# defineZYP/ADT

Hardware: AMD Instinct MI355X
Metric: train sequences/sec, SASRec-ADT ml-1m (seq_len=200, d=64, 2 blocks) (higher is better)
Workload: dtype bf16; 1 GPU; SASRec-ADT ml-1m shape, 2 blocks d=64 H=2 seq_len=200, global batch 256 (256 sequences on this GPU), dropout 0.5, full train step (fwd+loss+bwd+clip+Adam), ids resident in HBM; global_batch=256, seq_len=200, parallelism=dp1, hip_graph=True, table_gradients=sorted segmented sums, bit-reproducible (ADT_ITEM_SORT=1), world_size=1

## Files before the change

### adt_amd/csrc/adt_attn_args.h

```cpp
#pragma once
#include "adt_common.cuh"

namespace adt {

struct AttnArgs {
  const float* Q; int ldq;
  const float* K; int ldk;
  const float* V; int ldv;
  float* O; int ldo;
  float* LSE;
  int B, H, L;
  int causal;
  float scale;
  DropCfg drop;
  uint32_t bh_offset;
  const float* dO; int lddo;
  float* dQ; int lddq;
  float* dK; int lddk;
  float* dV; int lddv;
  uint32_t* mask;
  unsigned long long* stamps;
  int in_bf16;
  int out_bf16;
  const void* do_bf16; const float* do_delta;
};

}
```

### adt_amd/csrc/adt_bwdchain_args.h

```cpp
#pragma once
#include "adt_common.cuh"

namespace adt {

struct BwdChainArgs {
  int T, L, B;
  const int* ids;
  DropCfg drop; uint32_t site1, site2; uint32_t row_offset;
  float ln_eps;
  const float* gy;
  const float* u;
  const float* xin;
  const float* o;
  const float* dqkv; int lddqkv;
  const float* dkv2;
  int grad_bf16;
  const float* dh;
  const float* f;
  const float* W0; const float* W1; const float* W2; const float* W3;
  const float* gamma; const float* beta;
  float* out0; int acc0;
  float* out1; int acc1;
  float* dW0; float* dW1; float* dW2; float* dW3;
  float* db0; float* db1; float* db2; float* db3;
  float* dgamma; float* dbeta;
  const float* rec; const float* drec; const float* Ws; float* dWs; float* dbs; int H;
  int ablate;
  int nrep; size_t rep_stride;
  float gy_scale;
  float* part[4]; size_t part_stride;
  int saved_bf16;
  unsigned long long* stamps;
  const float* wp_base; const void* wp_img;
  float* vpart;
  const float* lnl_x; const float* lnl_gamma; float lnl_eps; float* vpart2; float* lnl_dgamma; float* lnl_dbeta;
  void* do_bf16; float* do_delta; float do_scale; int do_hd;
  int nsplit;
};

}
```

### adt_amd/csrc/adt_sasrec.hip

```cpp
#include "adt_host.h"
#include <string.h>
#include <mutex>
#include "adt_bwdchain_args.h"
#include "adt_fwdchain_args.h"
#include "adt_seq_args.h"
#include "adt_seqbwd_args.h"

namespace {

constexpr float LN_EPS = 1e-8f;
constexpr int NREPP = 16;
constexpr int LN_PART_BLOCKS = 1024;
constexpr int NREP = 16;

struct Layout {
  int64_t off[4 + 30 * 16];
  int64_t total;
  int nl;
  int64_t item() const { return off[0]; }
  int64_t posw() const { return off[1]; }
  int64_t lnl_w() const { return off[2]; }
  int64_t lnl_b() const { return off[3]; }
  int64_t enc(int i, int k) const { return off[4 + 14 * i + k]; }
  int64_t dec(int i, int k) const { return off[4 + 14 * nl + 16 * i + k]; }
};
enum { E_LN1W, E_LN1B, E_INW, E_INB, E_OW, E_OB, E_LN2W, E_LN2B, E_C1W, E_C1B, E_C2W, E_C2B, E_SW, E_SB };
enum { D_LNW, D_LNB, D_SINW, D_SINB, D_SOW, D_SOB, D_EINW, D_EINB, D_EOW, D_EOB, D_C1W, D_C1B, D_C2W, D_C2B, D_UW, D_UB };

int64_t up64(int64_t x) { return (x + 63) / 64 * 64; }

StepPlan step_plan(const adt_sasrec_cfg* c, int B) {
  const StepFacts f{c->prec, c->maxlen, c->hidden, c->num_heads, c->num_layers, B, c->item_num + 1, adt_item_sort_supported(c->item_num + 1) != 0,
                    c->num_heads > 0 ? adt_seq_attn_bwd_lds(c->maxlen, c->num_heads) : 0};
  return adt_step_plan(f, adt_seq_switches());
}

bool make_layout(const adt_sasrec_cfg* c, Layout* lo) {
  if (c->num_layers < 1 || c->num_layers > 16) return false;
  const int64_t d = c->hidden, H = c->num_heads, hd = d / H, L = c->maxlen, V = c->item_num;
  lo->nl = c->num_layers;
  int64_t o = 0;
  int n = 0;
  auto put = [&](int64_t sz) { lo->off[n++] = o; o += up64(sz); };
  put((V + 1) * d); put(L * d); put(d); put(d);
  for (int i = 0; i < c->num_layers; ++i) {
    put(d); put(d); put(3 * d * d); put(3 * d); put(d * d); put(d); put(d); put(d);
    put(d * d); put(d); put(d * d); put(d); put(H * hd); put(H);
  }
  for (int i = 0; i < c->num_layers; ++i) {
    put(d); put(d);
    put(3 * d * d); put(3 * d); put(d * d); put(d);
    put(3 * d * d); put(3 * d); put(d * d); put(d);
    put(d * d); put(d); put(d * d); put(d); put(d); put(d);
  }
  lo->total = o;
  return true;
}

struct WS {
  int64_t T, d, H, L, nl, B;
  int64_t enc_x, dec_x, f, posl, negl;
  int64_t e_qn, e_qkv, e_o, e_lse, e_h, e_h2, e_u, e_rec, e_mask, e_stride;
  int64_t d_dn, d_qkv, d_o1, d_lse1, d_a1, d_q2, d_kv2, d_o2, d_lse2, d_a2, d_u, d_mask1, d_mask2, d_stride;
  int64_t g_enc_x, g_dec_x, g_f, g_pos, g_neg, g_rec;
  int64_t s1, s2, s3, s4, s5;
  int64_t loss, norms, scal;
  int64_t rep, rep_stride;
  int64_t prep, prep_stride;
  int64_t wpack;
  int64_t part, part_stride;
  int64_t isort, isort_n;
  int64_t dodelta;
  int64_t vpart, vcall, lnpart, gnpart;
  int64_t total;
};

void make_ws(const adt_sasrec_cfg* c, int B, const StepPlan& pl, WS* w) {
  w->B = B; w->d = c->hidden; w->H = c->num_heads; w->L = c->maxlen; w->nl = c->num_layers;
  w->T = (int64_t)B * w->L;
  const int64_t Td = up64(w->T * w->d), T1 = up64(w->T), lse = up64((int64_t)B * w->H * w->L);
  const int64_t rec = up64(w->T * w->H * w->H);
  int64_t o = 0;
  auto take = [&](int64_t n) { int64_t r = o; o += n; return r; };
  w->enc_x = take((w->nl + 1) * Td); w->dec_x = take((w->nl + 1) * Td); w->f = take(Td);
  w->posl = take(T1); w->negl = take(T1);
  {
    const int64_t s = o;
    w->e_qn = take(Td); w->e_qkv = take(3 * Td); w->e_o = take(Td); w->e_lse = take(lse); w->e_h = take(Td);
    w->e_h2 = take(Td); w->e_u = take(Td); w->e_rec = take(rec); w->e_mask = take(8 * lse);
    w->e_stride = o - s;
    o = s + w->e_stride * w->nl;
  }
  {
    const int64_t s = o;
    w->d_dn = take(Td); w->d_qkv = take(3 * Td); w->d_o1 = take(Td); w->d_lse1 = take(lse); w->d_a1 = take(Td);
    w->d_q2 = take(Td); w->d_kv2 = take(2 * Td); w->d_o2 = take(Td); w->d_lse2 = take(lse); w->d_a2 = take(Td);
    w->d_u = take(Td); w->d_mask1 = take(8 * lse); w->d_mask2 = take(8 * lse);
    w->d_stride = o - s;
    o = s + w->d_stride * w->nl;
  }
  w->g_enc_x = take((w->nl + 1) * Td); w->g_dec_x = take((w->nl + 1) * Td); w->g_f = take(Td);
  w->g_pos = take(T1); w->g_neg = take(T1); w->g_rec = take(rec * w->nl);
  w->s1 = take(Td); w->s2 = take(Td); w->s3 = take(3 * Td); w->s4 = take(2 * Td); w->s5 = take(Td);
  w->loss = take(64 * (2 + 2 * 16)); w->norms = take(64); w->scal = take(192);
  w->rep_stride = up64((int64_t)(c->item_num + 1) * w->d);
  w->rep = take(NREP * w->rep_stride);
  {
    Layout lo;
    make_layout(c, &lo);
    w->prep_stride = up64(lo.total - lo.posw());
    w->prep = take(NREPP * w->prep_stride);
    w->wpack = take(3 * w->prep_stride);
  }
  w->part_stride = pl.parts_area ? (int64_t)w->nl * 16 * 4096 : 0;
  w->part = take((int64_t)B * pl.seq_split * w->part_stride);
  w->isort_n = pl.sort_area ? adt_item_sort_work_ints(4, (int)w->T, c->item_num + 1) : 0;
  w->isort = take(up64(w->isort_n));
  w->vcall = (int64_t)B * pl.seq_split * 512;
  w->vpart = take(w->part_stride > 0 ? (5 * w->nl + 1) * w->vcall : 0);
  w->lnpart = take(LN_PART_BLOCKS * 128);
  w->gnpart = take(4096);
  w->dodelta = take(pl.do_handover ? up64(w->T * 4) : 0);
  w->total = o;
}

#define CK(call) do { int _r = (call); if (_r) return _r; } while (0)

struct SideStream {
  hipStream_t s = nullptr;
  hipEvent_t fork_ev[4] = {nullptr, nullptr, nullptr, nullptr}, join_ev[4] = {nullptr, nullptr, nullptr, nullptr};
};
SideStream* side_stream(const StepPlan& pl, hipStream_t main) {
  static SideStream g[16];
  static std::mutex mu;
  if (!pl.side_sites) return nullptr;
  int dev = 0;
  if (hipGetDevice(&dev) != hipSuccess || dev < 0 || dev >= 16) return nullptr;
  SideStream* sd = &g[dev];
  std::lock_guard<std::mutex> lock(mu);
  if (sd->s) return sd;
  hipStreamCaptureStatus cs = hipStreamCaptureStatusNone;
  if (hipStreamIsCapturing(main, &cs) != hipSuccess || cs != hipStreamCaptureStatusNone) { (void)hipGetLastError(); return nullptr; }
  hipStream_t s = nullptr;
  if (hipStreamCreateWithFlags(&s, hipStreamNonBlocking) != hipSuccess) { (void)hipGetLastError(); return nullptr; }
  for (int i = 0; i < 4; ++i)
    if (hipEventCreateWithFlags(&sd->fork_ev[i], hipEventDisableTiming) != hipSuccess ||
        hipEventCreateWithFlags(&sd->join_ev[i], hipEventDisableTiming) != hipSuccess) {
      (void)hipGetLastError();
      (void)hipStreamDestroy(s);
      return nullptr;
    }
  sd->s = s;
  return sd;
}
int side_mark(SideStream* sd, int k, void* main) {
  if (!sd) return 0;
  if (hipEventRecord(sd->fork_ev[k], (hipStream_t)main) != hipSuccess) return adt_set_error("backward: side-stream fork %d failed", k);
  return 0;
}
int side_enter(SideStream* sd, int k, void* main, void** out) {
  *out = main;
  if (!sd) return 0;
  if (hipStreamWaitEvent(sd->s, sd->fork_ev[k], 0) != hipSuccess) return adt_set_error("backward: side-stream fork %d failed", k);
  *out = sd->s;
  return 0;
}
int side_join(SideStream* sd, int k, void* main) {
  if (!sd) return 0;
  if (hipEventRecord(sd->join_ev[k], sd->s) != hipSuccess || hipStreamWaitEvent((hipStream_t)main, sd->join_ev[k], 0) != hipSuccess)
    return adt_set_error("backward: side-stream join %d failed", k);
  return 0;
}

int layout_ws(const adt_sasrec_cfg* c, int B, Layout* lo, WS* w, StepPlan* pl) {
  *pl = step_plan(c, B);
// ... 44 lines not shown
int partial_slots(const adt_sasrec_cfg* c, const Layout& lo, bool enc, bool dec, int* slots, int* offs);
int partial_nwg(const StepPlan& pl, int slot, int B) {
  const int k = slot % 16;
  const bool attn_block = (k >= PS_E_IN && k < PS_E_IN + 3) || (k >= PS_D_SIN && k < PS_D_SIN + 3);
  return attn_block ? B * pl.attn_split : B * pl.seq_split;
}
int reduce_partials(const adt_sasrec_cfg* c, const Layout& lo, const WS& w, const StepPlan& pl, float* G, float* ws, bool enc, bool dec, void* st) {
  int slots[256], offs[256];
  const int n = partial_slots(c, lo, enc, dec, slots, offs);
  int nwg[256];
  for (int i = 0; i < n; ++i) nwg[i] = partial_nwg(pl, slots[i], (int)w.B);
  return adt_dwpart_reduce_n(G, ws + w.part, (size_t)w.part_stride, (int)w.B, nwg, slots, offs, n, st);
}
int partial_slots(const adt_sasrec_cfg* c, const Layout& lo, bool enc, bool dec, int* slots, int* offs) {
  int n = 0;
  const int dd = c->hidden * c->hidden;
  for (int i = 0; i < c->num_layers; ++i) {
    if (enc) {
      for (int j = 0; j < 3; ++j) { slots[n] = 16 * i + PS_E_IN + j; offs[n++] = (int)(lo.enc(i, E_INW) + j * dd); }
      slots[n] = 16 * i + PS_E_O; offs[n++] = (int)lo.enc(i, E_OW);
      slots[n] = 16 * i + PS_E_C1; offs[n++] = (int)lo.enc(i, E_C1W);
      slots[n] = 16 * i + PS_E_C2; offs[n++] = (int)lo.enc(i, E_C2W);
    }
    if (dec) {
      for (int j = 0; j < 3; ++j) { slots[n] = 16 * i + PS_D_SIN + j; offs[n++] = (int)(lo.dec(i, D_SINW) + j * dd); }
      for (int j = 0; j < 3; ++j) { slots[n] = 16 * i + PS_D_EIN + j; offs[n++] = (int)(lo.dec(i, D_EINW) + j * dd); }
      slots[n] = 16 * i + PS_D_SO; offs[n++] = (int)lo.dec(i, D_SOW);
      slots[n] = 16 * i + PS_D_EO; offs[n++] = (int)lo.dec(i, D_EOW);
      slots[n] = 16 * i + PS_D_C1; offs[n++] = (int)lo.dec(i, D_C1W);
      slots[n] = 16 * i + PS_D_C2; offs[n++] = (int)lo.dec(i, D_C2W);
    }
  }
  return n;
}

adt::SeqBwdArgs seq_bwd_args(int L, int B, int H, const int32_t* ids, float p, const uint32_t* seed, uint32_t site, uint32_t b_offset, int hd) {
  adt::SeqBwdArgs a;
  memset(&a, 0, sizeof(a));
  a.L = L; a.B = B; a.H = H; a.ids = ids; a.drop = adt_make_drop(p, seed, site); a.b_offset = b_offset; a.ln_eps = LN_EPS;
  a.scale = 1.0f / sqrtf((float)hd);
  return a;
}

adt::SeqFwdArgs seq_args(int nsplit, int L, int B, int H, const int32_t* ids, float p, const uint32_t* seed, uint32_t b_offset, int hd) {
  adt::SeqFwdArgs a;
  memset(&a, 0, sizeof(a));
  a.nsplit = nsplit;
  a.L = L; a.B = B; a.H = H; a.ids = ids; a.drop = adt_make_drop(p, seed, 0); a.b_offset = b_offset; a.ln_eps = LN_EPS;
  a.scale = 1.0f / sqrtf((float)hd);
  return a;
}

adt::SeqFwdArgs enc_layer_seq_args(const adt_sasrec_cfg* c, const Layout& lo, const WS& w, const StepPlan& pl, const float* P, float* ws, const int32_t* seq,
                                   float p, const uint32_t* seed, uint32_t b_offset, int i, bool training_outputs, bool lean) {
  const int d = (int)w.d, H = (int)w.H, hd = d / H, L = (int)w.L, B = (int)w.B, prec = c->prec;
  const int64_t Td = up64(w.T * w.d);
  float* x = ws + w.enc_x + i * Td;
  float* y = ws + w.enc_x + (i + 1) * Td;
  float* base = ws + i * w.e_stride;
  adt::SeqFwdArgs a = seq_args(pl.seq_split, L, B, H, seq, p, seed, b_offset, hd);
  a.x = i == 0 ? nullptr : x; a.E = P + lo.item(); a.P = P + lo.posw(); a.emb_scale = sqrtf((float)d); a.site_emb = SITE_EMB_SEQ;
  a.site_attn = enc_site(i, 0); a.site1 = enc_site(i, 1); a.site2 = enc_site(i, 2);
  a.gamma = P + lo.enc(i, E_LN1W); a.beta = P + lo.enc(i, E_LN1B); a.Win = P + lo.enc(i, E_INW); a.bin = P + lo.enc(i, E_INB);
  a.Wo = P + lo.enc(i, E_OW); a.bo = P + lo.enc(i, E_OB); a.gamma2 = P + lo.enc(i, E_LN2W); a.beta2 = P + lo.enc(i, E_LN2B);
  a.W1 = P + lo.enc(i, E_C1W); a.b1 = P + lo.enc(i, E_C1B); a.W2 = P + lo.enc(i, E_C2W); a.b2 = P + lo.enc(i, E_C2B);
  a.x_out = x; a.xn = base + w.e_qn; a.qkv = base + w.e_qkv; a.o = base + w.e_o; a.lse = base + w.e_lse;
  a.mask = reinterpret_cast<uint32_t*>(base + w.e_mask); a.h = base + w.e_h; a.u = base + w.e_u; a.y = y;
  if (training_outputs && H > 1) { a.rec = base + w.e_rec; a.Ws = P + lo.enc(i, E_SW); a.bs = P + lo.enc(i, E_SB); }
  a.wp_base = P + lo.posw(); a.wp_img = prec == ADT_PREC_BF16 ? (const void*)(ws + w.wpack) : nullptr;
  if (lean) { a.xn = nullptr; a.qkv = nullptr; a.saved_bf16 = 1; }
  return a;
}

int encoder_forward(const adt_sasrec_cfg* c, const Layout& lo, const WS& w, const StepPlan& pl, const float* P, float* ws,
                    const int32_t* seq, const int32_t* pos, const int32_t* neg, float p, const uint32_t* seed,
                    uint32_t b_offset, bool training_outputs, void* st, bool packed = false) {
  const int T = (int)w.T, d = (int)w.d, H = (int)w.H, hd = d / H, L = (int)w.L, B = (int)w.B, prec = c->prec, nl = c->num_layers;
  const int64_t Td = up64(w.T * w.d);
  const uint32_t ro = b_offset * (uint32_t)L;
  const int dd = d * d;
  const bool use_seq = pl.use_seq;
  const bool lean = training_outputs && pl.lean;
  if (!packed) CK(pack_weights(c, lo, w, P, ws, st));
  const float* wp_base = P + lo.posw();
  const void* wp_img = prec == ADT_PREC_BF16 ? (const void*)(ws + w.wpack) : nullptr;
  for (int i = 0; i < nl; ++i) {
    float* x = ws + w.enc_x + i * Td;
    float* y = ws + w.enc_x + (i + 1) * Td;
    float* base = ws + i * w.e_stride;
    float *qn = base + w.e_qn, *qkv = base + w.e_qkv, *o = base + w.e_o, *lse = base + w.e_lse, *h = base + w.e_h,
          *u = base + w.e_u, *rec = base + w.e_rec;
    const float* inw = P + lo.enc(i, E_INW);
    const float* inb = P + lo.enc(i, E_INB);
    if (use_seq) {
      const adt::SeqFwdArgs a = enc_layer_seq_args(c, lo, w, pl, P, ws, seq, p, seed, b_offset, i, training_outputs, lean);
      CK(adt_launch_seq_enc_fwd(hd, a, st));
      continue;
    }
    {
      adt::FwdChainArgs a = fwd_args(T, L, B, H, seq, p, seed, ro);
      a.x = i == 0 ? nullptr : x; a.E = P + lo.item(); a.P = P + lo.posw(); a.emb_scale = sqrtf((float)d); a.site0 = SITE_EMB_SEQ;
      a.gamma = P + lo.enc(i, E_LN1W); a.beta = P + lo.enc(i, E_LN1B);
      for (int j = 0; j < 3; ++j) { a.W[j] = inw + j * dd; a.b[j] = inb + j * d; }
      a.o0 = x; a.ld0 = d; a.o1 = qn; a.ld1 = d; a.o2 = qkv; a.ld2 = 3 * d;
      CK(adt_launch_fwdchain(prec, 0, a, st));
    }
    CK(adt_attn_fwd(prec, qkv, 3 * d, qkv + d, 3 * d, qkv + 2 * d, 3 * d, B, H, L, hd, 1, p, seed, enc_site(i, 0), b_offset, o, d,
                    lse, reinterpret_cast<uint32_t*>(base + w.e_mask), st));
    {
      adt::FwdChainArgs a = fwd_args(T, L, B, H, seq, p, seed, ro);
      a.x = o; a.r0 = qn; a.site1 = enc_site(i, 1); a.site2 = enc_site(i, 2);
      a.W[0] = P + lo.enc(i, E_OW); a.b[0] = P + lo.enc(i, E_OB);
      a.W[1] = P + lo.enc(i, E_C1W); a.b[1] = P + lo.enc(i, E_C1B);
      a.W[2] = P + lo.enc(i, E_C2W); a.b[2] = P + lo.enc(i, E_C2B);
      a.gamma = P + lo.enc(i, E_LN2W); a.beta = P + lo.enc(i, E_LN2B);
      a.o0 = h; a.ld0 = d; a.o1 = u; a.ld1 = d; a.o2 = y; a.ld2 = d;
      int which = 2;
      if (training_outputs) {
        a.rec = rec; a.Ws = P + lo.enc(i, E_SW); a.bs = P + lo.enc(i, E_SB);
        which = H <= 2 ? 6 : (H <= 4 ? 7 : 8);
      }
      CK(adt_launch_fwdchain(prec, which, a, st));
    }
  }
  for (int j0 = 0; j0 == 0 || (training_outputs && !use_seq && j0 < nl); j0 += 2) {
    adt::FwdChainArgs a = fwd_args(T, L, B, H, seq, 0.f, nullptr, ro);
    a.x = ws + w.enc_x + nl * Td; a.gamma = P + lo.lnl_w(); a.beta = P + lo.lnl_b();
    if (j0 == 0) { a.o0 = ws + w.f; a.ld0 = d; }
    if (training_outputs) {
      if (j0 == 0) { a.E = P + lo.item(); a.pos = pos; a.neg = neg; a.pos_logits = ws + w.posl; a.neg_logits = ws + w.negl; }
      a.nkv = use_seq ? 0 : (nl - j0 >= 2 ? 2 : 1);
      for (int k = 0; k < a.nkv; ++k) {
        const float* einw = P + lo.dec(j0 + k, D_EINW);
        const float* einb = P + lo.dec(j0 + k, D_EINB);
        a.W[2 * k] = einw + dd; a.W[2 * k + 1] = einw + 2 * dd; a.b[2 * k] = einb + d; a.b[2 * k + 1] = einb + 2 * d;
        float* kv2 = ws + (j0 + k) * w.d_stride + w.d_kv2;
        if (k == 0) { a.o2 = kv2; a.ld2 = 2 * d; } else { a.o3 = kv2; a.ld3 = 2 * d; }
      }
    }
    CK(adt_launch_fwdchain(prec, 5, a, st));
  }
  return 0;
}

adt::SeqFwdArgs dec_layer_seq_args(const Layout& lo, const WS& w, const StepPlan& pl, const float* P, float* ws, const int32_t* dec, float p,
                                   const uint32_t* seed, uint32_t b_offset, int i) {
  const int d = (int)w.d, H = (int)w.H, hd = d / H, L = (int)w.L, B_ = (int)w.B;
  const int64_t Td = up64(w.T * w.d);
  float* x = ws + w.dec_x + i * Td;
  float* y = ws + w.dec_x + (i + 1) * Td;
  float* base = ws + i * w.d_stride;
  float *dn = base + w.d_dn, *qkv = base + w.d_qkv, *o1 = base + w.d_o1, *lse1 = base + w.d_lse1, *a1 = base + w.d_a1,
        *q2 = base + w.d_q2, *kv2 = base + w.d_kv2, *o2 = base + w.d_o2, *lse2 = base + w.d_lse2, *a2 = base + w.d_a2, *u = base + w.d_u;
  adt::SeqFwdArgs a = seq_args(pl.seq_split, L, B_, H, dec, p, seed, b_offset, hd);
  a.x = i == 0 ? nullptr : x; a.E = P + lo.item(); a.P = P + lo.posw(); a.emb_scale = sqrtf((float)d); a.site_emb = SITE_EMB_DEC;
  a.site_attn = dec_site(i, 0); a.site_attn2 = dec_site(i, 1); a.site1 = dec_site(i, 2); a.site2 = dec_site(i, 3);
  a.gamma = P + lo.dec(i, D_LNW); a.beta = P + lo.dec(i, D_LNB); a.Win = P + lo.dec(i, D_SINW); a.bin = P + lo.dec(i, D_SINB);
  a.Wo = P + lo.dec(i, D_SOW); a.bo = P + lo.dec(i, D_SOB); a.f = ws + w.f; a.Win2 = P + lo.dec(i, D_EINW); a.bin2 = P + lo.dec(i, D_EINB);
  a.Wo2 = P + lo.dec(i, D_EOW); a.bo2 = P + lo.dec(i, D_EOB);
  a.W1 = P + lo.dec(i, D_C1W); a.b1 = P + lo.dec(i, D_C1B); a.W2 = P + lo.dec(i, D_C2W); a.b2 = P + lo.dec(i, D_C2B);
  a.x_out = x; a.xn = dn; a.qkv = qkv; a.o = o1; a.lse = lse1; a.mask = reinterpret_cast<uint32_t*>(base + w.d_mask1);
  a.a1 = a1; a.q2 = q2; a.kv2 = kv2; a.o2 = o2; a.lse2 = lse2; a.mask2 = reinterpret_cast<uint32_t*>(base + w.d_mask2);
  a.h = a2; a.u = u; a.y = y;
  a.wp_base = P + lo.posw(); a.wp_img = ws + w.wpack;
  if (pl.lean) { a.xn = nullptr; a.qkv = nullptr; a.saved_bf16 = 1; }
  return a;
}
int dec_layer_seq_fwd(const Layout& lo, const WS& w, const StepPlan& pl, const float* P, float* ws, const int32_t* dec, float p,
                      const uint32_t* seed, uint32_t b_offset, int i, void* st) {
  const adt::SeqFwdArgs a = dec_layer_seq_args(lo, w, pl, P, ws, dec, p, seed, b_offset, i);
  return adt_launch_seq_dec_fwd((int)(w.d / w.H), a, st);
}

SideStream* fwd_logits_stream(const StepPlan& pl, void* st) { return ((pl.side_sites & 1) && !pl.bce_merged) ? side_stream(pl, (hipStream_t)st) : nullptr; }
bool ring_prefetch_split(const adt::RingPrefetchArgs& rr, bool bce_by_forward, const StepPlan& pl) {
  return rr.ring && rr.staging && rr.state && bce_by_forward && pl.embed3_on;
}

struct LossPtrs { const float *A[4], *Bm[4], *rc[4]; float *GA[4], *GB[4], *lm[4], *dr[4], *ln[4]; };
AdtLossSeedsJob loss_terms(const WS& w, float* ws, const float* lambdas1, const float* lambdas2, bool all_seeds, LossPtrs* q) {
  const int nl = (int)w.nl, H = (int)w.H;
  const int64_t Td = up64(w.T * w.d), rec = up64(w.T * w.H * w.H);
  float* loss = ws + w.loss;
  for (int i = 0; i < nl; ++i) {
    q->A[i] = ws + w.enc_x + i * Td; q->Bm[i] = ws + w.dec_x + (nl - i) * Td;
    q->GA[i] = all_seeds ? ws + w.g_enc_x + i * Td : nullptr;
    q->GB[i] = (all_seeds || i == 0) ? ws + w.g_dec_x + (nl - i) * Td : nullptr;
    q->lm[i] = loss + 64 * (2 + i);
    q->rc[i] = ws + i * w.e_stride + w.e_rec; q->dr[i] = ws + w.g_rec + i * rec; q->ln[i] = loss + 64 * (2 + nl + i);
  }
  AdtLossSeedsJob j{};
  j.T = (int)w.T; j.norms = ws + w.norms; j.loss_bce = loss;
  j.nmse = nl; j.A = q->A; j.Bm = q->Bm; j.n = w.T * w.d; j.lambdas = lambdas1; j.GA = q->GA; j.GB = q->GB; j.loss_mse = q->lm;
  j.nnll = H > 1 ? nl : 0; j.rec = q->rc; j.n_rows = (int)w.T; j.H = H; j.lambda2 = lambdas2[nl - 1]; j.drec = q->dr; j.loss_nll = q->ln;
  return j;
}

int forward_loss_lean(const adt_sasrec_cfg* c, const Layout& lo, const WS& w, const StepPlan& pl, const float* P, float* ws, const int32_t* seq, const int32_t* dec,
                      const int32_t* pos, const int32_t* neg, bool bce_side, float p, const uint32_t* seed, uint32_t b_offset, const float* lambdas1,
                      const float* lambdas2, const adt::RingPrefetchArgs& rr, void* st) {
  const int hd = (int)(w.d / w.H), nl = c->num_layers;
  if (!pl.bce_deferred) return 1;
  for (int i = 0; i < nl; ++i) {
    adt::SeqFwdArgs a = enc_layer_seq_args(c, lo, w, pl, P, ws, seq, p, seed, b_offset, i, true, true);
    if (i == nl - 1) { a.lnl_gamma = P + lo.lnl_w(); a.lnl_beta = P + lo.lnl_b(); a.f_out = ws + w.f; }
    CK(adt_launch_seq_enc_fwd(hd, a, st));
  }
  for (int j = 0; j < nl; ++j) CK(dec_layer_seq_fwd(lo, w, pl, P, ws, dec, p, seed, b_offset, j, st));
  LossPtrs q;
  AdtLossSeedsJob job = loss_terms(w, ws, lambdas1, lambdas2, false, &q);
  job.ring = &rr; job.split = ring_prefetch_split(rr, bce_side, pl);
  const adt::LogitsBceArgs lb{ws + w.f, P + lo.item(), pos, neg, ws + w.norms, (int)w.T, ws + w.posl, ws + w.negl, ws + w.g_pos, ws + w.g_neg, ws + w.loss,
                              ws + w.g_f, pl.det ? nullptr : ws + w.rep, NREP, (size_t)w.rep_stride, pl.embed3_on ? 1 : 0};
  const bool merged = bce_side && pl.bce_merged;
  if (merged) job.logits = &lb;
  SideStream* const sd = (bce_side && !merged) ? fwd_logits_stream(pl, st) : nullptr;
  if (bce_side && !merged) CK(side_mark(sd, 0, st));
  CK(adt_loss_seeds_prefetch(job, st));
  if (bce_side && !merged) {
    void* s2 = nullptr;
    CK(side_enter(sd, 0, st, &s2));
    CK(adt_logits_bce_scatter_ex(lb.F, lb.E, pos, neg, lb.norms, lb.T, lb.pos_logits, lb.neg_logits, lb.dpos, lb.dneg, lb.loss, lb.dF, lb.rep, lb.nrep,
                                 w.rep_stride, lb.neg_only, s2));
    if (sd && hipEventRecord(sd->join_ev[0], sd->s) != hipSuccess) return adt_set_error("forward_loss: logits event");
  }
  return 0;
}

int g_time_which = 0, g_time_layer = 0;
hipEvent_t g_time_ev0 = nullptr, g_time_ev1 = nullptr;
inline void time_mark(int which, int layer, bool start, void* st) {
  if (!g_time_ev0 || !g_time_ev1 || g_time_layer != layer) return;
  if (g_time_which == 3 && which == 1 && start) {
    (void)hipEventRecord(g_time_ev0, (hipStream_t)st);
    (void)hipEventRecord(g_time_ev1, (hipStream_t)st);
  } else if (g_time_which == which) {
    (void)hipEventRecord(start ? g_time_ev0 : g_time_ev1, (hipStream_t)st);
  }
}

const char* const NO_FALLBACK = "backward: shape L=%d hd=%d left the per-sequence kernels although the partial-gradient path was chosen";

struct Bwd {
  const adt_sasrec_cfg* c; Layout lo; WS w;
  const float* P; float* G; float* ws;
  const int32_t *seq, *dec, *pos, *neg;
  float p; const uint32_t* seed; uint32_t b_offset, ro;
  void* st;
  BwdPlan plan;
  StepPlan sp;
  BwdCallPlan call;
  adt::RingPrefetchArgs ring;
  int T, d, H, hd, L, prec, nl;
  int64_t Td, recsz;
  float* Gq;
  float *s1, *s3, *s4, *s5, *gf;
  void* do_rows() const { return sp.do_handover ? (void*)s3 : nullptr; }
  void* do_rows_cross() const { return sp.do_handover ? (void*)s1 : nullptr; }
  float* do_delta() const { return sp.do_handover ? ws + w.dodelta : nullptr; }
  float do_scale(uint32_t site) const { return adt_make_drop(p, seed, site).scale; }
  const float* f;
  SideStream *sd, *sd_sort;

  adt::BwdChainArgs BA(const int32_t* ids, float pp, const uint32_t* sdp) const {
    adt::BwdChainArgs a = bwd_args(T, L, (int)w.B, ids, pp, sdp, ro);
    a.nrep = NREPP; a.rep_stride = (size_t)w.prep_stride;
    a.wp_base = P + lo.posw(); a.wp_img = prec == ADT_PREC_BF16 ? (const void*)(ws + w.wpack) : nullptr;
    a.nsplit = sp.seq_split;
    return a;
  }
  float* PART(int layer, int slot) const { return sp.parts ? ws + w.part + (int64_t)(16 * layer + slot) * 4096 : nullptr; }
  float* VPART(int layer, int k) const { return call.late_parts ? ws + w.vpart + (int64_t)(5 * layer + k) * w.vcall : nullptr; }
  int logits_scatter(void* s) const {
    if (plan.bce_here)
      return adt_logits_bce_scatter_ex(f, P + lo.item(), pos, neg, ws + w.norms, T, ws + w.posl, ws + w.negl, ws + w.g_pos, ws + w.g_neg, ws + w.loss,
                                       gf, sp.det ? nullptr : ws + w.rep, NREP, w.rep_stride, call.embed3 ? 1 : 0, s);
    if (sp.det) return adt_logits_bwd_df(P + lo.item(), pos, neg, ws + w.g_pos, ws + w.g_neg, T, d, gf, d, s);
    return adt_logits_bwd_scatter(f, d, P + lo.item(), pos, neg, ws + w.g_pos, ws + w.g_neg, T, d, gf, d, ws + w.rep, NREP, w.rep_stride, s);
  }
  int zero_unless_prezeroed(int64_t at, size_t n, void* s) const {
    return (!plan.prep_zeroed && adt::zero_f32_async(ws + at, n, (hipStream_t)s)) ? adt_set_error("replica zero") : 0;
  }
};

int bwd_init(Bwd& x, const adt_sasrec_cfg* c, const float* P, float* G, float* ws, const int32_t* seq, const int32_t* dec, const int32_t* pos,
             const int32_t* neg, int B, int training, const uint32_t* seed, uint32_t b_offset, int phase, const adt::RingPrefetchArgs& ring, void* st) {
  CK(layout_ws(c, B, &x.lo, &x.w, &x.sp));
  if (const char* err = adt_bwd_plan(phase, x.sp.bce_deferred, &x.plan)) return adt_set_error("%s", err);
  x.call = adt_bwd_call_plan(x.sp, x.plan);
  const WS& w = x.w;
  x.c = c; x.P = P; x.G = G; x.ws = ws; x.seq = seq; x.dec = dec; x.pos = pos; x.neg = neg; x.seed = seed; x.b_offset = b_offset; x.st = st; x.ring = ring;
  x.T = (int)w.T; x.d = (int)w.d; x.H = (int)w.H; x.hd = x.d / x.H; x.L = (int)w.L; x.prec = c->prec; x.nl = c->num_layers;
  x.Td = up64(w.T * w.d); x.recsz = up64(w.T * w.H * w.H);
  x.p = training ? c->dropout : 0.f;
  x.ro = b_offset * (uint32_t)x.L;
  x.s1 = ws + w.s1; x.s3 = ws + w.s3; x.s4 = ws + w.s4; x.s5 = ws + w.s5; x.gf = ws + w.g_f; x.f = ws + w.f;
  x.Gq = ws + w.prep - x.lo.posw();
  x.sd_sort = x.sp.det ? side_stream(x.sp, (hipStream_t)st) : nullptr;
  x.sd = x.call.side ? side_stream(x.sp, (hipStream_t)st) : nullptr;
  return 0;
}

struct LogitsSide {
  enum { DONE, MARKED, ENQUEUED, BY_FORWARD } at = DONE;

  int begin(const Bwd& x) {
    const WS& w = x.w;
    if (x.plan.bce_fwd) {
      at = BY_FORWARD;
    } else if (x.sp.det) {
      CK(x.zero_unless_prezeroed(w.prep, (size_t)NREPP * w.prep_stride, x.st));
      CK(x.logits_scatter(x.st));
    } else if (x.sd && (x.sp.side_sites & 1)) {
      CK(side_mark(x.sd, 0, x.st));
      CK(x.zero_unless_prezeroed(w.prep, (size_t)NREPP * w.prep_stride, x.st));
      at = MARKED;
    } else {
      CK(x.zero_unless_prezeroed(w.rep, (size_t)NREP * w.rep_stride + (size_t)NREPP * w.prep_stride, x.st));
      CK(x.logits_scatter(x.st));
    }
    return 0;
  }
  int after_first_chain_kernel(const Bwd& x) {
    if (at != MARKED) return 0;
    void* s2 = nullptr;
    CK(side_enter(x.sd, 0, x.st, &s2));
    CK(x.zero_unless_prezeroed(x.w.rep, (size_t)NREP * x.w.rep_stride, s2));
    CK(x.logits_scatter(s2));
    at = ENQUEUED;
    return 0;
  }
  int join(const Bwd& x) {
    if (at == ENQUEUED) CK(side_join(x.sd, 0, x.st));
    if (at == BY_FORWARD) {
      SideStream* const sl = fwd_logits_stream(x.sp, x.st);
      if (sl && hipStreamWaitEvent((hipStream_t)x.st, sl->join_ev[0], 0) != hipSuccess) return adt_set_error("backward: logits join");
    }
    at = DONE;
    return 0;
  }
};

int dec_post_bwd(const Bwd& x, int i) {
  const WS& w = x.w; const Layout& lo = x.lo; const float* P = x.P; float* const Gq = x.Gq;
  float* base = x.ws + i * w.d_stride;
  adt::BwdChainArgs a = x.BA(x.dec, x.p, x.seed);
  a.site1 = dec_site(i, 2); a.site2 = dec_site(i, 3);
  a.gy = x.ws + w.g_dec_x + (i + 1) * x.Td; a.u = base + w.d_u; a.xin = base + w.d_a2; a.o = base + w.d_o2; a.saved_bf16 = x.sp.lean;
  a.W0 = P + lo.dec(i, D_C2W); a.W1 = P + lo.dec(i, D_C1W); a.W2 = P + lo.dec(i, D_EOW);
  a.dW0 = Gq + lo.dec(i, D_C2W); a.dW1 = Gq + lo.dec(i, D_C1W); a.dW2 = Gq + lo.dec(i, D_EOW);
  a.db0 = Gq + lo.dec(i, D_C2B); a.db1 = Gq + lo.dec(i, D_C1B); a.db2 = Gq + lo.dec(i, D_EOB);
  a.out0 = x.s1;
  a.do_bf16 = x.do_rows_cross(); a.do_delta = x.do_delta(); a.do_scale = x.do_scale(dec_site(i, 1)); a.do_hd = x.hd;
  a.part[0] = x.PART(i, PS_D_C2); a.part[1] = x.PART(i, PS_D_C1); a.part[2] = x.PART(i, PS_D_EO); a.part_stride = (size_t)w.part_stride;
  a.vpart = x.VPART(i, 0);
  const int rc = x.sp.use_seq ? adt_launch_seq_post_bwd(x.hd, 0, a, x.st) : 1;
  if (rc < 0) return rc;
  if (rc && x.sp.parts) return adt_set_error(NO_FALLBACK, x.L, x.hd);
  return rc ? adt_launch_bwdchain(x.prec, 1, a, x.st) : 0;
}

adt::AttnArgs dec_cross_attn_lean_args(const Bwd& x, int i);

int dec_cross_attn_bwd(const Bwd& x, int i) {
  const WS& w = x.w; const int d = x.d, B = (int)w.B;
  float* base = x.ws + i * w.d_stride;
  float *q2 = base + w.d_q2, *kv2 = base + w.d_kv2, *o2 = base + w.d_o2, *lse2 = base + w.d_lse2, *s4 = x.s4;
  const uint32_t* mask2 = reinterpret_cast<const uint32_t*>(base + w.d_mask2);
  if (!x.sp.lean)
    return adt_attn_bwd(x.prec, q2, d, kv2, 2 * d, kv2 + d, 2 * d, o2, d, lse2, x.s1, d, B, x.H, x.L, x.hd, 1, x.p, x.seed, dec_site(i, 1), x.b_offset,
                        x.s5, d, s4, 2 * d, s4 + d, 2 * d, mask2, x.st);
  if (x.sp.do_handover) {
    const int rc = adt_launch_seq_attn_bwd(x.hd, dec_cross_attn_lean_args(x, i), x.st);
    return rc == 1 ? adt_set_error(NO_FALLBACK, x.L, x.hd) : rc;
  }
  const uint16_t* kvb = reinterpret_cast<const uint16_t*>(kv2);
  return adt_attn_bwd_saved_bf16(q2, d, kvb, 2 * d, kvb + d, 2 * d, o2, d, lse2, x.s1, d, B, x.H, x.L, x.hd, x.p, x.seed, dec_site(i, 1), x.b_offset,
                                 x.s5, d, s4, 2 * d, x.sp.parts ? s4 + d / 2 : s4 + d, 2 * d, mask2, x.sp.parts ? 1 : 0, x.st);
}

adt::BwdChainArgs dec_mid_seq_args(const Bwd& x, int i) {
  const WS& w = x.w; const Layout& lo = x.lo; const float* P = x.P; float* const Gq = x.Gq;
  const int d = x.d, dd = d * d;
  float* base = x.ws + i * w.d_stride;
  const float* einw = P + lo.dec(i, D_EINW);
  float* geinw = Gq + lo.dec(i, D_EINW);
  float* geinb = Gq + lo.dec(i, D_EINB);
  adt::BwdChainArgs a = x.BA(x.dec, 0.f, nullptr);
  a.dqkv = x.s5; a.lddqkv = d; a.xin = base + w.d_a1; a.o = base + w.d_o1; a.saved_bf16 = x.sp.lean; a.dkv2 = x.s4; a.f = x.f;
  a.grad_bf16 = (x.sp.lean && x.sp.parts) ? 1 : 0;
  a.W0 = einw; a.W1 = P + lo.dec(i, D_SOW); a.W2 = einw + dd; a.W3 = einw + 2 * dd;
  a.dW0 = geinw; a.dW1 = Gq + lo.dec(i, D_SOW); a.dW2 = geinw + dd; a.dW3 = geinw + 2 * dd;
  a.db0 = geinb; a.db1 = Gq + lo.dec(i, D_SOB); a.db2 = geinb + d; a.db3 = geinb + 2 * d;
  a.out0 = x.s1; a.out1 = x.gf; a.acc1 = 1;
  a.part[0] = x.PART(i, PS_D_EIN); a.part[1] = x.PART(i, PS_D_SO); a.part[2] = x.PART(i, PS_D_EIN + 1); a.part[3] = x.PART(i, PS_D_EIN + 2);
  a.part_stride = (size_t)w.part_stride;
  a.vpart = x.VPART(i, 1);
  a.do_bf16 = x.do_rows(); a.do_delta = x.do_delta(); a.do_scale = x.do_scale(dec_site(i, 0)); a.do_hd = x.hd;
  return a;
}

adt::AttnArgs dec_cross_attn_lean_args(const Bwd& x, int i) {
  const WS& w = x.w; const int d = x.d;
  float* base = x.ws + i * w.d_stride;
  const uint16_t* kvb = reinterpret_cast<const uint16_t*>(base + w.d_kv2);
  adt::AttnArgs a = adt_attn_bwd_saved_bf16_args(base + w.d_q2, d, kvb, 2 * d, kvb + d, 2 * d, base + w.d_o2, d, base + w.d_lse2, x.s1, d, (int)w.B, x.H, x.L,
                                                 x.hd, x.p, x.seed, dec_site(i, 1), x.b_offset, x.s5, d, x.s4, 2 * d, x.s4 + d / 2, 2 * d,
                                                 reinterpret_cast<const uint32_t*>(base + w.d_mask2), 1);
  a.do_bf16 = x.do_rows_cross(); a.do_delta = x.do_delta();
  return a;
}

int dec_mid_bwd(const Bwd& x, int i) {
  const WS& w = x.w; const Layout& lo = x.lo; const float* P = x.P; float* const Gq = x.Gq;
  const int d = x.d, dd = d * d;
  float* base = x.ws + i * w.d_stride;
  float *o1 = base + w.d_o1, *a1 = base + w.d_a1;
  const float* einw = P + lo.dec(i, D_EINW);
  float* geinw = Gq + lo.dec(i, D_EINW);
  float* geinb = Gq + lo.dec(i, D_EINB);
  if (x.sp.use_seq) {
    const int rc = adt_launch_seq_mid_bwd(x.hd, dec_mid_seq_args(x, i), x.st);
    if (rc <= 0) return rc;
    if (x.sp.parts) return adt_set_error(NO_FALLBACK, x.L, x.hd);
  }
  {
    adt::BwdChainArgs a = x.BA(x.dec, 0.f, nullptr);
    a.dqkv = x.s5; a.lddqkv = d; a.xin = a1; a.o = o1; a.saved_bf16 = x.sp.lean;
    a.W0 = einw; a.W1 = P + lo.dec(i, D_SOW);
    a.dW0 = geinw; a.dW1 = Gq + lo.dec(i, D_SOW); a.db0 = geinb; a.db1 = Gq + lo.dec(i, D_SOB);
    a.out0 = x.s1;
    CK(adt_launch_bwdchain(x.prec, 4, a, x.st));
  }
  adt::BwdChainArgs a = x.BA(x.dec, 0.f, nullptr);
  a.dkv2 = x.s4; a.f = x.f;
  a.W0 = einw + dd; a.W1 = einw + 2 * dd;
  a.dW0 = geinw + dd; a.dW1 = geinw + 2 * dd; a.db0 = geinb + d; a.db1 = geinb + 2 * d;
  a.out0 = x.gf; a.acc0 = 1;
  return adt_launch_bwdchain(x.prec, 5, a, x.st);
}

int attn_block_bwd(const Bwd& x, int i, bool dec) {
  const WS& w = x.w; const Layout& lo = x.lo; const float* P = x.P; float* const Gq = x.Gq; float* const ws = x.ws;
  const int d = x.d, dd = d * d, nl = x.nl;
  const int32_t* ids = dec ? x.dec : x.seq;
  float* gy = ws + (dec ? w.g_dec_x : w.g_enc_x) + (i + 1) * x.Td;
  float* gx = ws + (dec ? w.g_dec_x : w.g_enc_x) + i * x.Td;
  const float* xi = ws + (dec ? w.dec_x : w.enc_x) + i * x.Td;
  float* base = ws + i * (dec ? w.d_stride : w.e_stride);
  float *qkv = base + (dec ? w.d_qkv : w.e_qkv), *o = base + (dec ? w.d_o1 : w.e_o), *lse = base + (dec ? w.d_lse1 : w.e_lse);
  const uint32_t* mask = reinterpret_cast<const uint32_t*>(base + (dec ? w.d_mask1 : w.e_mask));
  const int64_t lnw = dec ? lo.dec(i, D_LNW) : lo.enc(i, E_LN1W), lnb = dec ? lo.dec(i, D_LNB) : lo.enc(i, E_LN1B);
  const int64_t inw = dec ? lo.dec(i, D_SINW) : lo.enc(i, E_INW), inb = dec ? lo.dec(i, D_SINB) : lo.enc(i, E_INB);
  const uint32_t site = dec ? dec_site(i, 0) : enc_site(i, 0);
  const int acc = dec ? (i > 0 ? 1 : 0) : 1;
  if (x.sp.use_seq) {
    adt::SeqBwdArgs a = seq_bwd_args(x.L, (int)w.B, x.H, ids, x.p, x.seed, site, x.b_offset, x.hd);
    a.x = xi; a.gamma = P + lnw; a.beta = P + lnb; a.Win = P + inw; a.bin = P + inb;
    a.dO = x.s1; a.o = o; a.lse = lse; a.mask = mask; a.dres = dec ? gy : x.s5;
    a.do_bf16 = x.do_rows(); a.do_delta = x.do_delta();
    a.gx = gx; a.acc = acc; a.dWin = Gq + inw; a.dbin = Gq + inb; a.dgamma = Gq + lnw; a.dbeta = Gq + lnb;
    if (x.plan.seeds_virtual && dec && i > 0) {
      a.acc = 0; a.seed_other = ws + w.enc_x + (nl - i) * x.Td; a.seed_coef = ws + w.norms + 8 + (nl - i);
    }
    if (x.plan.seeds_virtual && !dec) {
      a.acc = 0; a.seed_other = ws + w.dec_x + (nl - i) * x.Td; a.seed_coef = ws + w.norms + 8 + i;
      if (i > 0) { a.seed_loss = ws + w.loss + 64 * (2 + i); a.seed_norms = ws + w.norms; }
    }
    a.nrep = NREPP; a.rep_stride = (size_t)w.prep_stride; a.wp_base = P + lo.posw(); a.wp_img = ws + w.wpack; a.saved_bf16 = x.sp.lean;
    a.part = x.PART(i, dec ? PS_D_SIN : PS_E_IN); a.part_stride = (size_t)w.part_stride;
    a.vpart = x.VPART(i, dec ? 2 : 4);
    a.nsplit = a.part ? x.sp.attn_split : 1;
    time_mark(dec ? 2 : 1, i, true, x.st);
    const int rc = adt_launch_seq_attn_pre_bwd(x.hd, dec ? 1 : 0, a, x.st);
    time_mark(dec ? 2 : 1, i, false, x.st);
    if (rc <= 0) return rc;
    if (x.sp.lean) return adt_set_error("backward: the lean forward needs the fused attention-block backward (L=%d hd=%d)", x.L, x.hd);
  }
  if (x.sp.do_handover) return adt_set_error("backward: the staged attention backward was reached with the dO hand-over on (L=%d hd=%d)", x.L, x.hd);
  CK(adt_attn_bwd(x.prec, qkv, 3 * d, qkv + d, 3 * d, qkv + 2 * d, 3 * d, o, d, lse, x.s1, d, (int)w.B, x.H, x.L, x.hd, 1, x.p, x.seed, site, x.b_offset,
                  x.s3, 3 * d, x.s3 + d, 3 * d, x.s3 + 2 * d, 3 * d, mask, x.st));
  adt::BwdChainArgs a = x.BA(ids, 0.f, nullptr);
  a.dqkv = x.s3; a.lddqkv = 3 * d; a.xin = xi;
  if (dec) a.gy = gy; else a.dh = x.s5;
  a.W0 = P + inw; a.W1 = P + inw + dd; a.W2 = P + inw + 2 * dd; a.gamma = P + lnw; a.beta = P + lnb;
  a.dW0 = Gq + inw; a.dW1 = Gq + inw + dd; a.dW2 = Gq + inw + 2 * dd; a.db0 = Gq + inb; a.db1 = Gq + inb + d; a.db2 = Gq + inb + 2 * d;
  a.dgamma = Gq + lnw; a.dbeta = Gq + lnb;
  a.out0 = gx; a.acc0 = acc;
  return adt_launch_bwdchain(x.prec, dec ? 3 : 2, a, x.st);
}

int dec_block_backward(const Bwd& x, int i, LogitsSide& logits) {
  CK(dec_post_bwd(x, i));
  CK(logits.after_first_chain_kernel(x));
  if (x.sp.use_seq && x.sp.lean && x.sp.parts) {
    const adt::AttnArgs at = dec_cross_attn_lean_args(x, i);
    const adt::BwdChainArgs mid = dec_mid_seq_args(x, i);
    if (adt_seq_xattn_mid_covered(x.hd, at, mid)) {
      CK(logits.join(x));
      const int rc = adt_launch_seq_xattn_mid_bwd(x.hd, at, mid, x.st);
      if (rc) return rc < 0 ? rc : adt_set_error("backward: the fused cross-attention + mid launch refused a shape it covers (L=%d hd=%d)", x.L, x.hd);
      return attn_block_bwd(x, i, true);
    }
  }
  CK(dec_cross_attn_bwd(x, i));
  CK(logits.join(x));
  CK(dec_mid_bwd(x, i));
  return attn_block_bwd(x, i, true);
}

struct DecSide {
  enum { NONE, MARKED, ENQUEUED } at = NONE;
  bool parts_done = false;
// ... 26 lines not shown
    return 0;
  }
  int enter(const Bwd& x) {
    if (at != MARKED) return 0;
    void* s2 = nullptr;
    CK(side_enter(x.sd, 1, x.st, &s2));
    if (!x.sp.det && !x.call.embed3) CK(embed(x, s2));
    if (x.sp.parts && !x.call.late_parts) { CK(reduce_partials(x.c, x.lo, x.w, x.sp, x.G, x.ws, false, true, s2)); parts_done = true; }
    at = ENQUEUED;
    return 0;
  }
  int join(const Bwd& x, bool covered) {
    if (at == ENQUEUED && !covered) CK(side_join(x.sd, 1, x.st));
    at = NONE;
    return 0;
  }
};

int last_layernorm_bwd(const Bwd& x) {
  const WS& w = x.w; const Layout& lo = x.lo; float* const ws = x.ws;
  const int d = x.d;
  if (x.sp.lnl_fused) return 0;
  if (x.call.late_parts) {
    const int nb = adt_layernorm_bwd_parts(x.gf, d, ws + w.enc_x + x.nl * x.Td, d, x.P + lo.lnl_w(), LN_EPS, x.T, d, ws + w.g_enc_x + x.nl * x.Td, d, 0,
                                           ws + w.lnpart, LN_PART_BLOCKS, x.st);
    return nb < 0 ? nb : 0;
  }
  return adt_layernorm_bwd_rep(x.gf, d, ws + w.enc_x + x.nl * x.Td, d, x.P + lo.lnl_w(), LN_EPS, x.T, d, ws + w.g_enc_x + x.nl * x.Td, d, 0,
                               x.Gq + lo.lnl_w(), x.Gq + lo.lnl_b(), NREPP, w.prep_stride, x.st);
}

int enc_post_bwd(const Bwd& x, int i) {
  const WS& w = x.w; const Layout& lo = x.lo; const float* P = x.P; float* const Gq = x.Gq; float* const ws = x.ws;
  const int H = x.H, nl = x.nl;
  float* base = ws + i * w.e_stride;
  adt::BwdChainArgs a = x.BA(x.seq, x.p, x.seed);
  a.site1 = enc_site(i, 1); a.site2 = enc_site(i, 2);
  a.gy = ws + w.g_enc_x + (i + 1) * x.Td; a.u = base + w.e_u; a.xin = base + w.e_h; a.o = base + w.e_o; a.saved_bf16 = x.sp.lean;
  a.W0 = P + lo.enc(i, E_C2W); a.W1 = P + lo.enc(i, E_C1W); a.W2 = P + lo.enc(i, E_OW);
  a.gamma = P + lo.enc(i, E_LN2W); a.beta = P + lo.enc(i, E_LN2B);
  a.dW0 = Gq + lo.enc(i, E_C2W); a.dW1 = Gq + lo.enc(i, E_C1W); a.dW2 = Gq + lo.enc(i, E_OW);
  a.db0 = Gq + lo.enc(i, E_C2B); a.db1 = Gq + lo.enc(i, E_C1B); a.db2 = Gq + lo.enc(i, E_OB);
  a.dgamma = Gq + lo.enc(i, E_LN2W); a.dbeta = Gq + lo.enc(i, E_LN2B);
  a.out0 = x.s5; a.out1 = x.s1;
  int which = 0;
  if (H > 1 && H <= 4) {
    which = H <= 2 ? 6 : 7;
    a.rec = base + w.e_rec; a.drec = ws + w.g_rec + i * x.recsz; a.Ws = P + lo.enc(i, E_SW); a.dWs = Gq + lo.enc(i, E_SW);
    a.dbs = Gq + lo.enc(i, E_SB); a.H = H;
  }
  a.part[0] = x.PART(i, PS_E_C2); a.part[1] = x.PART(i, PS_E_C1); a.part[2] = x.PART(i, PS_E_O); a.part_stride = (size_t)w.part_stride;
  a.vpart = x.VPART(i, 3);
  a.do_bf16 = x.do_rows(); a.do_delta = x.do_delta(); a.do_scale = x.do_scale(enc_site(i, 0)); a.do_hd = x.hd;
  if (x.sp.lnl_fused && i == nl - 1) {
    a.gy = x.gf; a.lnl_x = ws + w.enc_x + nl * x.Td; a.lnl_gamma = P + lo.lnl_w(); a.lnl_eps = LN_EPS;
    a.vpart2 = x.call.late_parts ? ws + w.vpart + (int64_t)(5 * nl) * w.vcall : nullptr;
    a.lnl_dgamma = Gq + lo.lnl_w(); a.lnl_dbeta = Gq + lo.lnl_b();
  }
  const int rc = x.sp.use_seq ? adt_launch_seq_post_bwd(x.hd, 1, a, x.st) : 1;
  if (rc < 0) return rc;
  if (rc && x.sp.parts) return adt_set_error(NO_FALLBACK, x.L, x.hd);
  return rc ? adt_launch_bwdchain(x.prec, which, a, x.st) : 0;
}

int enc_block_backward(const Bwd& x, int i, DecSide& dec_side) {
  const WS& w = x.w; const Layout& lo = x.lo;
  CK(enc_post_bwd(x, i));
  if (x.sp.lnl_fused && i == x.nl - 1) CK(dec_side.enter(x));
  if (x.H > 4) {
    float* base = x.ws + i * w.e_stride;
    CK(adt_headcls_bwd(base + w.e_o, x.d, x.P + lo.enc(i, E_SW), base + w.e_rec, x.ws + w.g_rec + i * x.recsz, (int)w.B, x.L, x.H, x.hd, x.s1, x.d,
                       x.G + lo.enc(i, E_SW), x.G + lo.enc(i, E_SB), x.st));
  }
  return attn_block_bwd(x, i, false);
}

int table_gradients(const Bwd& x, DecSide& dec_side) {
  const WS& w = x.w; const Layout& lo = x.lo; float* const ws = x.ws; float* const G = x.G;
  const int phase = x.plan.phase;
  if (phase == 2 && !x.sp.det && adt::zero_f32_async(ws + w.rep, (size_t)NREP * w.rep_stride, (hipStream_t)x.st)) return adt_set_error("replica zero");
  SideStream* const sd2 = ((x.sp.side_sites & 4) && x.sp.parts && !x.call.late_parts) ? x.sd : nullptr;
  CK(dec_side.join(x, sd2 != nullptr));
  void* s2 = nullptr;
  CK(side_mark(sd2, 2, x.st));
  if (x.sp.det) {
    if (x.sd_sort && hipStreamWaitEvent((hipStream_t)x.st, x.sd_sort->join_ev[3], 0) != hipSuccess) return adt_set_error("backward: sort join");
    const uint32_t site4[4] = {SITE_EMB_SEQ, SITE_EMB_DEC, 0u, 0u};
    const int32_t* const ids2[2] = {x.seq, x.dec};
    const float* const dx2[2] = {ws + w.g_enc_x, ws + w.g_dec_x};
    CK(adt_item_segsum_posemb(reinterpret_cast<int32_t*>(ws + w.isort), 4, x.T, x.c->item_num + 1, 0xFu, site4, x.p, x.seed, sqrtf((float)x.d), G + lo.item(),
                              x.plan.prep_zeroed ? 0 : 1, ids2, dx2, site4, 2, (int)w.B, x.L, x.ro, G + lo.posw(), x.st));
  } else if (x.call.embed3) {
    const bool by_forward = phase == 2 ? x.plan.seeds_virtual : x.plan.bce_fwd;
    CK(adt_embed_bwd3_prefetch(x.seq, x.dec, x.pos, ws + w.g_enc_x, ws + w.g_dec_x, x.f, ws + w.g_pos, x.T, x.L, x.p, x.seed, SITE_EMB_SEQ, SITE_EMB_DEC, x.ro,
                               G + lo.posw(), ws + w.rep, NREP, w.rep_stride, ring_prefetch_split(x.ring, by_forward, x.sp) ? &x.ring : nullptr, x.st));
  } else {
    CK(adt_embed_bwd_rep(x.seq, ws + w.g_enc_x, x.T, x.L, x.d, x.p, x.seed, SITE_EMB_SEQ, x.ro, G + lo.posw(), ws + w.rep, NREP, w.rep_stride, x.st));
  }
  CK(side_enter(sd2, 2, x.st, &s2));
  if (x.sp.parts && !x.call.late_parts) CK(reduce_partials(x.c, lo, w, x.sp, G, ws, true, phase == 0 && !dec_side.parts_done, s2));
  CK(side_join(sd2, 2, x.st));
  if (x.plan.defer_fold) return 0;
  return adt_replica_reduce2(G + lo.item(), ws + w.rep, (int64_t)(x.c->item_num + 1) * x.d, x.sp.det ? 0 : NREP, w.rep_stride, G + lo.posw(), x.Gq + lo.posw(),
                             (phase == 0 ? lo.total : lo.dec(0, 0)) - lo.posw(), NREPP, w.prep_stride, x.st);
}

// ... 30 lines not shown

extern "C" {

int64_t adt_sasrec_param_layout(const adt_sasrec_cfg* cfg, int64_t* offsets) {
  Layout lo;
  if (!make_layout(cfg, &lo)) return adt_set_error("param_layout: bad cfg");
  if (offsets)
    for (int i = 0; i < 4 + 30 * cfg->num_layers; ++i) offsets[i] = lo.off[i];
  return lo.total;
}

int64_t adt_sasrec_workspace_floats(const adt_sasrec_cfg* cfg, int B) {
  WS w;
  make_ws(cfg, B, step_plan(cfg, B), &w);
  return w.total;
}

int64_t adt_sasrec_ws_offset(const adt_sasrec_cfg* cfg, int B, int what, int layer) {
  WS w;
  make_ws(cfg, B, step_plan(cfg, B), &w);
  const int64_t Td = up64(w.T * w.d), rec = up64(w.T * w.H * w.H);
  switch (what) {
    case ADT_WS_ENC_X: return w.enc_x + layer * Td;
    case ADT_WS_DEC_X: return w.dec_x + layer * Td;
    case ADT_WS_REC: return layer * w.e_stride + w.e_rec;
    case ADT_WS_POS_LOGITS: return w.posl;
    case ADT_WS_NEG_LOGITS: return w.negl;
    case ADT_WS_F: return w.f;
    case ADT_WS_G_ENC_X: return w.g_enc_x + layer * Td;
    case ADT_WS_G_DEC_X: return w.g_dec_x + layer * Td;
    case ADT_WS_G_REC: return w.g_rec + layer * rec;
    case ADT_WS_G_POS: return w.g_pos;
    case ADT_WS_G_NEG: return w.g_neg;
    case ADT_WS_LOSS: return w.loss;
    case ADT_WS_NORMS: return w.norms;
    case ADT_WS_SCAL: return w.scal;
  }
  return adt_set_error("ws_offset: unknown id %d", what);
}

int adt_sasrec_forward(const adt_sasrec_cfg* c, const float* P, float* ws, const int32_t* seq, const int32_t* dec,
                       const int32_t* pos, const int32_t* neg, int B, int training, const uint32_t* seed,
                       uint32_t b_offset, void* st) {
  Layout lo;
  WS w;
  StepPlan pl;
  CK(layout_ws(c, B, &lo, &w, &pl));
  const int T = (int)w.T, d = (int)w.d, H = (int)w.H, hd = d / H, L = (int)w.L, prec = c->prec;
  const int64_t Td = up64(w.T * w.d);
  const bool packed = (training & ADT_TRAIN_PACKED) != 0;
  training &= ADT_TRAIN_DROPOUT;
  const float p = training ? c->dropout : 0.f;
  const uint32_t ro = b_offset * (uint32_t)L;
  CK(encoder_forward(c, lo, w, pl, P, ws, seq, pos, neg, p, seed, b_offset, true, st, packed));
  const float* f = ws + w.f;
  const int dd = d * d;
  const int B_ = (int)w.B;
  for (int i = 0; i < c->num_layers; ++i) {
    float* x = ws + w.dec_x + i * Td;
    float* y = ws + w.dec_x + (i + 1) * Td;
    float* base = ws + i * w.d_stride;
    float *dn = base + w.d_dn, *qkv = base + w.d_qkv, *o1 = base + w.d_o1, *lse1 = base + w.d_lse1, *a1 = base + w.d_a1,
          *q2 = base + w.d_q2, *kv2 = base + w.d_kv2, *o2 = base + w.d_o2, *lse2 = base + w.d_lse2, *a2 = base + w.d_a2,
          *u = base + w.d_u;
    const float* sinw = P + lo.dec(i, D_SINW);
    const float* sinb = P + lo.dec(i, D_SINB);
    const float* einw = P + lo.dec(i, D_EINW);
    const float* einb = P + lo.dec(i, D_EINB);
    if (pl.use_seq) {
      CK(dec_layer_seq_fwd(lo, w, pl, P, ws, dec, p, seed, b_offset, i, st));
      continue;
    }
    {
      adt::FwdChainArgs a = fwd_args(T, L, B_, H, dec, p, seed, ro);
      a.x = i == 0 ? nullptr : x; a.E = P + lo.item(); a.P = P + lo.posw(); a.emb_scale = sqrtf((float)d); a.site0 = SITE_EMB_DEC;
      a.gamma = P + lo.dec(i, D_LNW); a.beta = P + lo.dec(i, D_LNB);
      for (int j = 0; j < 3; ++j) { a.W[j] = sinw + j * dd; a.b[j] = sinb + j * d; }
      a.o0 = x; a.ld0 = d; a.o1 = dn; a.ld1 = d; a.o2 = qkv; a.ld2 = 3 * d;
      CK(adt_launch_fwdchain(prec, 1, a, st));
    }
    CK(adt_attn_fwd(prec, qkv, 3 * d, qkv + d, 3 * d, qkv + 2 * d, 3 * d, B_, H, L, hd, 1, p, seed, dec_site(i, 0), b_offset, o1, d,
                    lse1, reinterpret_cast<uint32_t*>(base + w.d_mask1), st));
    {
      adt::FwdChainArgs a = fwd_args(T, L, B_, H, dec, 0.f, nullptr, ro);
      a.x = o1; a.W[0] = P + lo.dec(i, D_SOW); a.b[0] = P + lo.dec(i, D_SOB); a.W[1] = einw; a.b[1] = einb;
      a.o0 = a1; a.ld0 = d; a.o2 = q2; a.ld2 = d;
      CK(adt_launch_fwdchain(prec, 3, a, st));
    }
    CK(adt_attn_fwd(prec, q2, d, kv2, 2 * d, kv2 + d, 2 * d, B_, H, L, hd, 1, p, seed, dec_site(i, 1), b_offset, o2, d, lse2,
                    reinterpret_cast<uint32_t*>(base + w.d_mask2), st));
    {
      adt::FwdChainArgs a = fwd_args(T, L, B_, H, dec, p, seed, ro);
      a.x = o2; a.r0 = dn; a.site1 = dec_site(i, 2); a.site2 = dec_site(i, 3);
      a.W[0] = P + lo.dec(i, D_EOW); a.b[0] = P + lo.dec(i, D_EOB);
      a.W[1] = P + lo.dec(i, D_C1W); a.b[1] = P + lo.dec(i, D_C1B);
      a.W[2] = P + lo.dec(i, D_C2W); a.b[2] = P + lo.dec(i, D_C2B);
      a.o0 = a2; a.ld0 = d; a.o1 = u; a.ld1 = d; a.o2 = y; a.ld2 = d;
      CK(adt_launch_fwdchain(prec, 4, a, st));
    }
  }
  return 0;
}

int adt_sasrec_bce_deferred(const adt_sasrec_cfg* c) {
  const StepPlan pl = step_plan(c, 1);
  if (pl.cfg_error[0]) (void)adt_set_error("%s", pl.cfg_error);
  return !pl.cfg_error[0] && pl.bce_deferred ? 1 : 0;
// ... 335 lines not shown
```

### adt_amd/csrc/adt_seq.hip

```cpp
#include "adt_host.h"
#include <limits.h>
#include <atomic>
#include "adt_seqfwd.cuh"
#include "adt_seqfwd_tt.cuh"
#include "adt_seqattn.cuh"
#include "adt_seqbwd_tt.cuh"
#include "adt_seqpost_tt.cuh"
#include "adt_seqxattn_tt.cuh"

using namespace adt;

template <class Args>
static int seq_launch(const void* fn, size_t smem, AdtLdsOptIn& slot, int grid, const Args* args, hipStream_t s, const char* what, int nwaves = SQ_NW,
                      size_t optin = 0) {
  return adt_launch_lds1(fn, dim3(grid), dim3(nwaves * 64), smem, *args, s, what, slot, optin);
}

__global__ __launch_bounds__(256) void k_pack_wimg(PackArgs a) { pack_wimg_block(a, blockIdx.x); }

extern "C" int adt_pack_wimg(const float* base, void* img, const int* offs, int n, void* stream) {
  if (n < 1 || n > 256) return adt_set_error("pack_wimg: %d blocks", n);
  PackArgs a;
  a.base = base; a.img = reinterpret_cast<__bf16*>(img); a.n = n;
  for (int i = 0; i < n; ++i) a.off[i] = offs[i];
  hipLaunchKernelGGL(k_pack_wimg, dim3(n), dim3(256), 0, (hipStream_t)stream, a);
  return adt_check_launch("pack_wimg");
}

static_assert(ADT_SEQ_MAXLEN == SQ_LP && ADT_SEQ_MAXLEN == SB_R, "adt_step_plan.h restates the image rows of these kernels");

const SeqSwitches& adt_seq_switches() {
  static const SeqSwitches sw = [] {
    SeqSwitches s;
    s.seq = adt_env_on("ADT_SEQ"); s.seq_lean = adt_env_on("ADT_SEQ_LEAN"); s.seq_tt = adt_env_on("ADT_SEQ_TT"); s.seq_bwd = adt_env_on("ADT_SEQ_BWD");
    s.seq_attn_bwd = adt_env_on("ADT_SEQ_ATTN_BWD"); s.seq_post_bwd = adt_env_on("ADT_SEQ_POST_BWD"); s.seq_partials = adt_env_on("ADT_SEQ_PARTIALS");
    s.xattn_fused = adt_env_on("ADT_XATTN_FUSED"); s.do_bf16 = adt_env_on("ADT_DO_BF16");
    s.seq_ablate = adt_env_int("ADT_SEQ_ABLATE", 0); s.seq_ablate_set = adt_env_int("ADT_SEQ_ABLATE", INT_MIN) != INT_MIN;
    s.seq_split = adt_env_int("ADT_SEQ_SPLIT", 0); s.attn_split = adt_env_on("ADT_ATTN_SPLIT");
    s.side_stream = adt_env_int("ADT_SIDE_STREAM", 7); s.side_stream_dp = adt_env_int("ADT_SIDE_STREAM_DP", 0) != 0;
    s.item_sort = adt_env_int("ADT_ITEM_SORT", 0) != 0;
    s.lnl_fused = adt_env_on("ADT_LNL_FUSED"); s.fold_parts = adt_env_on("ADT_FOLD_PARTS"); s.fwd_fused = adt_env_on("ADT_FWD_FUSED");
    s.embed3 = adt_env_on("ADT_EMBED3"); s.bce_merged = adt_env_on("ADT_BCE_MERGED");
    return s;
  }();
  return sw;
}

static SeqAttnFacts attn_facts(const AttnArgs& a) {
  return {a.L, a.H, a.B, a.causal != 0, a.in_bf16 != 0, a.out_bf16 != 0, a.ldq, a.ldk, a.ldv, a.ldo, a.lddo, a.drop.thr != 0, a.mask != nullptr,
          sab_lds_bytes(a.L, a.H), xm_lds_bytes(a.L, a.H)};
}
size_t adt_seq_attn_bwd_lds(int L, int H) { return sab_lds_bytes(L, H); }
static SeqChainFacts chain_facts(const BwdChainArgs& a) {
  return {a.L, a.H, a.B, a.T, a.wp_img != nullptr, a.saved_bf16 != 0, a.grad_bf16 != 0, a.part[0] && a.part[1] && a.part[2] && a.part[3], a.nsplit, a.ablate,
          a.drec != nullptr};
}

static unsigned long long* g_stamps = nullptr;

extern "C" int adt_seq_stamps_read(unsigned long long* out, int n) {
  if (!g_stamps) return -1;
  if (hipDeviceSynchronize() != hipSuccess) return -2;
  return hipMemcpy(out, g_stamps, (size_t)n * sizeof(unsigned long long), hipMemcpyDeviceToHost) == hipSuccess ? 0 : -3;
}

static int seq_stamps_mode() {
  static const int st = [] {
    const int v = adt_env_int("ADT_SEQ_STAMPS", 0);
    return (v && hipMalloc(&g_stamps, 16 * 16 * sizeof(unsigned long long)) != hipSuccess) ? 0 : v;
  }();
  return st;
}
static unsigned long long* seq_stamp_buffer(bool for_attention) { return seq_stamps_mode() == (for_attention ? 2 : 1) ? g_stamps : nullptr; }
static unsigned long long* seq_stamp_buffer_post() { return seq_stamps_mode() == 3 ? g_stamps : nullptr; }
static unsigned long long* seq_stamp_buffer_mode(int mode) { return seq_stamps_mode() == mode ? g_stamps : nullptr; }

static void seq_ablate(SeqFwdArgs& a) {
  a.stamps = seq_stamp_buffer(false);
  const int ab = adt_seq_switches().seq_ablate;
  a.ablate = ab;
  if (ab & 1) { a.qkv = nullptr; a.o = nullptr; a.h = nullptr; a.u = nullptr; a.a1 = nullptr; a.q2 = nullptr; a.kv2 = nullptr; a.o2 = nullptr; a.mask = nullptr; a.mask2 = nullptr; }
}

static bool seq_use_tt(const SeqFwdArgs& a) {
  return adt_seq_fwd_tt(adt_seq_switches(), a.wp_img != nullptr, a.L);
}

int adt_launch_seq_enc_fwd(int hd, const SeqFwdArgs& a, void* stream) {
  static AdtLdsOptIn optin[3], optin_tt[3];
  SeqFwdArgs args = a;
  seq_ablate(args);
  hipStream_t s = (hipStream_t)stream;
  if (seq_use_tt(args)) {
    const int nsp = args.nsplit > 1 ? args.nsplit : 1;
    const size_t smem_tt = SeqTtLds<6>::bytes;
    if (hd == 64) return seq_launch((const void*)k_seqtt_enc_fwd<64>, smem_tt, optin_tt[0], a.B * nsp, &args, s, "seqtt_enc_fwd<64>", TQ_FWD_NW);
    if (hd == 32) return seq_launch((const void*)k_seqtt_enc_fwd<32>, smem_tt, optin_tt[1], a.B * nsp, &args, s, "seqtt_enc_fwd<32>", TQ_FWD_NW);
    if (hd == 16) return seq_launch((const void*)k_seqtt_enc_fwd<16>, smem_tt, optin_tt[2], a.B * nsp, &args, s, "seqtt_enc_fwd<16>", TQ_FWD_NW);
  }
  args.nsplit = 0;
  const size_t smem = SeqFwdLds<6>::bytes;
  if (hd == 64) return seq_launch((const void*)k_seq_enc_fwd<64, 2>, smem, optin[0], a.B, &args, s, "seq_enc_fwd<64>");
  if (hd == 32) return seq_launch((const void*)k_seq_enc_fwd<32, 2>, smem, optin[1], a.B, &args, s, "seq_enc_fwd<32>");
  if (hd == 16) return seq_launch((const void*)k_seq_enc_fwd<16, 4>, smem, optin[2], a.B, &args, s, "seq_enc_fwd<16>");
  return adt_set_error("seq_enc_fwd: head size %d", hd);
}

int adt_launch_seq_dec_fwd(int hd, const SeqFwdArgs& a, void* stream) {
  static AdtLdsOptIn optin[3], optin_tt[3];
  SeqFwdArgs args = a;
  seq_ablate(args);
  hipStream_t s = (hipStream_t)stream;
  if (seq_use_tt(args)) {
    const int nsp = args.nsplit > 1 ? args.nsplit : 1;
    const size_t smem_tt = SeqTtLds<5>::bytes;
    if (hd == 64) return seq_launch((const void*)k_seqtt_dec_fwd<64>, smem_tt, optin_tt[0], a.B * nsp, &args, s, "seqtt_dec_fwd<64>", TQ_FWD_NW);
    if (hd == 32) return seq_launch((const void*)k_seqtt_dec_fwd<32>, smem_tt, optin_tt[1], a.B * nsp, &args, s, "seqtt_dec_fwd<32>", TQ_FWD_NW);
    if (hd == 16) return seq_launch((const void*)k_seqtt_dec_fwd<16>, smem_tt, optin_tt[2], a.B * nsp, &args, s, "seqtt_dec_fwd<16>", TQ_FWD_NW);
  }
  args.nsplit = 0;
  const size_t smem = SeqFwdLds<5>::bytes;
  if (hd == 64) return seq_launch((const void*)k_seq_dec_fwd<64>, smem, optin[0], a.B, &args, s, "seq_dec_fwd<64>");
  if (hd == 32) return seq_launch((const void*)k_seq_dec_fwd<32>, smem, optin[1], a.B, &args, s, "seq_dec_fwd<32>");
  if (hd == 16) return seq_launch((const void*)k_seq_dec_fwd<16>, smem, optin[2], a.B, &args, s, "seq_dec_fwd<16>");
  return adt_set_error("seq_dec_fwd: head size %d", hd);
}

static std::atomic<unsigned long long> g_do_handover_launches{0};
extern "C" unsigned long long adt_seq_do_handover_launches() { return g_do_handover_launches.load(); }

int adt_launch_seq_attn_bwd(int hd, const AttnArgs& a, void* stream) {
  if (!adt_covers_attn_bwd(adt_seq_switches(), hd, attn_facts(a))) return 1;
  if (a.do_bf16 && (!a.do_delta || !a.in_bf16)) return adt_set_error("seq_attn_bwd: handed-over dO rows need their delta and bf16 operand rows");
  const size_t smem = sab_lds_bytes(a.L, a.H);
  const int mode = a.drop.thr == 0 ? 0 : (a.mask != nullptr ? 1 : 2);
  static AdtLdsOptIn optin[9];
  const void* fns[9] = {(const void*)k_seq_attn_bwd<64, 0>, (const void*)k_seq_attn_bwd<64, 1>, (const void*)k_seq_attn_bwd<64, 2>,
                        (const void*)k_seq_attn_bwd<32, 0>, (const void*)k_seq_attn_bwd<32, 1>, (const void*)k_seq_attn_bwd<32, 2>,
                        (const void*)k_seq_attn_bwd<16, 0>, (const void*)k_seq_attn_bwd<16, 1>, (const void*)k_seq_attn_bwd<16, 2>};
  const int slot = (hd == 64 ? 0 : hd == 32 ? 3 : 6) + mode;
  AttnArgs args = a;
  args.stamps = seq_stamp_buffer(true);
  if (!args.stamps) args.stamps = seq_stamp_buffer_mode(4);
  const int rc = adt_launch_lds1(fns[slot], dim3(a.B), dim3(SAB_NW * 64), smem, args, (hipStream_t)stream, "seq_attn_bwd", optin[slot], ADT_LDS_MAX);
  if (rc == 0 && a.do_bf16) ++g_do_handover_launches;
  return rc;
}

template <int HD, bool DEC>
static int seq_attn_pre_bwd_t(int mode, const SeqBwdArgs& a, hipStream_t s) {
  constexpr int H = 64 / HD;
  const size_t smem = SeqBwdLds<H>::bytes;
  static AdtLdsOptIn optin[3];
  const void* fns[3] = {(const void*)k_seqtt_attn_pre_bwd<HD, 0, DEC>, (const void*)k_seqtt_attn_pre_bwd<HD, 1, DEC>,
                        (const void*)k_seqtt_attn_pre_bwd<HD, 2, DEC>};
  SeqBwdArgs args = a;
  args.stamps = seq_stamp_buffer(true);
  if (a.nsplit == 2 && !a.part) return adt_set_error("seqtt_attn_pre_bwd: two workgroups per sequence need the weight-gradient partials");
  if (a.nsplit != 2) args.nsplit = 1;
  const int rc = seq_launch(fns[mode], smem, optin[mode], a.B * args.nsplit, &args, s, "seqtt_attn_pre_bwd");
  if (rc == 0 && a.do_bf16) ++g_do_handover_launches;
  return rc;
}

int adt_launch_seq_attn_pre_bwd(int hd, int dec, const SeqBwdArgs& a, void* stream) {
  SeqChainFacts f{};
  f.L = a.L; f.H = a.H; f.B = a.B; f.T = a.B * a.L; f.wimg = a.wp_img != nullptr;
  if (!adt_covers_attn_pre_bwd(adt_seq_switches(), hd, f)) return 1;
  if (a.do_bf16 && !a.do_delta) return adt_set_error("seqtt_attn_pre_bwd: handed-over dO rows without their delta");
  const int mode = a.drop.thr == 0 ? 0 : (a.mask != nullptr ? 1 : 2);
  hipStream_t s = (hipStream_t)stream;
  if (hd == 32) return dec ? seq_attn_pre_bwd_t<32, true>(mode, a, s) : seq_attn_pre_bwd_t<32, false>(mode, a, s);
  if (hd == 64) return dec ? seq_attn_pre_bwd_t<64, true>(mode, a, s) : seq_attn_pre_bwd_t<64, false>(mode, a, s);
  return dec ? seq_attn_pre_bwd_t<16, true>(mode, a, s) : seq_attn_pre_bwd_t<16, false>(mode, a, s);
}

int adt_launch_seq_post_bwd(int hd, int enc, const BwdChainArgs& a, void* stream) {
  if (!adt_covers_post_bwd(adt_seq_switches(), hd, enc != 0, chain_facts(a))) return 1;
  static AdtLdsOptIn optin[6];
  const void* fns[6] = {(const void*)k_seqtt_post_bwd<64, false>, (const void*)k_seqtt_post_bwd<64, true>, (const void*)k_seqtt_post_bwd<32, false>,
                        (const void*)k_seqtt_post_bwd<32, true>, (const void*)k_seqtt_post_bwd<16, false>, (const void*)k_seqtt_post_bwd<16, true>};
  const int slot = (hd == 64 ? 0 : hd == 32 ? 2 : 4) + (enc ? 1 : 0);
  BwdChainArgs args = a;
  args.stamps = enc ? seq_stamp_buffer_post() : nullptr;
  return seq_launch(fns[slot], SeqPostLds<3>::bytes, optin[slot], a.B * (a.nsplit > 1 ? a.nsplit : 1), &args, (hipStream_t)stream, "seqtt_post_bwd", SP_NW);
}

int adt_launch_seq_mid_bwd(int hd, const BwdChainArgs& a, void* stream) {
  if (!adt_covers_mid_bwd(adt_seq_switches(), hd, chain_facts(a))) return 1;
  static AdtLdsOptIn optin;
  BwdChainArgs args = a;
  args.stamps = seq_stamp_buffer_mode(5);
  return seq_launch((const void*)k_seqtt_mid_bwd, SeqPostLds<4>::bytes, optin, a.B * (a.nsplit > 1 ? a.nsplit : 1), &args, (hipStream_t)stream, "seqtt_mid_bwd", SP_MID_NW);
}

static std::atomic<unsigned long long> g_xattn_fused_launches{0};
extern "C" unsigned long long adt_seq_xattn_fused_launches() { return g_xattn_fused_launches.load(); }

int adt_seq_xattn_mid_covered(int hd, const AttnArgs& at, const BwdChainArgs& ch) {
  const bool handover = ch.dqkv == at.dQ && ch.lddqkv == at.lddq && at.lddq == 64 && ch.dkv2 == at.dK && at.lddk == 128 && at.lddv == 128 &&
                        reinterpret_cast<const __bf16*>(at.dV) == reinterpret_cast<const __bf16*>(at.dK) + 64;
  return adt_covers_xattn_mid(adt_seq_switches(), hd, attn_facts(at), chain_facts(ch), handover);
}

int adt_launch_seq_xattn_mid_bwd(int hd, const AttnArgs& at, const BwdChainArgs& ch, void* stream) {
  if (!adt_seq_xattn_mid_covered(hd, at, ch)) return 1;
  XattnMidArgs a{};
  a.Q = reinterpret_cast<const __bf16*>(at.Q); a.K = reinterpret_cast<const __bf16*>(at.K); a.V = reinterpret_cast<const __bf16*>(at.V);
  a.O = reinterpret_cast<const __bf16*>(at.O); a.ldq = at.ldq; a.ldk = at.ldk; a.ldv = at.ldv; a.ldo = at.ldo;
  a.LSE = at.LSE; a.dO = at.dO; a.lddo = at.lddo; a.L = at.L; a.mask = at.mask; a.scale = at.scale; a.drop = at.drop;
  a.xin = ch.xin; a.o = ch.o; a.f = ch.f; a.wp_base = ch.wp_base; a.wp_img = ch.wp_img;
  a.W0 = ch.W0; a.W1 = ch.W1; a.W2 = ch.W2; a.W3 = ch.W3;
  a.out0 = ch.out0; a.out1 = ch.out1; a.acc1 = ch.acc1; a.nrep = ch.nrep; a.rep_stride = ch.rep_stride;
  a.db0 = ch.db0; a.db1 = ch.db1; a.db2 = ch.db2; a.db3 = ch.db3; a.vpart = ch.vpart;
  for (int k = 0; k < 4; ++k) a.part[k] = ch.part[k];
  a.part_stride = ch.part_stride;
  a.do_bf16 = ch.do_bf16; a.do_delta = ch.do_delta; a.do_scale = ch.do_scale;
  a.dO_bf16 = reinterpret_cast<const __bf16*>(at.do_bf16); a.dO_delta = at.do_delta;
  if (at.do_bf16 && !at.do_delta) return adt_set_error("seqtt_xattn_mid_bwd: handed-over dO rows without their delta");
  a.stamps = seq_stamp_buffer_mode(6);
  const int mode = at.drop.thr == 0 ? 0 : 1;
  static AdtLdsOptIn optin[6];
  const void* fns[6] = {(const void*)k_seqtt_xattn_mid_bwd<64, 0>, (const void*)k_seqtt_xattn_mid_bwd<64, 1>, (const void*)k_seqtt_xattn_mid_bwd<32, 0>,
                        (const void*)k_seqtt_xattn_mid_bwd<32, 1>, (const void*)k_seqtt_xattn_mid_bwd<16, 0>, (const void*)k_seqtt_xattn_mid_bwd<16, 1>};
  const int slot = (hd == 64 ? 0 : hd == 32 ? 2 : 4) + mode;
  const size_t most = xm_lds_bytes(ADT_SEQ_MAXLEN, at.H) <= ADT_LDS_MAX ? xm_lds_bytes(ADT_SEQ_MAXLEN, at.H) : xm_lds_bytes(128, at.H);
  const int rc = seq_launch(fns[slot], xm_lds_bytes(at.L, at.H), optin[slot], at.B, &a, (hipStream_t)stream, "seqtt_xattn_mid_bwd", XM_NW, most);
  if (rc == 0) ++g_xattn_fused_launches;
  if (rc == 0 && at.do_bf16) ++g_do_handover_launches;
  return rc;
}

struct PartReduceArgs {
  float* G; const float* part; size_t stride; int nwg; int nslots;
  int slot[256]; int off[256];
  int nwg_slot[256];
};
constexpr int PR_SPLIT = 4;
__global__ __launch_bounds__(256) void k_dwpart_reduce(PartReduceArgs a) {
  typedef unsigned u4v __attribute__((ext_vector_type(4)));
  const int j = blockIdx.x, item = threadIdx.x;
  const int nwg = a.nwg_slot[j];
  const int per = (nwg + PR_SPLIT - 1) / PR_SPLIT, w0 = blockIdx.y * per, w1 = min(nwg, w0 + per);
  const __bf16* p = reinterpret_cast<const __bf16*>(a.part + (size_t)a.slot[j] * 4096) + item * 16;
  const size_t strideb = a.stride * 2;
  float sum[16];
#pragma unroll
  for (int i = 0; i < 16; ++i) sum[i] = 0.f;
  int wg = w0;
  for (; wg + 4 <= w1; wg += 4) {
    u4v lo[4], hi[4];
#pragma unroll
    for (int u = 0; u < 4; ++u) {
      const u4v* src = reinterpret_cast<const u4v*>(p + (size_t)(wg + u) * strideb);
      lo[u] = src[0]; hi[u] = src[1];
    }
#pragma unroll
    for (int u = 0; u < 4; ++u) {
      const unsigned wds[8] = {lo[u].x, lo[u].y, lo[u].z, lo[u].w, hi[u].x, hi[u].y, hi[u].z, hi[u].w};
#pragma unroll
      for (int i = 0; i < 8; ++i) { sum[2 * i] += __uint_as_float(wds[i] << 16); sum[2 * i + 1] += __uint_as_float(wds[i] & 0xFFFF0000u); }
    }
  }
  for (; wg < w1; ++wg) {
    const u4v* src = reinterpret_cast<const u4v*>(p + (size_t)wg * strideb);
    const u4v lo = src[0], hi = src[1];
    const unsigned wds[8] = {lo.x, lo.y, lo.z, lo.w, hi.x, hi.y, hi.z, hi.w};
#pragma unroll
    for (int i = 0; i < 8; ++i) { sum[2 * i] += __uint_as_float(wds[i] << 16); sum[2 * i + 1] += __uint_as_float(wds[i] & 0xFFFF0000u); }
  }
  const int tile = item >> 4, lane0 = (item & 15) * 4;
#pragma unroll
  for (int r = 0; r < 4; ++r) {
    float* dst = a.G + a.off[j] + (16 * (tile >> 2) + 4 * (lane0 >> 4) + r) * 64 + 16 * (tile & 3) + (lane0 & 15);
#pragma unroll
    for (int k = 0; k < 4; ++k) atomicAdd(dst + k, sum[4 * k + r]);
  }
}

int adt_dwpart_reduce(float* G, const float* part, size_t stride, int nwg, const int* slots, const int* offs, int nslots, void* stream) {
  return adt_dwpart_reduce_n(G, part, stride, nwg, nullptr, slots, offs, nslots, stream);
}
int adt_dwpart_reduce_n(float* G, const float* part, size_t stride, int nwg, const int* nwg_slot, const int* slots, const int* offs, int nslots, void* stream) {
// ... 8 lines not shown
```

### adt_amd/csrc/adt_seq_args.h

```cpp
#pragma once
#include "adt_common.cuh"

namespace adt {

struct SeqFwdArgs {
  int L, B, H;
  const int* ids;
  DropCfg drop;
  uint32_t site_emb, site_attn, site_attn2, site1, site2;
  uint32_t b_offset;
  float ln_eps, scale;
  const float* x;
  const float* E; const float* P; float emb_scale;
  const float* gamma; const float* beta;
  const float* Win; const float* bin;
  const float* Wo; const float* bo;
  const float* gamma2; const float* beta2;
  const float* Ws; const float* bs;
  const float* f;
  const float* Win2; const float* bin2;
  const float* Wo2; const float* bo2;
  const float* W1; const float* b1; const float* W2; const float* b2;
  float* x_out;
  float* xn;
  float* qkv;
  float* o; float* lse; uint32_t* mask;
  float* h;
  float* u;
  float* y;
  float* rec;
  float* a1; float* q2; float* kv2;
  float* o2; float* lse2; uint32_t* mask2;
  float y_scale; int y_acc;
  int saved_bf16;
  const float* wp_base; const void* wp_img;
  unsigned long long* stamps;
  int ablate;
  const float* lnl_gamma; const float* lnl_beta; float* f_out;
  int nsplit;
};

}
```

### adt_amd/csrc/adt_seqbwd_args.h

```cpp
#pragma once
#include "adt_common.cuh"

namespace adt {

struct SeqBwdArgs {
  int L, B, H;
  const int* ids;
  DropCfg drop; uint32_t b_offset;
  float ln_eps, scale;
  const float* x;
  const float* gamma; const float* beta;
  const float* Win; const float* bin;
  const float* dO; const float* o;
  const void* do_bf16; const float* do_delta;
  const float* lse; const uint32_t* mask;
  float dres_scale;
  const float* dres;
  float* gx; int acc;
  const float* seed_other; const float* seed_coef; float* seed_loss; const float* seed_norms;
  float* dWin; float* dbin; float* dgamma; float* dbeta;
  float* part; size_t part_stride;
  int nrep; size_t rep_stride;
  const float* wp_base; const void* wp_img;
  int saved_bf16;
  float* vpart;
  int nsplit;
  unsigned long long* stamps;
};

}
```

### adt_amd/csrc/adt_seqbwd_tt.cuh

```cuda
#pragma once
#include "adt_seqattn.cuh"
#include "adt_seqbwd_args.h"
#include "adt_seqfwd_tt.cuh"
#include "adt_tt.cuh"

namespace adt {

constexpr int SB_NW = 8;
constexpr int SB_R = 224;

template <int H>
struct SeqBwdLds {
  static constexpr size_t wbytes = 6 * (size_t)TT_WIMG * 2, ibytes = (size_t)SB_R * TT_RS * 2;
  static constexpr size_t mbytes = (size_t)H * SB_R * 8 * 4, sbytes = 2 * (size_t)H * SB_R * 4, rbytes = (320 + 320) * 4;
  static constexpr size_t pbytes = ibytes + 64 > wbytes / 2 ? ibytes + 64 : wbytes / 2;
  static constexpr size_t poff = wbytes / 2 + 2 * ibytes + 64  + mbytes + sbytes + rbytes;
  static constexpr size_t bytes = poff + pbytes;
};

template <int HD>
ADT_DEVICE_INLINE void sb_frags(const TT& t, float mul, bf16x8 (&f)[(64 / HD) * ((HD + 31) / 32)]) {
  if constexpr (HD >= 32) {
    f[0] = tt_pack(t.v[0], t.v[1], mul);
    f[1] = tt_pack(t.v[2], t.v[3], mul);
// ... 168 lines not shown
  constexpr int CH = TT_WIMG * 2 / 16;
  const int i1 = threadIdx.x + SB_NW * 64;
#pragma unroll
  for (int k = 0; k < N; ++k) {
    uint4* dst = reinterpret_cast<uint4*>(wimg + k * TT_WIMG);
    dst[threadIdx.x] = t.r0[k];
    if (i1 < CH) dst[i1] = t.r1[k];
  }
}

ADT_DEVICE_INLINE int sb_tile_b(int s, int w, int ntiles) {
  if (ntiles != 13) return tq_tile(s, w, ntiles);
  const int t0 = (0x0 << 0) | (0x1 << 4) | (0x2 << 8) | (0x3 << 12) | (0x7 << 16) | (0x5 << 20) | (0x6 << 24) | (0x4 << 28);
  const int t1 = (0xC << 12) | (0x8 << 16) | (0x9 << 20) | (0xA << 24) | (0xB << 28);
  if (s == 0) return (int)(((unsigned)t0 >> (4 * w)) & 15u);
  return w >= 3 ? (int)(((unsigned)t1 >> (4 * w)) & 15u) : -1;
}

#define SB_STAMP(k) do { if (a.stamps && blockIdx.x == 0 && lane == 0) a.stamps[w * 16 + (k)] = __builtin_amdgcn_s_memtime(); } while (0)

template <int HD, int MODE, bool DEC>
__global__ __launch_bounds__(SB_NW * 64) void k_seqtt_attn_pre_bwd(SeqBwdArgs a) {
  adt_prefetch_kernargs<(sizeof(SeqBwdArgs) + 63) / 64 * 64 <= 512 ? sizeof(SeqBwdArgs) : 512>();
  constexpr int H = 64 / HD, NT = HD / 16, KB = (HD + 31) / 32, NF = H * KB, NW = SB_NW, R = SB_R;
  extern __shared__ __attribute__((aligned(16))) unsigned char smem_raw[];
  typedef SeqBwdLds<H> Lds;
  __bf16* wtr = reinterpret_cast<__bf16*>(smem_raw);
  __bf16* wpl = reinterpret_cast<__bf16*>(smem_raw + Lds::poff);
  __bf16* img2 = wpl;
  __bf16* img0 = reinterpret_cast<__bf16*>(smem_raw + Lds::wbytes / 2);
  __bf16* img1 = reinterpret_cast<__bf16*>(smem_raw + Lds::wbytes / 2 + Lds::ibytes);
  uint32_t* sM = reinterpret_cast<uint32_t*>(smem_raw + Lds::wbytes / 2 + 2 * Lds::ibytes + 64);
  float* sLse = reinterpret_cast<float*>(reinterpret_cast<unsigned char*>(sM) + Lds::mbytes);
  float* sDelta = sLse + H * R;
  float* sRed = sDelta + H * R;
  float* sVec = sRed + 320;
  const float *vgamma = sVec, *vbeta = sVec + 64, *vbin = sVec + 128;
  const int lane = threadIdx.x & 63, w = threadIdx.x >> 6, c = lane & 15, g = lane >> 4;
  const int L = a.L, ntiles = (L + 15) / 16, npair = (L + 31) / 32;
  const bool split = a.nsplit == 2;
  const int b = split ? blockIdx.x >> 1 : blockIdx.x, wpart = split ? (blockIdx.x & 1) : 0;
  auto TM = [&](int s) {
    if (!split) return tq_tile(s, w, ntiles);
    const int t = (s == 0 ? wpart : 1 - wpart) + 2 * w;
    return t < ntiles ? t : -1;
  };
  auto TA = [&](int s) { return (split && s == 1) ? -1 : TM(s); };
  auto TB = [&](int s) { return split ? TA(s) : sb_tile_b(s, w, ntiles); };
  if (a.nrep > 1) {
    const size_t off = (size_t)(blockIdx.x % a.nrep) * a.rep_stride;
    a.dWin += off; a.dbin += off; a.dgamma += off; a.dbeta += off;
  }
  float* const part = a.part ? a.part + (size_t)blockIdx.x * a.part_stride : nullptr;
  SB_STAMP(0);
  constexpr int MI = (H * R * 2 + NW * 64 - 1) / (NW * 64), LI = (H * R + NW * 64 - 1) / (NW * 64);
  tt_u4 mreg[MI];
  float lreg[LI];
  typedef const tt_u4 __attribute__((address_space(1))) * gu4;
  typedef const float __attribute__((address_space(1))) * gf1;
  if constexpr (MODE == 1) {
    adt_static_for<MI>([&](auto k) {
      const int i = threadIdx.x + k * NW * 64, hr = i >> 1, h = hr / R, r = hr - h * R;
      const bool ok = i < H * R * 2 && r < L;
      const gu4 p = ok ? (gu4)(a.mask + ((size_t)(b * H + h) * L + r) * 8) + (i & 1) : (gu4)tt_zero_row;
      mreg[k] = *p;
    });
  }
  adt_static_for<LI>([&](auto k) {
    const int i = threadIdx.x + k * NW * 64, h = i / R, r = i - h * R;
    const bool ok = i < H * R && r < L;
    const float v = *(ok ? (gf1)(a.lse + (size_t)(b * H + h) * L + r) : (gf1)tt_zero_row);
    lreg[k] = ok ? v * 1.4426950408889634f : INFINITY;
  });
  float vreg = 0.f;
  {
    const int t = threadIdx.x;
    const gf1 p = t < 64 ? (gf1)(a.gamma + t) : t < 128 ? (gf1)(a.beta + (t - 64)) : t < 320 ? (gf1)(a.bin + (t - 128)) : (gf1)tt_zero_row;
    vreg = *p;
  }
  const __bf16* wsrc = reinterpret_cast<const __bf16*>(a.wp_img) + 6 * (a.Win - a.wp_base);
  const __bf16* const src6[6] = {wsrc + 2 * WPACK_IMG, wsrc + 6 * 4096 + 2 * WPACK_IMG, wsrc + 12 * 4096 + 2 * WPACK_IMG,
                                 wsrc + 3 * WPACK_IMG, wsrc + 6 * 4096 + 3 * WPACK_IMG, wsrc + 12 * 4096 + 3 * WPACK_IMG};
#pragma unroll
  for (int k = 0; k < 3; ++k) adt_glds_block<NW>(src6[k], wpl + k * TT_WIMG, TT_WIMG * 2);
  TT xa[2], doa[2], oa[2];
  TTRowB dob[2];
  float delta[2][H];
  const bool hand = a.do_bf16 != nullptr;
  int idv[2] = {1, 1};
#pragma unroll
  for (int s = 0; s < 2; ++s) {
    const int tile = TM(s);
    const int l = tile * 16 + c, row = b * L + l;
    xa[s] = tt_load(a.x + (size_t)row * 64, tile >= 0 && l < L, g);
    if (DEC) idv[s] = tt_load_id(a.ids, row, tile >= 0 && l < L);
  }
  SB_STAMP(11);
  {
    uint4* z = reinterpret_cast<uint4*>(img0);
    for (int i = threadIdx.x; i < (int)((2 * Lds::ibytes + 64) / 16); i += NW * 64) z[i] = make_uint4(0u, 0u, 0u, 0u);
    if (threadIdx.x < 320) sRed[threadIdx.x] = 0.f;
    SB_STAMP(12);
    if constexpr (MODE == 1) {
      adt_static_for<MI>([&](auto k) {
        const int i = threadIdx.x + k * NW * 64;
        if (i < H * R * 2) reinterpret_cast<tt_u4*>(sM + (size_t)(i >> 1) * 8)[i & 1] = mreg[k];
      });
    }
    adt_static_for<LI>([&](auto k) {
      const int i = threadIdx.x + k * NW * 64;
      if (i < H * R) { sLse[i] = lreg[k]; sDelta[i] = 0.f; }
    });
    if (threadIdx.x < 320) sVec[threadIdx.x] = vreg;
    SB_STAMP(13);
    adt_wait_vm0();
    SB_STAMP(14);
  }
  __syncthreads();
  SB_STAMP(1);
#pragma unroll
  for (int s = 0; s < 2; ++s) {
    const int tile = TM(s);
    const int l = tile * 16 + c, row = b * L + l;
    const bool valid = tile >= 0 && l < L;
    if (hand) {
      dob[s] = tt_load_bf16_raw(reinterpret_cast<const __bf16*>(a.do_bf16) + (size_t)row * 64, valid, g);
      tt_delta_load<H>(a.do_delta, (size_t)row, valid, delta[s]);
    } else {
      doa[s] = tt_load(a.dO + (size_t)row * 64, valid, g);
      oa[s] = tt_load_saved(a.o, row, valid, g, a.saved_bf16);
    }
  }
#pragma unroll
  for (int k = 3; k < 6; ++k) adt_glds_block<NW>(src6[k], wtr + (k - 3) * TT_WIMG, TT_WIMG * 2);
  const float qmul = a.scale * 1.4426950408889634f;
  const uint32_t key_rng = drop_key(a.drop);
  bf16x8 fq[2][NF], fdo[2][NF];
#pragma unroll
  for (int s = 0; s < 2; ++s) {
    const int tile = TM(s);
    if (tile < 0) continue;
    const int l = tile * 16 + c;
    const bool valid = l < L;
    const TT& x = xa[s];
    const TT xn = tt_ln_apply(tt_ln_stats(x, a.ln_eps).xhat, vgamma, vbeta, g);
    const TTB bn = tt_bfrags(xn);
    TTB bx;
    if (!DEC) bx = tt_bfrags(x);
    TT q = tt_gemm(bn, wpl, c, g);
    tt_add_vec(q, vbin, g);
    sb_frags<HD>(q, qmul, fq[s]);
    TT k = tt_gemm(DEC ? bn : bx, wpl + TT_WIMG, c, g);
    tt_add_vec(k, vbin + 64, g);
    tt_put_rows(img0, l, k, valid, g);
    TT v = tt_gemm(DEC ? bn : bx, wpl + 2 * TT_WIMG, c, g);
    tt_add_vec(v, vbin + 128, g);
    tt_put_rows(img1, l, v, valid, g);
    if (hand) {
      sb_frags_rows<HD>(dob[s], fdo[s]);
    } else {
      sb_frags<HD>(doa[s], a.drop.scale, fdo[s]);
      tt_head_delta<HD>(doa[s], oa[s], delta[s]);
    }
#pragma unroll
    for (int h = 0; h < H; ++h)
      if (g == 0 && valid) sDelta[h * R + l] = delta[s][h];
  }
  __syncthreads();
  SB_STAMP(2);
  {
    uint4* z = reinterpret_cast<uint4*>(img2);
    for (int i = threadIdx.x; i < (int)((Lds::ibytes + 64) / 16); i += NW * 64) z[i] = make_uint4(0u, 0u, 0u, 0u);
  }
  TT dq[2], dk[2], dv[2];
  dq[1] = tt_zero();
#pragma unroll
  for (int s = 0; s < 2; ++s) {
    const int tile = TA(s);
    if (tile < 0) continue;
    const int q = tile * 16 + c;
#pragma unroll
    for (int h = 0; h < H; ++h) {
      f32x4 t[NT];
      const uint32_t bh_rng = (uint32_t)(b * H + h) + a.b_offset * (uint32_t)H;
      sab_pass_a<HD, MODE>(img0, img1, fq[s] + h * KB, fdo[s] + h * KB, sLse[h * R + q], delta[s][h], sM + ((size_t)h * R + q) * 8, tile, h, a.drop,
                           key_rng, (bh_rng * (uint32_t)L + (uint32_t)q) * (uint32_t)L, c, g, t);
#pragma unroll
      for (int nt = 0; nt < NT; ++nt) dq[s].v[h * NT + nt] = t[nt] * a.scale;
    }
  }
  bf16x8 fk[2][NF], fv[2][NF];
#pragma unroll
  for (int s = 0; s < 2; ++s) {
    const int tile = TB(s);
    const int row = (tile >= 0 ? tile : 0) * 16 + c;
#pragma unroll
    for (int h = 0; h < H; ++h)
#pragma unroll
      for (int kb = 0; kb < KB; ++kb) {
        fk[s][h * KB + kb] = sab_rowfrag<HD>(img0, row, h, kb, g);
        fv[s][h * KB + kb] = sab_rowfrag<HD>(img1, row, h, kb, g);
      }
  }
  adt_wait_vm0();
  __syncthreads();
  SB_STAMP(3);
#pragma unroll
  for (int s = 0; s < 2; ++s) {
    const int tile = TM(s);
    if (tile < 0) continue;
    const int l = tile * 16 + c;
    sb_put_frags<HD>(img0, l, fq[s], l < L, g);
    sb_put_frags<HD>(img1, l, fdo[s], l < L, g);
  }
  __syncthreads();
  TT xk[2];
#pragma unroll
  for (int s = 0; s < 2; ++s) {
    if (s == 1) {
#pragma unroll
      for (int s2 = 0; s2 < 2; ++s2) {
        const int tile2 = TM(s2);
        const int l2 = tile2 * 16 + c;
        xk[s2] = tt_load(a.x + (size_t)(b * L + l2) * 64, tile2 >= 0 && l2 < L, g);
      }
    }
    const int tile = TB(s);
    if (tile < 0) continue;
    {
      f32x4 tk[4], tv[4];
      sab_pass_b_heads<HD, MODE>(img0, img1, fk[s], fv[s], sLse, sDelta, sM, R, tile, ntiles, a.drop, key_rng,
                                 (uint32_t)(b * H) + a.b_offset * (uint32_t)H, L, c, g, tk, tv);
#pragma unroll
      for (int i = 0; i < 4; ++i) {
        dk[s].v[i] = tk[i] * 0.6931471805599453f;
        dv[s].v[i] = tv[i];
      }
    }
  }
  __syncthreads();
  SB_STAMP(4);
  {
#pragma unroll
    for (int s = 0; s < 2; ++s) {
      const int tile = TM(s);
      if (tile < 0) continue;
      const int l = tile * 16 + c;
      const bool valid = l < L;
      tt_put_rows(img0, l, dq[s], valid, g);
      tt_put_rows(img1, l, tt_ln_apply(tt_ln_stats(xk[s], a.ln_eps).xhat, vgamma, vbeta, g), valid, g);
    }
#pragma unroll
    for (int s = 0; s < 2; ++s) {
      const int tile = TB(s);
      if (tile < 0) continue;
      const int l = tile * 16 + c;
      tt_put_rows(img2, l, dk[s], l < L, g);
    }
    SB_STAMP(7);
  }
  SB_STAMP(8);
  __syncthreads();
  TT resa[2], gxo[2];
#pragma unroll
  for (int s = 0; s < 2; ++s) {
    const int tile = TA(s);
    const int l = tile * 16 + c;
    resa[s] = tt_load(a.dres + (size_t)(b * L + l) * 64, tile >= 0 && l < L, g);
  }
  sb_dw_product16(img0, img1, npair, a.dWin, part, sRed + 128, w, c, g);
  if (DEC) sb_dw_product16(img2, img1, npair, a.dWin + 4096, part ? part + 4096 : nullptr, sRed + 192, w, c, g);
  SB_STAMP(9);
  __syncthreads();
#pragma unroll
  for (int s = 0; s < 2; ++s) {
    const int tile = TM(s);
    if (tile < 0) continue;
    const int l = tile * 16 + c;
    const bool valid = l < L;
    if (!DEC) tt_put_rows(img1, l, xk[s], valid, g);
  }
#pragma unroll
  for (int s = 0; s < 2; ++s) {
    const int tile = TB(s);
    if (tile < 0) continue;
    const int l = tile * 16 + c;
    tt_put_rows(img0, l, dv[s], l < L, g);
  }
  __syncthreads();
  if (!DEC) sb_dw_product16(img2, img1, npair, a.dWin + 4096, part ? part + 4096 : nullptr, sRed + 192, w, c, g);
  sb_dw_product16(img0, img1, npair, a.dWin + 8192, part ? part + 8192 : nullptr, sRed + 256, w, c, g);
  SB_STAMP(5);
  TT dgm = tt_zero(), dbt = tt_zero();
  auto gx_request = [&](int s) {
    const int tile = TA(s);
    const int l = tile * 16 + c;
    const float* const src = a.seed_other ? a.seed_other : a.gx;
    gxo[s] = tt_load(src + (size_t)(b * L + l) * 64, (a.acc || a.seed_other) && tile >= 0 && l < L, g);
  };
  const float seed_coef = a.seed_other ? *a.seed_coef : 0.f;
  float seed_sq = 0.f;
  gx_request(0);
#pragma unroll
  for (int s = 0; s < 2; ++s) {
    const int tile = TA(s);
    if (tile < 0) continue;
    const int l = tile * 16 + c, row = b * L + l;
    const bool valid = l < L;
    if (s == 0) gx_request(1);
    const TTLn st = tt_ln_stats(xk[s], a.ln_eps);
    TT dn = tt_gemm(tt_bfrags(dq[s]), wtr, c, g);
    TTB bdk, bdv;
    bdk.kb[0] = sab_rowfrag<32>(img2, l, 0, 0, g); bdk.kb[1] = sab_rowfrag<32>(img2, l, 1, 0, g);
    bdv.kb[0] = sab_rowfrag<32>(img0, l, 0, 0, g); bdv.kb[1] = sab_rowfrag<32>(img0, l, 1, 0, g);
    TT dkv = tt_gemm(bdk, wtr + TT_WIMG, c, g);
    tt_add(dkv, tt_gemm(bdv, wtr + 2 * TT_WIMG, c, g));
    TT res = resa[s];
    if (DEC && (!valid || idv[s] == 0)) res = tt_zero();
    if (DEC && a.dres_scale != 0.f) {
#pragma unroll
      for (int nt = 0; nt < 4; ++nt) res.v[nt] *= a.dres_scale;
// ... 65 lines not shown
```

### adt_amd/csrc/adt_seqfwd_tt.cuh

```cuda
#pragma once
#include "adt_seq_args.h"
#include "adt_tt.cuh"

namespace adt {

#define TQ_STAMP(k) do { if (a.stamps && blockIdx.x == 0 && lane == 0) a.stamps[w * 16 + (k)] = __builtin_amdgcn_s_memtime(); } while (0)

constexpr int TQ_NW = 8;
constexpr int TQ_FWD_NW = 12;
constexpr int TQ_MAXKT = 14;
constexpr int TQ_LP = TQ_MAXKT * 16;

template <int NWT>
struct SeqTtLds {
  static constexpr size_t wbytes = (size_t)NWT * TT_WIMG * 2, ibytes = (size_t)TQ_LP * TT_RS * 2;
  static constexpr size_t vbytes = 1152 * sizeof(float);
  static constexpr size_t bytes = wbytes + 2 * ibytes + vbytes;
  __bf16* w[NWT]; __bf16* sK; __bf16* sV; float* vec;
  __device__ SeqTtLds(unsigned char* base) {
    __bf16* pw = reinterpret_cast<__bf16*>(base);
    for (int i = 0; i < NWT; ++i) w[i] = pw + i * TT_WIMG;
    sK = reinterpret_cast<__bf16*>(base + wbytes);
    sV = reinterpret_cast<__bf16*>(base + wbytes + ibytes);
    vec = reinterpret_cast<float*>(base + wbytes + 2 * ibytes);
// ... 44 lines not shown

ADT_DEVICE_INLINE void tq_store_y(const SeqFwdArgs& a, size_t row, TT y, bool valid, int g) {
  float* dst = a.y + row * 64;
  if (a.y_scale != 0.f) {
#pragma unroll
    for (int nt = 0; nt < 4; ++nt) y.v[nt] *= a.y_scale;
    if (a.y_acc) tt_add(y, tt_load(dst, valid, g));
  }
  tt_store(dst, y, valid, g);
}

ADT_DEVICE_INLINE int tq_tile(int s, int w, int ntiles, int nw = TQ_NW) {
  if (s == 0) return ntiles - 1 - w;
  const int t = ntiles - 2 * nw + w;
  return t >= 0 ? t : -1;
}
ADT_DEVICE_INLINE int tq_tile12(int s, int w, int ntiles) {
  if (ntiles == 13) {
    const int t13 = (0xC << 0) | (0xB << 4) | (0xA << 8) | (0x3 << 12) | (0x9 << 16) | (0x8 << 20) | (0x7 << 24) | (0x6 << 28);
    const int t13b = (0x1 << 0) | (0x2 << 4) | (0x5 << 8) | (0x4 << 12);
    if (s == 0) return w < 8 ? (int)(((unsigned)t13 >> (4 * w)) & 15u) : ((t13b >> (4 * (w - 8))) & 15);
    return w == 3 ? 0 : -1;
  }
  const int cl = w & 3, k = s == 0 ? (w >> 2) : ((w >> 2) == 2 ? 3 : 4);
  const int j = 4 * k + ((k & 1) ? 3 - cl : cl);
  return (k < 4 && j < ntiles) ? ntiles - 1 - j : -1;
}

constexpr int TQ_HELPER_WAVE = 0;
ADT_DEVICE_INLINE int tq_helper_tile(int w, int ntiles) { return (ntiles == 13 && w == TQ_HELPER_WAVE) ? 0 : -1; }
ADT_DEVICE_INLINE bool tq_split_second(int ntiles) { return ntiles == 13; }

template <int NTHREADS>
ADT_DEVICE_INLINE void tq_stage(__bf16* img, const float* W, bool transposed, const SeqFwdArgs& a) {
  const uint4* src = reinterpret_cast<const uint4*>(reinterpret_cast<const __bf16*>(a.wp_img) + 6 * (W - a.wp_base) + (transposed ? 3 : 2) * WPACK_IMG);
  uint4* dst = reinterpret_cast<uint4*>(img);
  for (int i = threadIdx.x; i < TT_WIMG * 2 / 16; i += NTHREADS) dst[i] = src[i];
}

ADT_DEVICE_INLINE const uint4* tq_img_src(const SeqFwdArgs& a, const float* W, bool transposed) {
  return reinterpret_cast<const uint4*>(reinterpret_cast<const __bf16*>(a.wp_img) + 6 * (W - a.wp_base) + (transposed ? 3 : 2) * WPACK_IMG);
}
constexpr int TQ_CH = TT_WIMG * 2 / 16;
#define TQ_IMG_LOAD(k, Wk) const uint4* tqp##k = tq_img_src(a, Wk, false); const uint4 tqr##k = tqp##k[tq_body ? threadIdx.x : 0]; \
  const uint4 tqt##k = tqp##k[tq_tail ? threadIdx.x + TQW * 64 : 0];
#define TQ_IMG_STORE(k, dstk) if (tq_body) reinterpret_cast<uint4*>(dstk)[threadIdx.x] = tqr##k; if (tq_tail) reinterpret_cast<uint4*>(dstk)[threadIdx.x + TQW * 64] = tqt##k;

template <int NTHREADS>
ADT_DEVICE_INLINE void tq_zero(__bf16* p, size_t nbytes) {
  uint4* q = reinterpret_cast<uint4*>(p);
  for (int i = threadIdx.x; i < (int)(nbytes / 16); i += NTHREADS) q[i] = make_uint4(0u, 0u, 0u, 0u);
}

struct TqX { TT e; TT p; int id; };
ADT_DEVICE_INLINE TqX tq_x_request(const SeqFwdArgs& a, int row, int l, bool valid, int id, int g) {
  TqX r;
  r.id = id;
  if (a.x) {
    r.e = tt_load(a.x + (size_t)row * 64, valid, g);
    r.p = tt_zero();
  } else {
    r.e = tt_load(a.E + (size_t)id * 64, valid, g);
    r.p = tt_load(a.P + (size_t)l * 64, valid, g);
  }
  return r;
}
ADT_DEVICE_INLINE TT tq_x_finish(const SeqFwdArgs& a, const TqX& r, int row, bool valid, uint32_t key0, int g) {
  if (a.x) return r.e;
  TT x = tt_zero();
  if (r.id != 0) {
#pragma unroll
    for (int nt = 0; nt < 4; ++nt)
#pragma unroll
      for (int e = 0; e < 4; ++e) x.v[nt][e] = r.e.v[nt][e] * a.emb_scale + r.p.v[nt][e];
    tt_dropout(x, key0, a.drop, (uint32_t)row + a.b_offset * (uint32_t)a.L, g);
  }
  if (a.x_out) tt_store(a.x_out + (size_t)row * 64, x, valid, g);
  return x;
}

template <int HD, bool ENC, int PART = 0>
ADT_DEVICE_INLINE void tq_pre_tile(const SeqFwdArgs& a, const float* vec, const __bf16* wq, const __bf16* wk, const __bf16* wv, __bf16* sK, __bf16* sV,
                                   int tile, int b, uint32_t key0, float qmul, int c, int g,
                                   bf16x8 (&fq)[(64 / HD) * ((HD + 31) / 32)], TT& xn_out, const TqX& xr) {
  const int l = tile * 16 + c, row = b * a.L + l;
  const bool valid = l < a.L;
  TT x;
  if (PART == 1) {
    SeqFwdArgs a1 = a;
    a1.x_out = nullptr;
    x = tq_x_finish(a1, xr, row, valid, key0, g);
  } else {
    x = tq_x_finish(a, xr, row, valid, key0, g);
  }
  const TT xn = tt_layernorm(x, vec + SV_GAMMA, vec + SV_BETA, a.ln_eps, g);
  if (PART != 1 && a.xn) tt_store(a.xn + (size_t)row * 64, xn, valid, g);
  if (PART != 1) xn_out = xn;
  const TTB bn = tt_bfrags(xn);
  TTB bx;
  if (ENC) bx = tt_bfrags(x);
  if (PART != 1) {
    TT q = tt_gemm(bn, wq, c, g);
    tt_add_vec(q, vec + SV_BIN, g);
    if (a.qkv && valid) {
#pragma unroll
      for (int nt = 0; nt < 4; ++nt) *reinterpret_cast<float4*>(a.qkv + (size_t)row * 192 + 16 * nt + 4 * g) = make_float4(q.v[nt][0], q.v[nt][1], q.v[nt][2], q.v[nt][3]);
    }
    tt_qfrags<HD>(q, qmul, fq);
  }
  if (PART == 2) return;
  {
    TT k = tt_gemm(ENC ? bx : bn, wk, c, g);
    tt_add_vec(k, vec + SV_BIN + 64, g);
    if (a.qkv && valid) {
#pragma unroll
      for (int nt = 0; nt < 4; ++nt) *reinterpret_cast<float4*>(a.qkv + (size_t)row * 192 + 64 + 16 * nt + 4 * g) = make_float4(k.v[nt][0], k.v[nt][1], k.v[nt][2], k.v[nt][3]);
    }
    tt_put_slot(sK, l, k, valid, g);
  }
  {
    TT v = tt_gemm(ENC ? bx : bn, wv, c, g);
    tt_add_vec(v, vec + SV_BIN + 128, g);
    if (a.qkv && valid) {
#pragma unroll
      for (int nt = 0; nt < 4; ++nt) *reinterpret_cast<float4*>(a.qkv + (size_t)row * 192 + 128 + 16 * nt + 4 * g) = make_float4(v.v[nt][0], v.v[nt][1], v.v[nt][2], v.v[nt][3]);
    }
    tt_put_rows(sV, l, v, valid, g);
  }
}

ADT_DEVICE_INLINE TT tq_ffn(const SeqFwdArgs& a, const float* vec, const __bf16* w1, const __bf16* w2, const TT& xin, uint32_t key1, uint32_t key2, int row,
                            bool valid, int c, int g) {
  const uint32_t rg = (uint32_t)row + a.b_offset * (uint32_t)a.L;
  TT u = tt_gemm(tt_bfrags(xin), w1, c, g);
  tt_add_vec(u, vec + SV_B1, g);
  tt_dropout(u, key1, a.drop, rg, g);
#pragma unroll
  for (int nt = 0; nt < 4; ++nt)
#pragma unroll
    for (int r = 0; r < 4; ++r) u.v[nt][r] = fmaxf(u.v[nt][r], 0.f);
  tt_save(a.u, row, u, valid, g, a.saved_bf16);
  TT y = tt_gemm(tt_bfrags(u), w2, c, g);
  tt_add_vec(y, vec + SV_B2, g);
  tt_dropout(y, key2, a.drop, rg, g);
  return y;
}

template <int HD>
__global__ __launch_bounds__(TQ_FWD_NW * 64) void k_seqtt_enc_fwd(SeqFwdArgs a) {
  constexpr int TQW = TQ_FWD_NW;
  adt_prefetch_kernargs<(sizeof(SeqFwdArgs) + 63) / 64 * 64 <= 512 ? sizeof(SeqFwdArgs) : 512>();
  constexpr int H = 64 / HD, KB = (HD + 31) / 32, NF = H * KB;
  extern __shared__ __attribute__((aligned(16))) unsigned char smem_raw[];
  const int lane = threadIdx.x & 63, w = threadIdx.x >> 6, c = lane & 15, g = lane >> 4;
  SeqTtLds<6> lds(smem_raw);
  const int nsp = a.nsplit > 1 ? a.nsplit : 1, b = blockIdx.x / nsp, part = blockIdx.x % nsp;
  const int L = a.L, ntiles = (L + 15) / 16;
  const bool own[2] = {tq_tile12(0, w, ntiles) >= 0 && tq_tile12(0, w, ntiles) % nsp == part, tq_tile12(1, w, ntiles) >= 0 && tq_tile12(1, w, ntiles) % nsp == part};
  TQ_STAMP(0);
  uint32_t seedv = 0u;
  TqX xr[2];
  const int htile = tq_helper_tile(w, ntiles);
  const bool split2 = tq_split_second(ntiles);
  int idm[2] = {0, 0};
  {
    int idr[2] = {0, 0};
    if (!a.x) {
#pragma unroll
      for (int s = 0; s < 2; ++s) {
        const int tile = tq_tile12(s, w, ntiles), l = tile * 16 + c;
        idm[s] = tt_load_id(a.ids, b * L + l, tile >= 0 && l < L);
        idr[s] = idm[s];
      }
      if (htile >= 0) idr[1] = tt_load_id(a.ids, b * L + htile * 16 + c, htile * 16 + c < L);
    }
    const bool tq_body = TQW * 64 <= TQ_CH || threadIdx.x < TQ_CH;
    const bool tq_tail = (int)threadIdx.x < TQ_CH - TQW * 64;
    TQ_IMG_LOAD(0, a.Win) TQ_IMG_LOAD(1, a.Win + 4096) TQ_IMG_LOAD(2, a.Win + 8192)
    const TqVecRegs vr = tq_vec_load<TQW * 64>(a, H, HD);
    if (a.drop.thr) seedv = *a.drop.seed;
#pragma unroll
    for (int s = 0; s < 2; ++s) {
      const int tile = (s == 1 && htile >= 0) ? htile : tq_tile12(s, w, ntiles), l = tile * 16 + c;
      xr[s] = tq_x_request(a, b * L + l, l, tile >= 0 && l < L, idr[s], g);
    }
    if (a.x) {
#pragma unroll
      for (int s = 0; s < 2; ++s) {
        const int tile = tq_tile12(s, w, ntiles), l = tile * 16 + c;
        idm[s] = tt_load_id(a.ids, b * L + l, tile >= 0 && l < L);
      }
    }
    TQ_STAMP(11);
    tq_zero<TQW * 64>(lds.sK, 2 * SeqTtLds<6>::ibytes);
    TQ_STAMP(12);
    TQ_IMG_STORE(0, lds.w[0]) TQ_IMG_STORE(1, lds.w[1]) TQ_IMG_STORE(2, lds.w[2])
    TQ_STAMP(13);
    tq_vec_store<TQW * 64>(lds.vec, vr);
    TQ_STAMP(14);
  }
  __syncthreads();
  TQ_STAMP(1);
  adt_glds_block<TQW>(tq_img_src(a, a.Wo, false), lds.w[3], TT_WIMG * 2);
  adt_glds_block<TQW>(tq_img_src(a, a.W1, false), lds.w[4], TT_WIMG * 2);
  adt_glds_block<TQW>(tq_img_src(a, a.W2, false), lds.w[5], TT_WIMG * 2);
  const uint32_t key0 = adt_site_key(seedv, a.site_emb), key1 = adt_site_key(seedv, a.site1), key2 = adt_site_key(seedv, a.site2);
  const float qmul = a.scale * 1.4426950408889634f;
  bf16x8 fq[2][NF];
  TT xn[2];
  {
    const int tile = tq_tile12(0, w, ntiles);
    if (tile >= 0 && own[0]) tq_pre_tile<HD, true>(a, lds.vec, lds.w[0], lds.w[1], lds.w[2], lds.sK, lds.sV, tile, b, key0, qmul, c, g, fq[0], xn[0], xr[0]);
    else if (tile >= 0) tq_pre_tile<HD, true, 1>(a, lds.vec, lds.w[0], lds.w[1], lds.w[2], lds.sK, lds.sV, tile, b, key0, qmul, c, g, fq[0], xn[0], xr[0]);
    TQ_STAMP(2);
    const int tile1 = tq_tile12(1, w, ntiles);
    if (htile >= 0) tq_pre_tile<HD, true, 1>(a, lds.vec, lds.w[0], lds.w[1], lds.w[2], lds.sK, lds.sV, htile, b, key0, qmul, c, g, fq[1], xn[1], xr[1]);
    else if (tile1 >= 0 && !split2 && own[1]) tq_pre_tile<HD, true>(a, lds.vec, lds.w[0], lds.w[1], lds.w[2], lds.sK, lds.sV, tile1, b, key0, qmul, c, g, fq[1], xn[1], xr[1]);
    else if (tile1 >= 0 && !split2) tq_pre_tile<HD, true, 1>(a, lds.vec, lds.w[0], lds.w[1], lds.w[2], lds.sK, lds.sV, tile1, b, key0, qmul, c, g, fq[1], xn[1], xr[1]);
    TQ_STAMP(3);
  }
  adt_wait_vm0();
  __syncthreads();
  TQ_STAMP(4);
  {
    const int tile1 = tq_tile12(1, w, ntiles);
    if (split2 && tile1 >= 0 && own[1]) tq_pre_tile<HD, true, 2>(a, lds.vec, lds.w[0], lds.w[1], lds.w[2], lds.sK, lds.sV, tile1, b, key0, qmul, c, g, fq[1], xn[1], xr[1]);
  }
#pragma unroll
  for (int s = 0; s < 2; ++s) {
    const int tile = tq_tile12(s, w, ntiles);
    if (tile < 0 || !own[s]) continue;
    const int l = tile * 16 + c, row = b * L + l;
    const bool valid = l < L;
    const TT o = tt_attn_heads<HD, TQ_MAXKT>(lds.sK, lds.sV, fq[s], tile, L, b, a.b_offset, a.drop, a.site_attn, seedv, a.lse, a.mask, lane, c, g);
    TQ_STAMP(5 + 3 * s);
    tt_save(a.o, row, o, valid, g, a.saved_bf16);
    if (a.rec) {
      constexpr int NT = HD / 16;
#pragma unroll
      for (int h = 0; h < H; ++h) {
        float z[H];
#pragma unroll
        for (int cc = 0; cc < H; ++cc) {
          float acc = 0.f;
#pragma unroll
          for (int nt = 0; nt < NT; ++nt) {
            const float4 ws = *reinterpret_cast<const float4*>(lds.vec + SV_WS + cc * HD + 16 * nt + 4 * g);
            const f32x4& ov = o.v[h * NT + nt];
            acc += ov[0] * ws.x + ov[1] * ws.y + ov[2] * ws.z + ov[3] * ws.w;
          }
          z[cc] = tt_colsum(acc) + lds.vec[SV_BS + cc];
        }
        float m = z[0];
#pragma unroll
        for (int cc = 1; cc < H; ++cc) m = fmaxf(m, z[cc]);
        float se = 0.f;
#pragma unroll
        for (int cc = 0; cc < H; ++cc) se += __expf(z[cc] - m);
        const float lz = m + __logf(se);
        if (g == 0 && valid) {
          float* dst = a.rec + ((size_t)(l * a.B + b) * H + h) * H;
#pragma unroll
          for (int cc = 0; cc < H; ++cc) dst[cc] = z[cc] - lz;
        }
      }
    }
    TT hh = tt_gemm(tt_bfrags(o), lds.w[3], c, g);
    tt_add_vec(hh, lds.vec + SV_BO, g);
    tt_add(hh, xn[s]);
    TQ_STAMP(6 + 3 * s);
    tt_save(a.h, row, hh, valid, g, a.saved_bf16);
    const TT h2 = tt_layernorm(hh, lds.vec + SV_GAMMA2, lds.vec + SV_BETA2, a.ln_eps, g);
    TT y = tq_ffn(a, lds.vec, lds.w[4], lds.w[5], h2, key1, key2, row, valid, c, g);
    tt_add(y, h2);
    if (!valid || idm[s] == 0) y = tt_zero();
    tq_store_y(a, row, y, valid, g);
    if (a.f_out) tt_store(a.f_out + (size_t)row * 64, tt_layernorm(y, lds.vec + SV_LNL_G, lds.vec + SV_LNL_B, a.ln_eps, g), valid, g);
    TQ_STAMP(7 + 3 * s);
  }
}

template <int HD>
__global__ __launch_bounds__(TQ_FWD_NW * 64) void k_seqtt_dec_fwd(SeqFwdArgs a) {
  constexpr int TQW = TQ_FWD_NW;
  adt_prefetch_kernargs<(sizeof(SeqFwdArgs) + 63) / 64 * 64 <= 512 ? sizeof(SeqFwdArgs) : 512>();
  constexpr int H = 64 / HD, KB = (HD + 31) / 32, NF = H * KB;
  extern __shared__ __attribute__((aligned(16))) unsigned char smem_raw[];
  const int lane = threadIdx.x & 63, w = threadIdx.x >> 6, c = lane & 15, g = lane >> 4;
  SeqTtLds<5> lds(smem_raw);
  const int nsp = a.nsplit > 1 ? a.nsplit : 1, b = blockIdx.x / nsp, part = blockIdx.x % nsp;
  const int L = a.L, ntiles = (L + 15) / 16;
  const bool own[2] = {tq_tile12(0, w, ntiles) >= 0 && tq_tile12(0, w, ntiles) % nsp == part, tq_tile12(1, w, ntiles) >= 0 && tq_tile12(1, w, ntiles) % nsp == part};
  uint32_t seedv = 0u;
  const bool tq_body = TQW * 64 <= TQ_CH || threadIdx.x < TQ_CH;
  const bool tq_tail = (int)threadIdx.x < TQ_CH - TQW * 64;
  TqX xr[2];
  const int htile = tq_helper_tile(w, ntiles);
  const bool split2 = tq_split_second(ntiles);
  int idm[2] = {0, 0};
  {
    int idr[2] = {0, 0};
    if (!a.x) {
#pragma unroll
      for (int s = 0; s < 2; ++s) {
        const int tile = tq_tile12(s, w, ntiles), l = tile * 16 + c;
        idm[s] = tt_load_id(a.ids, b * L + l, tile >= 0 && l < L);
        idr[s] = idm[s];
      }
      if (htile >= 0) idr[1] = tt_load_id(a.ids, b * L + htile * 16 + c, htile * 16 + c < L);
    }
    TQ_IMG_LOAD(0, a.Win) TQ_IMG_LOAD(1, a.Win + 4096) TQ_IMG_LOAD(2, a.Win + 8192)
    const TqVecRegs vr = tq_vec_load<TQW * 64>(a, H, HD);
    if (a.drop.thr) seedv = *a.drop.seed;
#pragma unroll
    for (int s = 0; s < 2; ++s) {
      const int tile = (s == 1 && htile >= 0) ? htile : tq_tile12(s, w, ntiles), l = tile * 16 + c;
      xr[s] = tq_x_request(a, b * L + l, l, tile >= 0 && l < L, idr[s], g);
    }
    if (a.x) {
#pragma unroll
      for (int s = 0; s < 2; ++s) {
        const int tile = tq_tile12(s, w, ntiles), l = tile * 16 + c;
        idm[s] = tt_load_id(a.ids, b * L + l, tile >= 0 && l < L);
      }
    }
    tq_zero<TQW * 64>(lds.sK, 2 * SeqTtLds<5>::ibytes);
    TQ_IMG_STORE(0, lds.w[0]) TQ_IMG_STORE(1, lds.w[1]) TQ_IMG_STORE(2, lds.w[2])
    tq_vec_store<TQW * 64>(lds.vec, vr);
  }
  __syncthreads();
  adt_glds_block<TQW>(tq_img_src(a, a.Wo, false), lds.w[3], TT_WIMG * 2);
  adt_glds_block<TQW>(tq_img_src(a, a.Win2, false), lds.w[4], TT_WIMG * 2);
  const uint32_t key0 = adt_site_key(seedv, a.site_emb), key1 = adt_site_key(seedv, a.site1), key2 = adt_site_key(seedv, a.site2);
  const float qmul = a.scale * 1.4426950408889634f;
  bf16x8 fq[2][NF];
  TT dn[2];
  {
    const int tile = tq_tile12(0, w, ntiles), tile1 = tq_tile12(1, w, ntiles);
    if (tile >= 0 && own[0]) tq_pre_tile<HD, false>(a, lds.vec, lds.w[0], lds.w[1], lds.w[2], lds.sK, lds.sV, tile, b, key0, qmul, c, g, fq[0], dn[0], xr[0]);
    else if (tile >= 0) tq_pre_tile<HD, false, 1>(a, lds.vec, lds.w[0], lds.w[1], lds.w[2], lds.sK, lds.sV, tile, b, key0, qmul, c, g, fq[0], dn[0], xr[0]);
    if (htile >= 0) tq_pre_tile<HD, false, 1>(a, lds.vec, lds.w[0], lds.w[1], lds.w[2], lds.sK, lds.sV, htile, b, key0, qmul, c, g, fq[1], dn[1], xr[1]);
    else if (tile1 >= 0 && !split2 && own[1]) tq_pre_tile<HD, false>(a, lds.vec, lds.w[0], lds.w[1], lds.w[2], lds.sK, lds.sV, tile1, b, key0, qmul, c, g, fq[1], dn[1], xr[1]);
    else if (tile1 >= 0 && !split2) tq_pre_tile<HD, false, 1>(a, lds.vec, lds.w[0], lds.w[1], lds.w[2], lds.sK, lds.sV, tile1, b, key0, qmul, c, g, fq[1], dn[1], xr[1]);
  }
  adt_wait_vm0();
  __syncthreads();
  {
    const int tile1 = tq_tile12(1, w, ntiles);
    if (split2 && tile1 >= 0 && own[1]) tq_pre_tile<HD, false, 2>(a, lds.vec, lds.w[0], lds.w[1], lds.w[2], lds.sK, lds.sV, tile1, b, key0, qmul, c, g, fq[1], dn[1], xr[1]);
  }
#pragma unroll
  for (int s = 0; s < 2; ++s) {
    const int tile = tq_tile12(s, w, ntiles);
    if (tile < 0 || !own[s]) continue;
    const int l = tile * 16 + c, row = b * L + l;
    const bool valid = l < L;
    const TT o1 = tt_attn_heads<HD, TQ_MAXKT>(lds.sK, lds.sV, fq[s], tile, L, b, a.b_offset, a.drop, a.site_attn, seedv, a.lse, a.mask, lane, c, g);
    tt_save(a.o, row, o1, valid, g, a.saved_bf16);
    TT a1 = tt_gemm(tt_bfrags(o1), lds.w[3], c, g);
    tt_add_vec(a1, lds.vec + SV_BO, g);
    tt_save(a.a1, row, a1, valid, g, a.saved_bf16);
    TT q2 = tt_gemm(tt_bfrags(a1), lds.w[4], c, g);
    tt_add_vec(q2, lds.vec + SV_BIN2, g);
    tt_save(a.q2, row, q2, valid, g, a.saved_bf16);
    tt_qfrags<HD>(q2, qmul, fq[s]);
  }
  TQ_IMG_LOAD(5, a.Win2 + 4096) TQ_IMG_LOAD(6, a.Win2 + 8192) TQ_IMG_LOAD(7, a.Wo2) TQ_IMG_LOAD(8, a.W1) TQ_IMG_LOAD(9, a.W2)
  TT fa[2];
#pragma unroll
  for (int s = 0; s < 2; ++s) {
// ... 55 lines not shown
```

### adt_amd/csrc/adt_seqpost_tt.cuh

```cuda
#pragma once
#include "adt_bwdchain_args.h"
#include "adt_seqbwd_tt.cuh"

namespace adt {

template <int NWT>
struct SeqPostLds {
  static constexpr size_t wbytes = (size_t)NWT * TT_WIMG * 2, ibytes = (size_t)SB_R * TT_RS * 2;
  static constexpr size_t rbytes = (448 + 256) * 4;
  static constexpr int wvrow = 384;
  static constexpr size_t wvbytes = 8 * wvrow * 4;
  static constexpr size_t bytes = wbytes + 2 * ibytes + 64 + rbytes + wvbytes;
};

ADT_DEVICE_INLINE void sp_replica(BwdChainArgs& a) {
  if (a.nrep <= 1) return;
  const size_t off = (size_t)(blockIdx.x % a.nrep) * a.rep_stride;
  float** const ptrs[] = {&a.dW0, &a.dW1, &a.dW2, &a.dW3, &a.db0, &a.db1, &a.db2, &a.db3, &a.dgamma, &a.dbeta, &a.dWs, &a.dbs, &a.lnl_dgamma, &a.lnl_dbeta};
#pragma unroll
  for (int i = 0; i < 14; ++i)
    if (*ptrs[i]) *ptrs[i] += off;
}

template <int N, int NW>
ADT_DEVICE_INLINE void sp_wdma(const BwdChainArgs& a, const float* const (&W)[N], __bf16* wimg) {
#pragma unroll
  for (int j = 0; j < N; ++j)
    adt_glds_block<NW>(reinterpret_cast<const __bf16*>(a.wp_img) + 6 * (W[j] - a.wp_base) + 3 * WPACK_IMG, wimg + j * TT_WIMG, TT_WIMG * 2);
}
template <int NW>
ADT_DEVICE_INLINE void sp_zero_images(__bf16* img0) {
  constexpr size_t ibytes = (size_t)SB_R * TT_RS * 2;
  uint4* z = reinterpret_cast<uint4*>(img0);
  for (int i = threadIdx.x; i < (int)((2 * ibytes + 64) / 16); i += NW * 64) z[i] = make_uint4(0u, 0u, 0u, 0u);
}
template <int HD, bool CHUNKS = false>
ADT_DEVICE_INLINE void sp_hand_do(void* do_bf16, float* do_delta, float scale, size_t row, const TT& dO, const TT& o, bool valid, int g) {
  float dl[64 / HD];
  if constexpr (CHUNKS) tt_head_delta_chunks<HD>(dO, o, dl);
  else tt_head_delta<HD>(dO, o, dl);
  tt_store_bf16(reinterpret_cast<__bf16*>(do_bf16) + row * 64, dO, valid, g, scale);
  tt_delta_store<64 / HD>(do_delta, row, dl, valid, g, CHUNKS ? 1 : 0);
}
ADT_DEVICE_INLINE void sp_store_do1(float* out0, void* do_bf16, float* do_delta, float scale, int hd, size_t row, const TT& dO, const TT& o, bool valid, int g) {
  if (!do_bf16) { tt_store(out0 + row * 64, dO, valid, g); return; }
  if (hd == 32) sp_hand_do<32>(do_bf16, do_delta, scale, row, dO, o, valid, g);
  else if (hd == 64) sp_hand_do<64>(do_bf16, do_delta, scale, row, dO, o, valid, g);
  else sp_hand_do<16>(do_bf16, do_delta, scale, row, dO, o, valid, g);
}
constexpr int SP_NW = 8;
constexpr int SP_NS = (14 + SP_NW - 1) / SP_NW;

template <int HD, bool ENC>
__global__ __launch_bounds__(SP_NW * 64) void k_seqtt_post_bwd(BwdChainArgs a) {
  adt_prefetch_kernargs<(sizeof(BwdChainArgs) + 63) / 64 * 64 <= 512 ? sizeof(BwdChainArgs) : 512>();
  constexpr int H = 64 / HD, NT = HD / 16, NW = SP_NW, NS = SP_NS;
  typedef SeqPostLds<3> Lds;
  extern __shared__ __attribute__((aligned(16))) unsigned char smem_raw[];
  __bf16* wimg = reinterpret_cast<__bf16*>(smem_raw);
  __bf16* img0 = reinterpret_cast<__bf16*>(smem_raw + Lds::wbytes);
  __bf16* img1 = reinterpret_cast<__bf16*>(smem_raw + Lds::wbytes + Lds::ibytes);
  float* sRed = reinterpret_cast<float*>(smem_raw + Lds::wbytes + 2 * Lds::ibytes + 64);
  float* sVec = sRed + 448;
  float* sWave = sVec + 256;
  constexpr int WVR = Lds::wvrow;
  const float *vgamma = sVec, *vbeta = sVec + 64, *vws = sVec + 128, *vgl = sVec + 192;
  const bool lnl = ENC && a.lnl_x != nullptr;
  const int lane = threadIdx.x & 63, w = threadIdx.x >> 6, c = lane & 15, g = lane >> 4;
  const int nsp = a.nsplit > 1 ? a.nsplit : 1, b = blockIdx.x / nsp, part = blockIdx.x % nsp;
  const int L = a.L, ntiles = (L + 15) / 16, npair = (L + 31) / 32;
  auto tileof = [&](int s) { const int t = tq_tile(s, w, ntiles, NW); return (t >= 0 && t % nsp == part) ? t : -1; };
  const bool cls = ENC && H > 1 && a.drec != nullptr;
  sp_replica(a);
  SB_STAMP(0);
  const float* const ws3[3] = {a.W0, a.W1, a.W2};
  sp_wdma<3, NW>(a, ws3, wimg);
  TT dy[NS], xl[NS];
  TTSaved uraw[NS], hreq[NS];
  int idv[NS];
#pragma unroll
  for (int s = 0; s < NS; ++s) {
    const int tile = tileof(s);
    const int l = tile * 16 + c, row = b * L + l;
    const bool valid = tile >= 0 && l < L;
    dy[s] = tt_load(a.gy + (size_t)row * 64, valid, g);
    if (ENC) xl[s] = tt_load(a.lnl_x + (size_t)row * 64, valid && lnl, g);
    uraw[s] = tt_saved_request(a.u, row, valid, g, a.saved_bf16);
    hreq[s] = tt_saved_request(a.xin, row, valid, g, a.saved_bf16);
    idv[s] = tt_load_id(a.ids, row, valid);
  }
  if (a.gy_scale != 0.f) {
#pragma unroll
    for (int s = 0; s < NS; ++s)
#pragma unroll
      for (int nt = 0; nt < 4; ++nt) dy[s].v[nt] *= a.gy_scale;
  }
  {
    sp_zero_images<NW>(img0);
    if (threadIdx.x < 448) sRed[threadIdx.x] = 0.f;
    if (ENC) { tt_stage_vec<NW * 64>(sVec, a.gamma, 64); tt_stage_vec<NW * 64>(sVec + 64, a.beta, 64); }
    if (cls) tt_stage_vec<NW * 64>(sVec + 128, a.Ws, 64);
    if (lnl) tt_stage_vec<NW * 64>(sVec + 192, a.lnl_gamma, 64);
    adt_wait_vm0();
  }
  const uint32_t seedv = a.drop.thr ? *a.drop.seed : 0u;
  const uint32_t key1 = adt_site_key(seedv, a.site1), key2 = adt_site_key(seedv, a.site2);
  SB_STAMP(1);
  __syncthreads();
  SB_STAMP(2);
  TT dt[NS];
  if (ENC) {
    if (lnl) {
      TT dgl = tt_zero(), dbl = tt_zero();
#pragma unroll
      for (int s = 0; s < NS; ++s) {
        if (tileof(s) < 0) continue;
        dy[s] = tt_ln_bwd(dy[s], tt_ln_stats(xl[s], a.lnl_eps), vgl, dgl, dbl, g);
      }
      float* mine = sWave + w * WVR + 256;
#pragma unroll
      for (int nt = 0; nt < 4; ++nt)
#pragma unroll
        for (int r = 0; r < 4; ++r) {
          const float sg = tt_rowsum16(dgl.v[nt][r]), sb = tt_rowsum16(dbl.v[nt][r]);
          if (c == 0) { mine[16 * nt + 4 * g + r] = sg; mine[64 + 16 * nt + 4 * g + r] = sb; }
        }
    }
  }
#pragma unroll
  for (int s = 0; s < NS; ++s) {
    const int tile = tileof(s);
    if (tile < 0) continue;
    const int l = tile * 16 + c, row = b * L + l;
    const bool valid = l < L;
    const TT u = tt_saved_value(uraw[s], a.saved_bf16);
    if (a.stamps) { asm volatile("s_waitcnt vmcnt(0)" ::: "memory"); if (s == 0) SB_STAMP(3); }
    if (idv[s] == 0) dy[s] = tt_zero();
    TT gyv = dy[s];
    tt_dropout(gyv, key2, a.drop, (uint32_t)row + a.row_offset, g);
    tt_put_rows(img0, l, gyv, valid, g);
    tt_put_rows(img1, l, u, valid, g);
    TT t = tt_gemm(tt_bfrags(gyv), wimg, c, g);
#pragma unroll
    for (int nt = 0; nt < 4; ++nt)
#pragma unroll
      for (int r = 0; r < 4; ++r)
        if (!(u.v[nt][r] > 0.f)) t.v[nt][r] = 0.f;
    tt_dropout(t, key1, a.drop, (uint32_t)row + a.row_offset, g);
    dt[s] = t;
    if (s == 0) SB_STAMP(4);
  }
  SB_STAMP(5);
  __syncthreads();
  SB_STAMP(6);
  sb_dw_product16<NW>(img0, img1, npair, a.dW0, a.part[0] ? a.part[0] + (size_t)blockIdx.x * a.part_stride : nullptr, sRed + 256, w, c, g);
  SB_STAMP(7);
  __syncthreads();
  SB_STAMP(8);
  TT dh[NS];
  TTSaved oreq[NS];
  f32x4 drq[NS], rcq[NS];
#pragma unroll
  for (int s = 0; s < NS; ++s) drq[s] = rcq[s] = f32x4{0.f, 0.f, 0.f, 0.f};
  TT dgm = tt_zero(), dbt = tt_zero();
#pragma unroll
  for (int s = 0; s < NS; ++s) {
    const int tile = tileof(s);
    if (tile < 0) continue;
    const int l = tile * 16 + c, row = b * L + l;
    const bool valid = l < L;
    oreq[s] = tt_saved_request(a.o, row, valid, g, a.saved_bf16);
    if constexpr (H == 2) {
      if (cls) {
        typedef const f32x4 __attribute__((address_space(1))) * gf4;
        const size_t off = (size_t)(l * a.B + b) * (H * H);
        drq[s] = *(valid ? (gf4)(a.drec + off) : (gf4)tt_zero_row);
        rcq[s] = *(valid ? (gf4)(a.rec + off) : (gf4)tt_zero_row);
      }
    }
    const TT hraw_s = tt_saved_value(hreq[s], a.saved_bf16);
    tt_put_rows(img0, l, dt[s], valid, g);
    TT d = tt_gemm(tt_bfrags(dt[s]), wimg + TT_WIMG, c, g);
    tt_add(d, dy[s]);
    if (ENC) {
      const TTLn st = tt_ln_stats(hraw_s, a.ln_eps);
      tt_put_rows(img1, l, tt_ln_apply(st.xhat, vgamma, vbeta, g), valid, g);
      dh[s] = tt_ln_bwd(d, st, vgamma, dgm, dbt, g);
      tt_store(a.out0 + (size_t)row * 64, dh[s], valid, g);
    } else {
      tt_put_rows(img1, l, hraw_s, valid, g);
      dh[s] = d;
    }
  }
  SB_STAMP(9);
  __syncthreads();
  sb_dw_product16<NW>(img0, img1, npair, a.dW1, a.part[1] ? a.part[1] + (size_t)blockIdx.x * a.part_stride : nullptr, sRed + 320, w, c, g);
  SB_STAMP(10);
  __syncthreads();
  SB_STAMP(11);
  float dws[H][NT][4], dbs_acc[H];
#pragma unroll
  for (int cc = 0; cc < H; ++cc) {
    dbs_acc[cc] = 0.f;
#pragma unroll
    for (int nt = 0; nt < NT; ++nt)
#pragma unroll
      for (int r = 0; r < 4; ++r) dws[cc][nt][r] = 0.f;
  }
#pragma unroll
  for (int s = 0; s < NS; ++s) {
    const int tile = tileof(s);
    if (tile < 0) continue;
    const int l = tile * 16 + c, row = b * L + l;
    const bool valid = l < L;
    const TT oraw_s = tt_saved_value(oreq[s], a.saved_bf16);
    tt_put_rows(img0, l, dh[s], valid, g);
    tt_put_rows(img1, l, oraw_s, valid, g);
    TT dO = tt_gemm(tt_bfrags(dh[s]), wimg + 2 * TT_WIMG, c, g);
    if (cls) {
      const size_t off = (size_t)(l * a.B + b) * (H * H);
#pragma unroll
      for (int h = 0; h < H; ++h) {
        float dz[H], rcv[H], sd = 0.f;
        if constexpr (H == 2) {
// ... 206 lines not shown
```

### adt_amd/csrc/adt_seqxattn_tt.cuh

```cuda
#pragma once
#include "adt_seqattn.cuh"
#include "adt_seqpost_tt.cuh"

namespace adt {

constexpr int XM_NW = 16;

struct XattnMidArgs {
  const __bf16* Q; const __bf16* K; const __bf16* V; const __bf16* O; int ldq, ldk, ldv, ldo;
  const float* LSE; const float* dO; int lddo; int L;
  const uint32_t* mask; float scale; DropCfg drop;
  const float* xin; const float* o; const float* f; const float* wp_base; const void* wp_img;
  const float* W0; const float* W1; const float* W2; const float* W3;
  float* out0; float* out1; int acc1; int nrep; size_t rep_stride;
  float* db0; float* db1; float* db2; float* db3; float* vpart;
  float* part[4]; size_t part_stride;
  void* do_bf16; float* do_delta; float do_scale;
  const __bf16* dO_bf16; const float* dO_delta;
  unsigned long long* stamps;
};

__host__ __device__ inline int xm_rows(int L) { return (L + 31) / 32 <= 4 ? 128 : SB_R; }
__host__ __device__ inline size_t xm_lds_bytes(int L, int H) {
  const size_t R = (size_t)xm_rows(L);
  return 4 * R * TT_RS * 2 + (size_t)H * R * 8 * 4 + 2 * (size_t)H * R * 4 + 256 * 4;
}

ADT_DEVICE_INLINE TTB xm_zero() {
  TTB t;
#pragma unroll
  for (int kb = 0; kb < 2; ++kb)
#pragma unroll
    for (int j = 0; j < 8; ++j) t.kb[kb][j] = (__bf16)0.f;
  return t;
}
ADT_DEVICE_INLINE void xm_put_rows(__bf16* img, int token, const TTB& t) {
#pragma unroll
  for (int nt = 0; nt < 4; ++nt) {
    bf16x4 v;
#pragma unroll
    for (int r = 0; r < 4; ++r) v[r] = t.kb[nt >> 1][4 * (nt & 1) + r];
    *reinterpret_cast<bf16x4*>(img + token * TT_RS + 16 * nt + 4 * (int)((threadIdx.x & 63) >> 4)) = v;
  }
}

template <int HD, int MODE>
__global__ __launch_bounds__(XM_NW * 64) void k_seqtt_xattn_mid_bwd(XattnMidArgs a) {
  static_assert(sizeof(XattnMidArgs) <= 512, "kernel-argument prefetch covers 512 bytes");
  static_assert(MODE == 0 || MODE == 1, "no dropout, or keep bits saved by the forward");
  adt_prefetch_kernargs<sizeof(XattnMidArgs)>();
  constexpr int H = 64 / HD, NT = HD / 16, KB = (HD + 31) / 32, NF = H * KB, NW = XM_NW;
  extern __shared__ __attribute__((aligned(16))) unsigned char smem_raw[];
  const int L = a.L, R = xm_rows(L);
  __bf16* sK = reinterpret_cast<__bf16*>(smem_raw);
  __bf16* sV = sK + R * TT_RS;
  __bf16* sQ = sV + R * TT_RS;
  __bf16* sdO = sQ + R * TT_RS;
  uint32_t* sM = reinterpret_cast<uint32_t*>(sdO + R * TT_RS);
  float* sLse = reinterpret_cast<float*>(sM + (size_t)H * R * 8);
  float* sDelta = sLse + H * R;
  float* sRed = sDelta + H * R;
  __bf16* wimg = sK;
  __bf16* img0 = sQ;
  __bf16* img1 = sdO;
  const int b = blockIdx.x;
  const int lane = threadIdx.x & 63, w = threadIdx.x >> 6, c = lane & 15, g = lane >> 4;
  const size_t row_b = (size_t)b * L;
  const float qmul = a.scale * 1.4426950408889634f;
  const int nqt = (L + 15) / 16, npair = (L + 31) / 32;
#define XM_STAMP(k) do { if (a.stamps && blockIdx.x == 0 && lane == 0) a.stamps[w * 16 + (k)] = __builtin_amdgcn_s_memtime(); } while (0)
  XM_STAMP(0);
  if (a.nrep > 1) {
    const size_t off = (size_t)(blockIdx.x % a.nrep) * a.rep_stride;
    if (a.db0) a.db0 += off;
    if (a.db1) a.db1 += off;
    if (a.db2) a.db2 += off;
    if (a.db3) a.db3 += off;
  }
  constexpr int NTH = NW * 64;
  constexpr int MI = (H * SB_R * 2 + NTH - 1) / NTH, LI = (H * SB_R + NTH - 1) / NTH, II = (SB_R * 8 + NTH - 1) / NTH;
  typedef const tt_u4 __attribute__((address_space(1))) * gu4;
  typedef const float __attribute__((address_space(1))) * gf1;
  typedef const bf16x4 __attribute__((address_space(1))) * gb4;
  typedef const f32x4 __attribute__((address_space(1))) * gp4;
  tt_u4 mreg[MI];
  float lreg[LI];
  if constexpr (MODE == 1) {
    adt_static_for<MI>([&](auto k) {
      const int i = threadIdx.x + k * NTH, hr = i >> 1, h = hr / R, r = hr - h * R;
      const bool ok = i < H * R * 2 && r < L;
      const gu4 p = ok ? (gu4)(a.mask + ((size_t)(b * H + h) * L + r) * 8) + (i & 1) : (gu4)tt_zero_row;
      mreg[k] = *p;
    });
  }
  adt_static_for<LI>([&](auto k) {
    const int i = threadIdx.x + k * NTH, h = i / R, r = i - h * R;
    const bool ok = i < H * R && r < L;
    const float v = *(ok ? (gf1)(a.LSE + (size_t)(b * H + h) * L + r) : (gf1)tt_zero_row);
    lreg[k] = ok ? v * 1.4426950408889634f : INFINITY;
  });
  bf16x4 qa[II], qc[II], ka[II], kc[II], va[II], vc[II], oa[II], oc[II], da[II], dc[II];
  f32x4 d0[II], d1[II];
  float dlt[II];
  const bool hand = a.dO_bf16 != nullptr;
  adt_static_for<II>([&](auto k) {
    const int i = threadIdx.x + k * NTH, r = i >> 3, c8 = (i & 7) * 8;
    const bool ok = r < L;
    const int pa = 16 * ((c8 >> 2) & 3) + 4 * (c8 >> 4);
    const size_t row = row_b + r;
    const gb4 zb = (gb4)tt_zero_row + (i & 7);
    const gb4 pq = ok ? (gb4)(a.Q + row * a.ldq + pa) : zb, pk = ok ? (gb4)(a.K + row * a.ldk + pa) : zb;
    const gb4 pv = ok ? (gb4)(a.V + row * a.ldv + pa) : zb, po = ok ? (gb4)(a.O + row * a.ldo + pa) : zb;
    qa[k] = pq[0]; qc[k] = pq[4]; ka[k] = pk[0]; kc[k] = pk[4]; va[k] = pv[0]; vc[k] = pv[4];
    if (hand) {
      const gb4 pdb = ok ? (gb4)(a.dO_bf16 + row * 64 + pa) : zb;
      da[k] = pdb[0]; dc[k] = pdb[4];
      dlt[k] = *(ok ? (gf1)(a.dO_delta + row * 4 + (i & 7) / (HD / 8)) : (gf1)tt_zero_row);
    } else {
      const gp4 pd = ok ? (gp4)(a.dO + row * a.lddo + c8) : (gp4)tt_zero_row + (i & 7);
      oa[k] = po[0]; oc[k] = po[4];
      d0[k] = pd[0]; d1[k] = pd[1];
    }
  });
  XM_STAMP(1);
  if constexpr (MODE == 1) {
    adt_static_for<MI>([&](auto k) {
      const int i = threadIdx.x + k * NTH;
      if (i < H * R * 2) reinterpret_cast<tt_u4*>(sM + (size_t)(i >> 1) * 8)[i & 1] = mreg[k];
    });
  }
  adt_static_for<LI>([&](auto k) {
    const int i = threadIdx.x + k * NTH;
    if (i < H * R) sLse[i] = lreg[k];
  });
  if (threadIdx.x < 256) sRed[threadIdx.x] = 0.f;
  adt_static_for<II>([&](auto k) {
    const int i = threadIdx.x + k * NTH, r = i >> 3, c8 = (i & 7) * 8;
    float q[8], kk[8], v[8];
#pragma unroll
    for (int j = 0; j < 4; ++j) {
      q[j] = (float)qa[k][j]; q[4 + j] = (float)qc[k][j]; kk[j] = (float)ka[k][j]; kk[4 + j] = (float)kc[k][j];
      v[j] = (float)va[k][j]; v[4 + j] = (float)vc[k][j];
    }
#pragma unroll
    for (int j = 0; j < 8; ++j) q[j] *= qmul;
    const bool in = i < R * 8;
    if (in) {
      *reinterpret_cast<bf16x8*>(sQ + r * TT_RS + c8) = pack8(q);
      *reinterpret_cast<bf16x8*>(sK + r * TT_RS + c8) = pack8(kk);
      *reinterpret_cast<bf16x8*>(sV + r * TT_RS + c8) = pack8(v);
    }
    float part;
    if (hand) {
      bf16x8 db;
#pragma unroll
      for (int j = 0; j < 4; ++j) { db[j] = da[k][j]; db[4 + j] = dc[k][j]; }
      if (in) *reinterpret_cast<bf16x8*>(sdO + r * TT_RS + c8) = db;
      part = dlt[k];
    } else {
      float d[8], o[8];
#pragma unroll
      for (int j = 0; j < 4; ++j) { o[j] = (float)oa[k][j]; o[4 + j] = (float)oc[k][j]; d[j] = d0[k][j]; d[4 + j] = d1[k][j]; }
      part = tt_chunk_delta(d, o);
#pragma unroll
      for (int j = 0; j < 8; ++j) d[j] *= a.drop.scale;
      if (in) *reinterpret_cast<bf16x8*>(sdO + r * TT_RS + c8) = pack8(d);
#pragma unroll
      for (int off = HD / 16; off > 0; off >>= 1) part += __shfl_xor(part, off, 64);
    }
    if (in && ((i & 7) % (HD / 8)) == 0) sDelta[((i & 7) / (HD / 8)) * R + r] = part;
  });
  XM_STAMP(2);
  __syncthreads();
  XM_STAMP(3);
  const uint32_t key_rng = 0u;
  const float ln2 = 0.6931471805599453f;
  const int rk = sab_rank16(w);
  const bool has = rk < nqt;
  const int qt = has ? nqt - 1 - rk : 0, kt = has ? rk : 0;
  const int lA = qt * 16 + c, lB = kt * 16 + c;
  const bool validA = has && lA < L, validB = has && lB < L;
  const size_t rowA = row_b + lA, rowB = row_b + lB;

  TTB dq = xm_zero();
  bf16x4 fkl[NF], fkh[NF], fvl[NF], fvh[NF];
  if (has) {
#pragma unroll
    for (int h = 0; h < H; ++h) {
      const float lse_q = sLse[h * R + lA], delta_q = sDelta[h * R + lA];
      bf16x8 fq[KB], fdo[KB];
#pragma unroll
      for (int kb = 0; kb < KB; ++kb) {
        fq[kb] = sab_rowfrag<HD>(sQ, lA, h, kb, g);
        fdo[kb] = sab_rowfrag<HD>(sdO, lA, h, kb, g);
      }
      f32x4 t[NT];
      sab_pass_a<HD, MODE>(sK, sV, fq, fdo, lse_q, delta_q, sM + ((size_t)h * R + lA) * 8, qt, h, a.drop, key_rng, 0u, c, g, t);
#pragma unroll
      for (int nt = 0; nt < NT; ++nt)
#pragma unroll
        for (int r = 0; r < 4; ++r) dq.kb[(h * NT + nt) >> 1][4 * ((h * NT + nt) & 1) + r] = (__bf16)(validA ? t[nt][r] * a.scale : 0.f);
    }
#pragma unroll
    for (int h = 0; h < H; ++h)
#pragma unroll
      for (int kb = 0; kb < KB; ++kb) {
        const bf16x8 k8 = sab_rowfrag<HD>(sK, lB, h, kb, g), v8 = sab_rowfrag<HD>(sV, lB, h, kb, g);
#pragma unroll
        for (int j = 0; j < 4; ++j) { fkl[h * KB + kb][j] = k8[j]; fkh[h * KB + kb][j] = k8[4 + j]; fvl[h * KB + kb][j] = v8[j]; fvh[h * KB + kb][j] = v8[4 + j]; }
      }
  }
  XM_STAMP(4);
  __syncthreads();
  XM_STAMP(5);
  {
    const float* const ws4[4] = {a.W0, a.W1, a.W2, a.W3};
#pragma unroll
    for (int j = 0; j < 4; ++j)
      adt_glds_block<NW>(reinterpret_cast<const __bf16*>(a.wp_img) + 6 * (ws4[j] - a.wp_base) + 3 * WPACK_IMG, wimg + j * TT_WIMG, TT_WIMG * 2);
  }
  TTSaved a1req;
  if constexpr (HD != 16) a1req = tt_saved_request(a.xin, rowA, validA, g, 1);

  TTB dk = xm_zero(), dv = xm_zero();
  if (has) {
#pragma unroll
    for (int h = 0; h < H; ++h) {
      f32x4 tk[NT], tv[NT];
      bf16x8 fk[KB], fv[KB];
#pragma unroll
      for (int kb = 0; kb < KB; ++kb)
#pragma unroll
        for (int j = 0; j < 4; ++j) {
          fk[kb][j] = fkl[h * KB + kb][j]; fk[kb][4 + j] = HD == 16 ? (__bf16)0.f : fkh[h * KB + kb][j];
          fv[kb][j] = fvl[h * KB + kb][j]; fv[kb][4 + j] = HD == 16 ? (__bf16)0.f : fvh[h * KB + kb][j];
        }
      sab_pass_b<HD, MODE>(sQ, sdO, fk, fv, sLse + h * R, sDelta + h * R, sM + (size_t)h * R * 8, kt, nqt, h, a.drop, key_rng, 0u, L,
                           c, g, tk, tv);
#pragma unroll
      for (int nt = 0; nt < NT; ++nt)
#pragma unroll
        for (int r = 0; r < 4; ++r) {
          dk.kb[(h * NT + nt) >> 1][4 * ((h * NT + nt) & 1) + r] = (__bf16)(validB ? tk[nt][r] * ln2 : 0.f);
          dv.kb[(h * NT + nt) >> 1][4 * ((h * NT + nt) & 1) + r] = (__bf16)(validB ? tv[nt][r] : 0.f);
        }
    }
  }
  if constexpr (HD == 16) a1req = tt_saved_request(a.xin, rowA, validA, g, 1);
  XM_STAMP(6);
  adt_wait_vm0();
  __syncthreads();
  XM_STAMP(7);
  TT da1 = tt_zero();
  const TTSaved oreq = tt_saved_request(a.o, rowA, validA, g, 1);
  const TT fx = tt_load(a.f + rowB * 64, validB, g);
  if (has) {
    xm_put_rows(img0, lA, dq);
    tt_put_rows(img1, lA, tt_saved_value(a1req, 1), validA, g);
    da1 = tt_gemm(dq, wimg, c, g);
  }
  __syncthreads();
  sb_dw_product16<NW>(img0, img1, npair, nullptr, a.part[0] + (size_t)blockIdx.x * a.part_stride, sRed, w, c, g);
  __syncthreads();
  XM_STAMP(8);
  const TT acc1v = tt_load(a.out1 + rowB * 64, validB && a.acc1, g);
  if (has) {
    tt_put_rows(img0, lA, da1, validA, g);
    const TT o1 = tt_saved_value(oreq, 1);
    tt_put_rows(img1, lA, o1, validA, g);
    sp_store_do1(a.out0, a.do_bf16, a.do_delta, a.do_scale, HD, rowA, tt_gemm(tt_bfrags(da1), wimg + TT_WIMG, c, g), o1, validA, g);
  }
  __syncthreads();
  sb_dw_product16<NW>(img0, img1, npair, nullptr, a.part[1] + (size_t)blockIdx.x * a.part_stride, sRed + 64, w, c, g);
  __syncthreads();
  XM_STAMP(9);
  TT df = tt_zero();
  if (has) {
    xm_put_rows(img0, lB, dk);
    tt_put_rows(img1, lB, fx, validB, g);
    df = tt_gemm(dk, wimg + 2 * TT_WIMG, c, g);
  }
  __syncthreads();
  sb_dw_product16<NW>(img0, img1, npair, nullptr, a.part[2] + (size_t)blockIdx.x * a.part_stride, sRed + 128, w, c, g);
  __syncthreads();
  XM_STAMP(10);
  if (has) {
    xm_put_rows(img0, lB, dv);
    tt_add(df, tt_gemm(dv, wimg + 3 * TT_WIMG, c, g));
    tt_add(df, acc1v);
    tt_store(a.out1 + rowB * 64, df, validB, g);
  }
  __syncthreads();
  sb_dw_product16<NW>(img0, img1, npair, nullptr, a.part[3] + (size_t)blockIdx.x * a.part_stride, sRed + 192, w, c, g);
  __syncthreads();
  XM_STAMP(11);
  {
    const int t = threadIdx.x;
    float* const dst[4] = {a.db0, a.db1, a.db2, a.db3};
    if (t < 256) {
      if (a.vpart) a.vpart[(size_t)blockIdx.x * 512 + t] = sRed[t];
      else atomicAdd(dst[t >> 6] + (t & 63), sRed[t]);
    }
  }
  XM_STAMP(12);
#undef XM_STAMP
}

// ... 2 lines not shown
```

### adt_amd/csrc/adt_step_plan.h

```cpp
#pragma once
#include <stddef.h>
#include <stdio.h>
#include "../../include/adt_hip.h"
#include "adt_bwd_plan.h"
#include "adt_wide_plan.h"

constexpr int ADT_SEQ_MAXLEN = 224;

struct SeqSwitches {
  bool seq = true;
  bool seq_lean = true;
  bool seq_tt = true;
  bool seq_bwd = true;
  bool seq_attn_bwd = true;
  bool seq_post_bwd = true;
  bool seq_partials = true;
  bool xattn_fused = true;
  int seq_ablate = 0;
  bool seq_ablate_set = false;
  int seq_split = 0;
  bool attn_split = true;
  int side_stream = 7;
  bool side_stream_dp = false;
  bool item_sort = false;
  bool lnl_fused = true;
  bool fold_parts = true;
  bool fwd_fused = true;
  bool embed3 = true;
  bool bce_merged = true;
  bool do_bf16{true};
};

constexpr bool adt_seq_head_ok(int hd) { return hd == 16 || hd == 32 || hd == 64; }

struct SeqAttnFacts {
  int L, H, B;
  bool causal, in_bf16, out_bf16;
  int ldq, ldk, ldv, ldo, lddo;
  bool dropout, keep_bits;
  size_t sab_lds, xm_lds;
};
struct SeqChainFacts {
  int L, H, B, T;
  bool wimg;
  bool saved_bf16, grad_bf16, parts4;
  int nsplit, ablate;
  bool drec;
};

static inline bool adt_covers_attn_bwd(const SeqSwitches& sw, int hd, const SeqAttnFacts& a) {
  if (!sw.seq_attn_bwd || !a.causal || a.H * hd != 64 || a.L > ADT_SEQ_MAXLEN) return false;
  if ((a.ldq % 4) || (a.ldk % 4) || (a.ldv % 4) || (a.ldo % 4)) return false;
  if (a.in_bf16 && ((a.ldq % 8) || (a.ldk % 8) || (a.ldv % 8) || (a.ldo % 8))) return false;
  return a.sab_lds <= ADT_LDS_MAX && adt_seq_head_ok(hd);
}
static inline bool adt_covers_attn_pre_bwd(const SeqSwitches& sw, int hd, const SeqChainFacts& a) {
  return sw.seq_bwd && a.wimg && a.L <= ADT_SEQ_MAXLEN && (a.L & 3) == 0 && a.H * hd == 64 && adt_seq_head_ok(hd);
}
static inline bool adt_covers_mid_bwd(const SeqSwitches& sw, int hd, const SeqChainFacts& a) {
  return sw.seq_post_bwd && a.wimg && a.L <= ADT_SEQ_MAXLEN && a.T == a.B * a.L && adt_seq_head_ok(hd);
}
static inline bool adt_covers_post_bwd(const SeqSwitches& sw, int hd, bool enc, const SeqChainFacts& a) {
  return adt_covers_mid_bwd(sw, hd, a) && !(enc && a.drec && a.H * hd != 64);
}
static inline bool adt_covers_xattn_mid(const SeqSwitches& sw, int hd, const SeqAttnFacts& at, const SeqChainFacts& ch, bool handover) {
  if (!sw.xattn_fused || !adt_covers_mid_bwd(sw, hd, ch)) return false;
  if (!at.in_bf16 || !at.out_bf16 || !ch.saved_bf16 || !ch.grad_bf16 || !ch.parts4) return false;
  if (ch.nsplit > 1 || ch.ablate) return false;
  if (!at.causal || at.H * hd != 64 || (at.L & 3) || at.L > ADT_SEQ_MAXLEN || at.L != ch.L || at.B != ch.B) return false;
  if (at.dropout && !at.keep_bits) return false;
  if ((at.ldq % 8) || (at.ldk % 8) || (at.ldv % 8) || (at.ldo % 8) || (at.lddo % 4)) return false;
  return handover && at.xm_lds <= ADT_LDS_MAX;
}
static inline bool adt_seq_fwd_tt(const SeqSwitches& sw, bool wimg, int L) { return sw.seq_tt && wimg && (L & 3) == 0; }

struct StepFacts {
  int prec, L, d, H, num_layers, B;
  int rows;
  bool item_sort_ok;
  size_t sab_lds;
};

struct StepPlan {
  char cfg_error[96];
  bool use_seq;
  bool lean;
  bool parts;
  bool fold_parts;
  bool parts_area, sort_area;
  bool det;
  bool embed3_on;
  bool lnl_fused;
  bool bce_deferred;
  bool bce_merged;
  int seq_split;
  int attn_split;
  int side_sites;
  bool side_dp;
  bool loss_one_launch;
  bool do_handover;
};

static inline StepPlan adt_step_plan(const StepFacts& f, const SeqSwitches& sw) {
  StepPlan p{};
  const int nl = f.num_layers;
  const int hd = (f.H >= 1 && f.d % f.H == 0) ? f.d / f.H : 0;
  if (f.d != 64) snprintf(p.cfg_error, sizeof p.cfg_error, "sasrec: hidden=%d unsupported in this build (64)", f.d);
  else if (hd == 0) snprintf(p.cfg_error, sizeof p.cfg_error, "sasrec: bad num_heads");
  else if (!adt_seq_head_ok(hd)) snprintf(p.cfg_error, sizeof p.cfg_error, "sasrec: head_dim=%d unsupported (16/32/64)", hd);
  else if (f.L > ADT_SEQ_MAXLEN) snprintf(p.cfg_error, sizeof p.cfg_error, "sasrec: maxlen=%d > %d unsupported", f.L, ADT_SEQ_MAXLEN);
  else if (nl < 1 || nl > 16) snprintf(p.cfg_error, sizeof p.cfg_error, "sasrec: num_layers");

  const bool bf16 = f.prec == ADT_PREC_BF16;
  p.use_seq = sw.seq && bf16 && f.d == 64 && f.L <= ADT_SEQ_MAXLEN && adt_seq_head_ok(hd);
  p.lean = sw.seq_lean && sw.seq_tt && sw.seq_bwd && sw.seq_attn_bwd && !sw.seq_ablate_set && p.use_seq && (f.L & 3) == 0 &&
           f.sab_lds <= ADT_LDS_MAX;
  p.parts = sw.seq_partials && sw.seq_post_bwd && p.lean;
  p.fold_parts = sw.fold_parts && nl <= 2 && p.parts;
  p.parts_area = bf16 && f.d == 64;
  p.sort_area = f.d == 64 && f.item_sort_ok;
  p.det = sw.item_sort && p.sort_area;
  p.embed3_on = sw.embed3 && !p.det && f.d == 64;
  p.lnl_fused = p.parts && sw.lnl_fused;
  p.bce_deferred = sw.fwd_fused && f.d == 64 && nl <= 4 && p.lean;
  p.bce_merged = sw.bce_merged;
  p.seq_split = 1;
  if (sw.seq_split > 0) p.seq_split = sw.seq_split;
  else while (p.seq_split < 8 && f.B * p.seq_split * 2 <= 256) p.seq_split *= 2;
  p.attn_split = sw.attn_split && p.seq_split >= 2 ? 2 : 1;
  p.side_sites = sw.side_stream & 7;
  p.side_dp = sw.side_stream_dp;
  p.loss_one_launch = nl <= 4;
  p.do_handover = sw.do_bf16 && p.parts;
  return p;
}

struct BwdCallPlan {
  bool late_parts;
  bool embed3;
  bool side;
};
static inline BwdCallPlan adt_bwd_call_plan(const StepPlan& s, const BwdPlan& b) {
  BwdCallPlan p;
  p.late_parts = b.defer_fold && s.fold_parts;
  p.embed3 = b.seeds_virtual && s.embed3_on;
  p.side = s.side_sites != 0 && (b.phase == 0 || s.side_dp);
  return p;
}
```

### adt_amd/csrc/adt_tt.cuh

```cuda
#pragma once
#include "adt_attn_bf16.cuh"
#include "adt_wave.cuh"

namespace adt {

struct TT { f32x4 v[4]; };

constexpr int TT_RS = 72;
constexpr int TT_WIMG = 64 * TT_RS;

ADT_DEVICE_INLINE bf16x8 tt_pack(const f32x4& lo, const f32x4& hi, float mul = 1.0f) {
  bf16x8 o;
#pragma unroll
  for (int j = 0; j < 4; ++j) { o[j] = (__bf16)(lo[j] * mul); o[4 + j] = (__bf16)(hi[j] * mul); }
  return o;
}

struct TTB { bf16x8 kb[2]; };

ADT_DEVICE_INLINE TTB tt_bfrags(const TT& x, float mul = 1.0f) {
  TTB b;
  b.kb[0] = tt_pack(x.v[0], x.v[1], mul);
  b.kb[1] = tt_pack(x.v[2], x.v[3], mul);
  return b;
// ... 6 lines not shown
  TT y;
#pragma unroll
  for (int nt = 0; nt < 4; ++nt) {
    f32x4 acc = {0.f, 0.f, 0.f, 0.f};
#pragma unroll
    for (int kb = 0; kb < 2; ++kb)
      acc = mfma_bf16(acc, *reinterpret_cast<const bf16x8*>(img + (16 * nt + c) * TT_RS + 32 * kb + 8 * g), b.kb[kb]);
    y.v[nt] = acc;
  }
  return y;
}

struct TTV { f32x4 v[4]; };
ADT_DEVICE_INLINE TTV tt_vec(const float* p, int g) {
  TTV t;
#pragma unroll
  for (int nt = 0; nt < 4; ++nt) {
    const float4 x = *reinterpret_cast<const float4*>(p + 16 * nt + 4 * g);
    t.v[nt] = f32x4{x.x, x.y, x.z, x.w};
  }
  return t;
}
ADT_DEVICE_INLINE void tt_add_vec(TT& t, const float* p, int g) {
#pragma unroll
  for (int nt = 0; nt < 4; ++nt) {
    const float4 x = *reinterpret_cast<const float4*>(p + 16 * nt + 4 * g);
    t.v[nt] += f32x4{x.x, x.y, x.z, x.w};
  }
}
ADT_DEVICE_INLINE void tt_add(TT& a, const TT& b) {
#pragma unroll
  for (int nt = 0; nt < 4; ++nt) a.v[nt] += b.v[nt];
}
ADT_DEVICE_INLINE TT tt_zero() {
  TT t;
#pragma unroll
  for (int nt = 0; nt < 4; ++nt) t.v[nt] = f32x4{0.f, 0.f, 0.f, 0.f};
  return t;
}

static __device__ __attribute__((aligned(256))) const float tt_zero_row[64] = {};
ADT_DEVICE_INLINE int tt_load_id(const int* ids, int row, bool valid) {
  typedef const int __attribute__((address_space(1))) * gi;
  return *(valid ? (gi)(ids + row) : (gi)tt_zero_row);
}
ADT_DEVICE_INLINE TT tt_load(const float* row, bool valid, int g) {
  TT t;
  typedef const f32x4 __attribute__((address_space(1))) * gp4;
  const gp4 p = valid ? (gp4)(row + 4 * g) : (gp4)(tt_zero_row + 4 * g);
#pragma unroll
  for (int nt = 0; nt < 4; ++nt) t.v[nt] = p[4 * nt];
  return t;
}
ADT_DEVICE_INLINE TT tt_load_if(const float* row, bool valid, int g) {
  TT t;
#pragma unroll
  for (int nt = 0; nt < 4; ++nt) {
    float4 x = make_float4(0.f, 0.f, 0.f, 0.f);
    if (valid) x = *reinterpret_cast<const float4*>(row + 16 * nt + 4 * g);
    t.v[nt] = f32x4{x.x, x.y, x.z, x.w};
  }
  return t;
}
ADT_DEVICE_INLINE void tt_store(float* row, const TT& t, bool valid, int g) {
  if (!valid) return;
#pragma unroll
  for (int nt = 0; nt < 4; ++nt) *reinterpret_cast<float4*>(row + 16 * nt + 4 * g) = make_float4(t.v[nt][0], t.v[nt][1], t.v[nt][2], t.v[nt][3]);
}

ADT_DEVICE_INLINE void tt_store_bf16(__bf16* row, const TT& t, bool valid, int g, float mul = 1.0f) {
  if (!valid) return;
  *reinterpret_cast<bf16x8*>(row + 16 * g) = tt_pack(t.v[0], t.v[1], mul);
  *reinterpret_cast<bf16x8*>(row + 16 * g + 8) = tt_pack(t.v[2], t.v[3], mul);
}
ADT_DEVICE_INLINE TT tt_load_bf16(const __bf16* row, bool valid, int g) {
  TT t;
  typedef const bf16x8 __attribute__((address_space(1))) * gp8;
  const gp8 p = valid ? (gp8)(row + 16 * g) : (gp8)(tt_zero_row + 8 * g);
  const bf16x8 lo = p[0], hi = p[1];
#pragma unroll
  for (int r = 0; r < 4; ++r) { t.v[0][r] = (float)lo[r]; t.v[1][r] = (float)lo[4 + r]; t.v[2][r] = (float)hi[r]; t.v[3][r] = (float)hi[4 + r]; }
  return t;
}

ADT_DEVICE_INLINE void tt_save(float* buf, size_t row, const TT& t, bool valid, int g, int as_bf16) {
  if (!buf) return;
  if (as_bf16) tt_store_bf16(reinterpret_cast<__bf16*>(buf) + row * 64, t, valid, g);
  else tt_store(buf + row * 64, t, valid, g);
}
typedef unsigned tt_u4 __attribute__((ext_vector_type(4)));
struct TTSaved { tt_u4 q[4]; };
ADT_DEVICE_INLINE TTSaved tt_saved_request(const float* buf, size_t row, bool valid, int g, int as_bf16) {
  typedef const tt_u4 __attribute__((address_space(1))) * gq;
  TTSaved r;
  if (as_bf16) {
    const gq p = valid ? (gq)(reinterpret_cast<const __bf16*>(buf) + row * 64 + 16 * g) : (gq)tt_zero_row;
    r.q[0] = p[0]; r.q[1] = p[1];
    r.q[2] = r.q[3] = tt_u4{0u, 0u, 0u, 0u};
  } else {
    const gq p = valid ? (gq)(buf + row * 64 + 4 * g) : (gq)(tt_zero_row + 4 * g);
#pragma unroll
    for (int nt = 0; nt < 4; ++nt) r.q[nt] = p[4 * nt];
  }
  return r;
}
ADT_DEVICE_INLINE TT tt_saved_value(TTSaved r, int as_bf16) {
// ... 447 lines not shown
```

Before: 436,700 sequences/s.

## Skip HBM loads for all-padding 16-row tiles using per-sequence pad prefixes

```diff
diff --git a/adt_amd/csrc/adt_attn_args.h b/adt_amd/csrc/adt_attn_args.h
--- a/adt_amd/csrc/adt_attn_args.h
+++ b/adt_amd/csrc/adt_attn_args.h
@@ -23,6 +23,7 @@
   int in_bf16;
   int out_bf16;
   const void* do_bf16; const float* do_delta;
+  const int* pad_pre;
 };
 
 }
diff --git a/adt_amd/csrc/adt_bwdchain_args.h b/adt_amd/csrc/adt_bwdchain_args.h
--- a/adt_amd/csrc/adt_bwdchain_args.h
+++ b/adt_amd/csrc/adt_bwdchain_args.h
@@ -36,6 +36,7 @@
   const float* lnl_x; const float* lnl_gamma; float lnl_eps; float* vpart2; float* lnl_dgamma; float* lnl_dbeta;
   void* do_bf16; float* do_delta; float do_scale; int do_hd;
   int nsplit;
+  const int* pad_pre;
 };
 
 }
diff --git a/adt_amd/csrc/adt_sasrec.hip b/adt_amd/csrc/adt_sasrec.hip
--- a/adt_amd/csrc/adt_sasrec.hip
+++ b/adt_amd/csrc/adt_sasrec.hip
@@ -71,6 +71,7 @@
   int64_t part, part_stride;
   int64_t isort, isort_n;
   int64_t dodelta;
+  int64_t padpre;
   int64_t vpart, vcall, lnpart, gnpart;
   int64_t total;
 };
@@ -121,6 +122,7 @@
   w->lnpart = take(LN_PART_BLOCKS * 128);
   w->gnpart = take(4096);
   w->dodelta = take(pl.do_handover ? up64(w->T * 4) : 0);
+  w->padpre = take(pl.pad_elide ? up64(2 * (int64_t)B) : 0);
   w->total = o;
 }
 
@@ -271,7 +273,7 @@
 }
 
 adt::SeqFwdArgs enc_layer_seq_args(const adt_sasrec_cfg* c, const Layout& lo, const WS& w, const StepPlan& pl, const float* P, float* ws, const int32_t* seq,
-                                   float p, const uint32_t* seed, uint32_t b_offset, int i, bool training_outputs, bool lean) {
+                                   float p, const uint32_t* seed, uint32_t b_offset, int i, bool training_outputs, bool lean, const int32_t* dec = nullptr) {
   const int d = (int)w.d, H = (int)w.H, hd = d / H, L = (int)w.L, B = (int)w.B, prec = c->prec;
   const int64_t Td = up64(w.T * w.d);
   float* x = ws + w.enc_x + i * Td;
@@ -288,12 +290,13 @@
   if (training_outputs && H > 1) { a.rec = base + w.e_rec; a.Ws = P + lo.enc(i, E_SW); a.bs = P + lo.enc(i, E_SB); }
   a.wp_base = P + lo.posw(); a.wp_img = prec == ADT_PREC_BF16 ? (const void*)(ws + w.wpack) : nullptr;
   if (lean) { a.xn = nullptr; a.qkv = nullptr; a.saved_bf16 = 1; }
+  if (lean && pl.pad_elide && dec) { a.pad_pre = reinterpret_cast<int*>(ws + w.padpre); a.pad_ids2 = dec; }
   return a;
 }
 
 int encoder_forward(const adt_sasrec_cfg* c, const Layout& lo, const WS& w, const StepPlan& pl, const float* P, float* ws,
                     const int32_t* seq, const int32_t* pos, const int32_t* neg, float p, const uint32_t* seed,
-                    uint32_t b_offset, bool training_outputs, void* st, bool packed = false) {
+                    uint32_t b_offset, bool training_outputs, void* st, bool packed = false, const int32_t* dec = nullptr) {
   const int T = (int)w.T, d = (int)w.d, H = (int)w.H, hd = d / H, L = (int)w.L, B = (int)w.B, prec = c->prec, nl = c->num_layers;
   const int64_t Td = up64(w.T * w.d);
   const uint32_t ro = b_offset * (uint32_t)L;
@@ -312,7 +315,7 @@
     const float* inw = P + lo.enc(i, E_INW);
     const float* inb = P + lo.enc(i, E_INB);
     if (use_seq) {
-      const adt::SeqFwdArgs a = enc_layer_seq_args(c, lo, w, pl, P, ws, seq, p, seed, b_offset, i, training_outputs, lean);
+      const adt::SeqFwdArgs a = enc_layer_seq_args(c, lo, w, pl, P, ws, seq, p, seed, b_offset, i, training_outputs, lean, dec);
       CK(adt_launch_seq_enc_fwd(hd, a, st));
       continue;
     }
@@ -383,6 +386,7 @@
   a.h = a2; a.u = u; a.y = y;
   a.wp_base = P + lo.posw(); a.wp_img = ws + w.wpack;
   if (pl.lean) { a.xn = nullptr; a.qkv = nullptr; a.saved_bf16 = 1; }
+  if (pl.pad_elide) a.pad_pre = reinterpret_cast<int*>(ws + w.padpre) + B_;
   return a;
 }
 int dec_layer_seq_fwd(const Layout& lo, const WS& w, const StepPlan& pl, const float* P, float* ws, const int32_t* dec, float p,
@@ -420,8 +424,9 @@
                       const float* lambdas2, const adt::RingPrefetchArgs& rr, void* st) {
   const int hd = (int)(w.d / w.H), nl = c->num_layers;
   if (!pl.bce_deferred) return 1;
+  if (pl.pad_elide && !dec) return adt_set_error("forward: the pad prefixes need the decoder's ids");
   for (int i = 0; i < nl; ++i) {
-    adt::SeqFwdArgs a = enc_layer_seq_args(c, lo, w, pl, P, ws, seq, p, seed, b_offset, i, true, true);
+    adt::SeqFwdArgs a = enc_layer_seq_args(c, lo, w, pl, P, ws, seq, p, seed, b_offset, i, true, true, dec);
     if (i == nl - 1) { a.lnl_gamma = P + lo.lnl_w(); a.lnl_beta = P + lo.lnl_b(); a.f_out = ws + w.f; }
     CK(adt_launch_seq_enc_fwd(hd, a, st));
   }
@@ -478,6 +483,7 @@
   void* do_rows_cross() const { return sp.do_handover ? (void*)s1 : nullptr; }
   float* do_delta() const { return sp.do_handover ? ws + w.dodelta : nullptr; }
   float do_scale(uint32_t site) const { return adt_make_drop(p, seed, site).scale; }
+  const int* pad_pre(bool dec_stack) const { return sp.pad_elide ? reinterpret_cast<const int*>(ws + w.padpre) + (dec_stack ? w.B : 0) : nullptr; }
   const float* f;
   SideStream *sd, *sd_sort;
 
@@ -571,6 +577,7 @@
   a.db0 = Gq + lo.dec(i, D_C2B); a.db1 = Gq + lo.dec(i, D_C1B); a.db2 = Gq + lo.dec(i, D_EOB);
   a.out0 = x.s1;
   a.do_bf16 = x.do_rows_cross(); a.do_delta = x.do_delta(); a.do_scale = x.do_scale(dec_site(i, 1)); a.do_hd = x.hd;
+  a.pad_pre = x.pad_pre(true);
   a.part[0] = x.PART(i, PS_D_C2); a.part[1] = x.PART(i, PS_D_C1); a.part[2] = x.PART(i, PS_D_EO); a.part_stride = (size_t)w.part_stride;
   a.vpart = x.VPART(i, 0);
   const int rc = x.sp.use_seq ? adt_launch_seq_post_bwd(x.hd, 0, a, x.st) : 1;
@@ -616,6 +623,7 @@
   a.part_stride = (size_t)w.part_stride;
   a.vpart = x.VPART(i, 1);
   a.do_bf16 = x.do_rows(); a.do_delta = x.do_delta(); a.do_scale = x.do_scale(dec_site(i, 0)); a.do_hd = x.hd;
+  a.pad_pre = x.pad_pre(true);
   return a;
 }
 
@@ -627,6 +635,7 @@
                                                  x.hd, x.p, x.seed, dec_site(i, 1), x.b_offset, x.s5, d, x.s4, 2 * d, x.s4 + d / 2, 2 * d,
                                                  reinterpret_cast<const uint32_t*>(base + w.d_mask2), 1);
   a.do_bf16 = x.do_rows_cross(); a.do_delta = x.do_delta();
+  a.pad_pre = x.pad_pre(true);
   return a;
 }
 
@@ -678,6 +687,7 @@
     a.x = xi; a.gamma = P + lnw; a.beta = P + lnb; a.Win = P + inw; a.bin = P + inb;
     a.dO = x.s1; a.o = o; a.lse = lse; a.mask = mask; a.dres = dec ? gy : x.s5;
     a.do_bf16 = x.do_rows(); a.do_delta = x.do_delta();
+    a.pad_pre = x.pad_pre(dec);
     a.gx = gx; a.acc = acc; a.dWin = Gq + inw; a.dbin = Gq + inb; a.dgamma = Gq + lnw; a.dbeta = Gq + lnb;
     if (x.plan.seeds_virtual && dec && i > 0) {
       a.acc = 0; a.seed_other = ws + w.enc_x + (nl - i) * x.Td; a.seed_coef = ws + w.norms + 8 + (nl - i);
@@ -810,6 +820,7 @@
   a.part[0] = x.PART(i, PS_E_C2); a.part[1] = x.PART(i, PS_E_C1); a.part[2] = x.PART(i, PS_E_O); a.part_stride = (size_t)w.part_stride;
   a.vpart = x.VPART(i, 3);
   a.do_bf16 = x.do_rows(); a.do_delta = x.do_delta(); a.do_scale = x.do_scale(enc_site(i, 0)); a.do_hd = x.hd;
+  a.pad_pre = x.pad_pre(false);
   if (x.sp.lnl_fused && i == nl - 1) {
     a.gy = x.gf; a.lnl_x = ws + w.enc_x + nl * x.Td; a.lnl_gamma = P + lo.lnl_w(); a.lnl_eps = LN_EPS;
     a.vpart2 = x.call.late_parts ? ws + w.vpart + (int64_t)(5 * nl) * w.vcall : nullptr;
@@ -946,7 +957,8 @@
   training &= ADT_TRAIN_DROPOUT;
   const float p = training ? c->dropout : 0.f;
   const uint32_t ro = b_offset * (uint32_t)L;
-  CK(encoder_forward(c, lo, w, pl, P, ws, seq, pos, neg, p, seed, b_offset, true, st, packed));
+  if (pl.pad_elide && !dec) return adt_set_error("forward: the pad prefixes need the decoder's ids");
+  CK(encoder_forward(c, lo, w, pl, P, ws, seq, pos, neg, p, seed, b_offset, true, st, packed, dec));
   const float* f = ws + w.f;
   const int dd = d * d;
   const int B_ = (int)w.B;
diff --git a/adt_amd/csrc/adt_seq.hip b/adt_amd/csrc/adt_seq.hip
--- a/adt_amd/csrc/adt_seq.hip
+++ b/adt_amd/csrc/adt_seq.hip
@@ -34,7 +34,7 @@
     SeqSwitches s;
     s.seq = adt_env_on("ADT_SEQ"); s.seq_lean = adt_env_on("ADT_SEQ_LEAN"); s.seq_tt = adt_env_on("ADT_SEQ_TT"); s.seq_bwd = adt_env_on("ADT_SEQ_BWD");
     s.seq_attn_bwd = adt_env_on("ADT_SEQ_ATTN_BWD"); s.seq_post_bwd = adt_env_on("ADT_SEQ_POST_BWD"); s.seq_partials = adt_env_on("ADT_SEQ_PARTIALS");
-    s.xattn_fused = adt_env_on("ADT_XATTN_FUSED"); s.do_bf16 = adt_env_on("ADT_DO_BF16");
+    s.xattn_fused = adt_env_on("ADT_XATTN_FUSED"); s.do_bf16 = adt_env_on("ADT_DO_BF16"); s.pad_elide = adt_env_on("ADT_PAD_ELIDE");
     s.seq_ablate = adt_env_int("ADT_SEQ_ABLATE", 0); s.seq_ablate_set = adt_env_int("ADT_SEQ_ABLATE", INT_MIN) != INT_MIN;
     s.seq_split = adt_env_int("ADT_SEQ_SPLIT", 0); s.attn_split = adt_env_on("ADT_ATTN_SPLIT");
     s.side_stream = adt_env_int("ADT_SIDE_STREAM", 7); s.side_stream_dp = adt_env_int("ADT_SIDE_STREAM_DP", 0) != 0;
@@ -86,18 +86,30 @@
   return adt_seq_fwd_tt(adt_seq_switches(), a.wp_img != nullptr, a.L);
 }
 
+static std::atomic<unsigned long long> g_pad_elide_launches{0};
+extern "C" unsigned long long adt_seq_pad_elide_launches() { return g_pad_elide_launches.load(); }
+static int pad_refused(int hd, const void* pad_pre) {
+  return (pad_pre && hd == 16) ? adt_set_error("per-sequence kernels: pad prefixes with 16-wide heads") : 0;
+}
+static int pad_counted(int rc, const void* pad_pre) {
+  if (rc == 0 && pad_pre) ++g_pad_elide_launches;
+  return rc;
+}
+
 int adt_launch_seq_enc_fwd(int hd, const SeqFwdArgs& a, void* stream) {
   static AdtLdsOptIn optin[3], optin_tt[3];
+  if (pad_refused(hd, a.pad_pre)) return -1;
   SeqFwdArgs args = a;
   seq_ablate(args);
   hipStream_t s = (hipStream_t)stream;
   if (seq_use_tt(args)) {
     const int nsp = args.nsplit > 1 ? args.nsplit : 1;
     const size_t smem_tt = SeqTtLds<6>::bytes;
-    if (hd == 64) return seq_launch((const void*)k_seqtt_enc_fwd<64>, smem_tt, optin_tt[0], a.B * nsp, &args, s, "seqtt_enc_fwd<64>", TQ_FWD_NW);
-    if (hd == 32) return seq_launch((const void*)k_seqtt_enc_fwd<32>, smem_tt, optin_tt[1], a.B * nsp, &args, s, "seqtt_enc_fwd<32>", TQ_FWD_NW);
-    if (hd == 16) return seq_launch((const void*)k_seqtt_enc_fwd<16>, smem_tt, optin_tt[2], a.B * nsp, &args, s, "seqtt_enc_fwd<16>", TQ_FWD_NW);
-  }
+    if (hd == 64) return pad_counted(seq_launch((const void*)k_seqtt_enc_fwd<64>, smem_tt, optin_tt[0], a.B * nsp, &args, s, "seqtt_enc_fwd<64>", TQ_FWD_NW), a.pad_pre);
+    if (hd == 32) return pad_counted(seq_launch((const void*)k_seqtt_enc_fwd<32>, smem_tt, optin_tt[1], a.B * nsp, &args, s, "seqtt_enc_fwd<32>", TQ_FWD_NW), a.pad_pre);
+    if (hd == 16) return pad_counted(seq_launch((const void*)k_seqtt_enc_fwd<16>, smem_tt, optin_tt[2], a.B * nsp, &args, s, "seqtt_enc_fwd<16>", TQ_FWD_NW), a.pad_pre);
+  }
+  if (a.pad_pre) return adt_set_error("seq_enc_fwd: the pad prefixes belong to the transposed-chain kernels (L=%d hd=%d)", a.L, hd);
   args.nsplit = 0;
   const size_t smem = SeqFwdLds<6>::bytes;
   if (hd == 64) return seq_launch((const void*)k_seq_enc_fwd<64, 2>, smem, optin[0], a.B, &args, s, "seq_enc_fwd<64>");
@@ -108,16 +120,18 @@
 
 int adt_launch_seq_dec_fwd(int hd, const SeqFwdArgs& a, void* stream) {
   static AdtLdsOptIn optin[3], optin_tt[3];
+  if (pad_refused(hd, a.pad_pre)) return -1;
   SeqFwdArgs args = a;
   seq_ablate(args);
   hipStream_t s = (hipStream_t)stream;
   if (seq_use_tt(args)) {
     const int nsp = args.nsplit > 1 ? args.nsplit : 1;
     const size_t smem_tt = SeqTtLds<5>::bytes;
-    if (hd == 64) return seq_launch((const void*)k_seqtt_dec_fwd<64>, smem_tt, optin_tt[0], a.B * nsp, &args, s, "seqtt_dec_fwd<64>", TQ_FWD_NW);
-    if (hd == 32) return seq_launch((const void*)k_seqtt_dec_fwd<32>, smem_tt, optin_tt[1], a.B * nsp, &args, s, "seqtt_dec_fwd<32>", TQ_FWD_NW);
-    if (hd == 16) return seq_launch((const void*)k_seqtt_dec_fwd<16>, smem_tt, optin_tt[2], a.B * nsp, &args, s, "seqtt_dec_fwd<16>", TQ_FWD_NW);
-  }
+    if (hd == 64) return pad_counted(seq_launch((const void*)k_seqtt_dec_fwd<64>, smem_tt, optin_tt[0], a.B * nsp, &args, s, "seqtt_dec_fwd<64>", TQ_FWD_NW), a.pad_pre);
+    if (hd == 32) return pad_counted(seq_launch((const void*)k_seqtt_dec_fwd<32>, smem_tt, optin_tt[1], a.B * nsp, &args, s, "seqtt_dec_fwd<32>", TQ_FWD_NW), a.pad_pre);
+    if (hd == 16) return pad_counted(seq_launch((const void*)k_seqtt_dec_fwd<16>, smem_tt, optin_tt[2], a.B * nsp, &args, s, "seqtt_dec_fwd<16>", TQ_FWD_NW), a.pad_pre);
+  }
+  if (a.pad_pre) return adt_set_error("seq_dec_fwd: the pad prefixes belong to the transposed-chain kernels (L=%d hd=%d)", a.L, hd);
   args.nsplit = 0;
   const size_t smem = SeqFwdLds<5>::bytes;
   if (hd == 64) return seq_launch((const void*)k_seq_dec_fwd<64>, smem, optin[0], a.B, &args, s, "seq_dec_fwd<64>");
@@ -160,7 +174,7 @@
   if (a.nsplit != 2) args.nsplit = 1;
   const int rc = seq_launch(fns[mode], smem, optin[mode], a.B * args.nsplit, &args, s, "seqtt_attn_pre_bwd");
   if (rc == 0 && a.do_bf16) ++g_do_handover_launches;
-  return rc;
+  return pad_counted(rc, a.pad_pre);
 }
 
 int adt_launch_seq_attn_pre_bwd(int hd, int dec, const SeqBwdArgs& a, void* stream) {
@@ -168,6 +182,7 @@
   f.L = a.L; f.H = a.H; f.B = a.B; f.T = a.B * a.L; f.wimg = a.wp_img != nullptr;
   if (!adt_covers_attn_pre_bwd(adt_seq_switches(), hd, f)) return 1;
   if (a.do_bf16 && !a.do_delta) return adt_set_error("seqtt_attn_pre_bwd: handed-over dO rows without their delta");
+  if (pad_refused(hd, a.pad_pre)) return -1;
   const int mode = a.drop.thr == 0 ? 0 : (a.mask != nullptr ? 1 : 2);
   hipStream_t s = (hipStream_t)stream;
   if (hd == 32) return dec ? seq_attn_pre_bwd_t<32, true>(mode, a, s) : seq_attn_pre_bwd_t<32, false>(mode, a, s);
@@ -177,13 +192,14 @@
 
 int adt_launch_seq_post_bwd(int hd, int enc, const BwdChainArgs& a, void* stream) {
   if (!adt_covers_post_bwd(adt_seq_switches(), hd, enc != 0, chain_facts(a))) return 1;
+  if (pad_refused(hd, a.pad_pre)) return -1;
   static AdtLdsOptIn optin[6];
   const void* fns[6] = {(const void*)k_seqtt_post_bwd<64, false>, (const void*)k_seqtt_post_bwd<64, true>, (const void*)k_seqtt_post_bwd<32, false>,
                         (const void*)k_seqtt_post_bwd<32, true>, (const void*)k_seqtt_post_bwd<16, false>, (const void*)k_seqtt_post_bwd<16, true>};
   const int slot = (hd == 64 ? 0 : hd == 32 ? 2 : 4) + (enc ? 1 : 0);
   BwdChainArgs args = a;
   args.stamps = enc ? seq_stamp_buffer_post() : nullptr;
-  return seq_launch(fns[slot], SeqPostLds<3>::bytes, optin[slot], a.B * (a.nsplit > 1 ? a.nsplit : 1), &args, (hipStream_t)stream, "seqtt_post_bwd", SP_NW);
+  return pad_counted(seq_launch(fns[slot], SeqPostLds<3>::bytes, optin[slot], a.B * (a.nsplit > 1 ? a.nsplit : 1), &args, (hipStream_t)stream, "seqtt_post_bwd", SP_NW), a.pad_pre);
 }
 
 int adt_launch_seq_mid_bwd(int hd, const BwdChainArgs& a, void* stream) {
@@ -217,6 +233,9 @@
   a.part_stride = ch.part_stride;
   a.do_bf16 = ch.do_bf16; a.do_delta = ch.do_delta; a.do_scale = ch.do_scale;
   a.dO_bf16 = reinterpret_cast<const __bf16*>(at.do_bf16); a.dO_delta = at.do_delta;
+  if (at.pad_pre && ch.pad_pre && at.pad_pre != ch.pad_pre) return adt_set_error("seqtt_xattn_mid_bwd: the two argument blocks name different pad prefixes");
+  a.pad_pre = at.pad_pre ? at.pad_pre : ch.pad_pre;
+  if (pad_refused(hd, a.pad_pre)) return -1;
   if (at.do_bf16 && !at.do_delta) return adt_set_error("seqtt_xattn_mid_bwd: handed-over dO rows without their delta");
   a.stamps = seq_stamp_buffer_mode(6);
   const int mode = at.drop.thr == 0 ? 0 : 1;
@@ -228,7 +247,7 @@
   const int rc = seq_launch(fns[slot], xm_lds_bytes(at.L, at.H), optin[slot], at.B, &a, (hipStream_t)stream, "seqtt_xattn_mid_bwd", XM_NW, most);
   if (rc == 0) ++g_xattn_fused_launches;
   if (rc == 0 && at.do_bf16) ++g_do_handover_launches;
-  return rc;
+  return pad_counted(rc, a.pad_pre);
 }
 
 struct PartReduceArgs {
diff --git a/adt_amd/csrc/adt_seq_args.h b/adt_amd/csrc/adt_seq_args.h
--- a/adt_amd/csrc/adt_seq_args.h
+++ b/adt_amd/csrc/adt_seq_args.h
@@ -38,6 +38,7 @@
   int ablate;
   const float* lnl_gamma; const float* lnl_beta; float* f_out;
   int nsplit;
+  int* pad_pre; const int* pad_ids2;
 };
 
 }
diff --git a/adt_amd/csrc/adt_seqbwd_args.h b/adt_amd/csrc/adt_seqbwd_args.h
--- a/adt_amd/csrc/adt_seqbwd_args.h
+++ b/adt_amd/csrc/adt_seqbwd_args.h
@@ -26,6 +26,7 @@
   float* vpart;
   int nsplit;
   unsigned long long* stamps;
+  const int* pad_pre;
 };
 
 }
diff --git a/adt_amd/csrc/adt_seqbwd_tt.cuh b/adt_amd/csrc/adt_seqbwd_tt.cuh
--- a/adt_amd/csrc/adt_seqbwd_tt.cuh
+++ b/adt_amd/csrc/adt_seqbwd_tt.cuh
@@ -244,6 +244,7 @@
     a.dWin += off; a.dbin += off; a.dgamma += off; a.dbeta += off;
   }
   float* const part = a.part ? a.part + (size_t)blockIdx.x * a.part_stride : nullptr;
+  const int padn = (HD != 16 && a.pad_pre) ? a.pad_pre[b] : 0;
   SB_STAMP(0);
   constexpr int MI = (H * R * 2 + NW * 64 - 1) / (NW * 64), LI = (H * R + NW * 64 - 1) / (NW * 64);
   tt_u4 mreg[MI];
@@ -284,7 +285,7 @@
   for (int s = 0; s < 2; ++s) {
     const int tile = TM(s);
     const int l = tile * 16 + c, row = b * L + l;
-    xa[s] = tt_load(a.x + (size_t)row * 64, tile >= 0 && l < L, g);
+    xa[s] = tt_load(a.x + (size_t)row * 64, tile >= 0 && l < L && !tt_pad_tile(tile, padn, L), g);
     if (DEC) idv[s] = tt_load_id(a.ids, row, tile >= 0 && l < L);
   }
   SB_STAMP(11);
@@ -316,8 +317,9 @@
     const int l = tile * 16 + c, row = b * L + l;
     const bool valid = tile >= 0 && l < L;
     if (hand) {
-      dob[s] = tt_load_bf16_raw(reinterpret_cast<const __bf16*>(a.do_bf16) + (size_t)row * 64, valid, g);
-      tt_delta_load<H>(a.do_delta, (size_t)row, valid, delta[s]);
+      const bool live = valid && !(DEC && tt_pad_tile(tile, padn, L));
+      dob[s] = tt_load_bf16_raw(reinterpret_cast<const __bf16*>(a.do_bf16) + (size_t)row * 64, live, g);
+      tt_delta_load<H>(a.do_delta, (size_t)row, live, delta[s]);
     } else {
       doa[s] = tt_load(a.dO + (size_t)row * 64, valid, g);
       oa[s] = tt_load_saved(a.o, row, valid, g, a.saved_bf16);
@@ -414,7 +416,7 @@
       for (int s2 = 0; s2 < 2; ++s2) {
         const int tile2 = TM(s2);
         const int l2 = tile2 * 16 + c;
-        xk[s2] = tt_load(a.x + (size_t)(b * L + l2) * 64, tile2 >= 0 && l2 < L, g);
+        xk[s2] = tt_load(a.x + (size_t)(b * L + l2) * 64, tile2 >= 0 && l2 < L && !tt_pad_tile(tile2, padn, L), g);
       }
     }
     const int tile = TB(s);
@@ -458,7 +460,7 @@
   for (int s = 0; s < 2; ++s) {
     const int tile = TA(s);
     const int l = tile * 16 + c;
-    resa[s] = tt_load(a.dres + (size_t)(b * L + l) * 64, tile >= 0 && l < L, g);
+    resa[s] = tt_load(a.dres + (size_t)(b * L + l) * 64, tile >= 0 && l < L && !(DEC && tt_pad_tile(tile, padn, L)), g);
   }
   sb_dw_product16(img0, img1, npair, a.dWin, part, sRed + 128, w, c, g);
   if (DEC) sb_dw_product16(img2, img1, npair, a.dWin + 4096, part ? part + 4096 : nullptr, sRed + 192, w, c, g);
diff --git a/adt_amd/csrc/adt_seqfwd_tt.cuh b/adt_amd/csrc/adt_seqfwd_tt.cuh
--- a/adt_amd/csrc/adt_seqfwd_tt.cuh
+++ b/adt_amd/csrc/adt_seqfwd_tt.cuh
@@ -120,6 +120,21 @@
   for (int i = threadIdx.x; i < (int)(nbytes / 16); i += NTHREADS) q[i] = make_uint4(0u, 0u, 0u, 0u);
 }
 
+constexpr int TQ_PAD_WAVE = 8;
+ADT_DEVICE_INLINE void tq_pad_finish(const int* ids, int* pad_pre, int b, int L, int lane) {
+  static_assert(TQ_LP <= 256, "four ids per lane cover a sequence");
+  int id[4];
+#pragma unroll
+  for (int k = 0; k < 4; ++k) id[k] = tt_load_id(ids, b * L + lane + 64 * k, lane + 64 * k < L);
+  int first = L;
+#pragma unroll
+  for (int k = 3; k >= 0; --k) {
+    const unsigned long long nz = __ballot(id[k] != 0);
+    if (nz) first = 64 * k + __builtin_ctzll(nz);
+  }
+  if (lane == 0) pad_pre[b] = first;
+}
+
 struct TqX { TT e; TT p; int id; };
 ADT_DEVICE_INLINE TqX tq_x_request(const SeqFwdArgs& a, int row, int l, bool valid, int id, int g) {
   TqX r;
@@ -225,6 +240,7 @@
   const int nsp = a.nsplit > 1 ? a.nsplit : 1, b = blockIdx.x / nsp, part = blockIdx.x % nsp;
   const int L = a.L, ntiles = (L + 15) / 16;
   const bool own[2] = {tq_tile12(0, w, ntiles) >= 0 && tq_tile12(0, w, ntiles) % nsp == part, tq_tile12(1, w, ntiles) >= 0 && tq_tile12(1, w, ntiles) % nsp == part};
+  const int padn = (HD != 16 && a.pad_pre && a.x) ? a.pad_pre[b] : 0;
   TQ_STAMP(0);
   uint32_t seedv = 0u;
   TqX xr[2];
@@ -250,7 +266,7 @@
 #pragma unroll
     for (int s = 0; s < 2; ++s) {
       const int tile = (s == 1 && htile >= 0) ? htile : tq_tile12(s, w, ntiles), l = tile * 16 + c;
-      xr[s] = tq_x_request(a, b * L + l, l, tile >= 0 && l < L, idr[s], g);
+      xr[s] = tq_x_request(a, b * L + l, l, tile >= 0 && l < L && !tt_pad_tile(tile, padn, L), idr[s], g);
     }
     if (a.x) {
 #pragma unroll
@@ -346,6 +362,8 @@
     if (a.f_out) tt_store(a.f_out + (size_t)row * 64, tt_layernorm(y, lds.vec + SV_LNL_G, lds.vec + SV_LNL_B, a.ln_eps, g), valid, g);
     TQ_STAMP(7 + 3 * s);
   }
+  if (HD != 16 && a.pad_pre && !a.x && part == 0 && (w == TQ_PAD_WAVE || w == TQ_PAD_WAVE + 1))
+    tq_pad_finish(w == TQ_PAD_WAVE ? a.ids : a.pad_ids2, a.pad_pre + (w == TQ_PAD_WAVE ? 0 : a.B), b, L, lane);
 }
 
 template <int HD>
@@ -359,6 +377,7 @@
   const int nsp = a.nsplit > 1 ? a.nsplit : 1, b = blockIdx.x / nsp, part = blockIdx.x % nsp;
   const int L = a.L, ntiles = (L + 15) / 16;
   const bool own[2] = {tq_tile12(0, w, ntiles) >= 0 && tq_tile12(0, w, ntiles) % nsp == part, tq_tile12(1, w, ntiles) >= 0 && tq_tile12(1, w, ntiles) % nsp == part};
+  const int padn = (HD != 16 && a.pad_pre && a.x) ? a.pad_pre[b] : 0;
   uint32_t seedv = 0u;
   const bool tq_body = TQW * 64 <= TQ_CH || threadIdx.x < TQ_CH;
   const bool tq_tail = (int)threadIdx.x < TQ_CH - TQW * 64;
@@ -383,7 +402,7 @@
 #pragma unroll
     for (int s = 0; s < 2; ++s) {
       const int tile = (s == 1 && htile >= 0) ? htile : tq_tile12(s, w, ntiles), l = tile * 16 + c;
-      xr[s] = tq_x_request(a, b * L + l, l, tile >= 0 && l < L, idr[s], g);
+      xr[s] = tq_x_request(a, b * L + l, l, tile >= 0 && l < L && !tt_pad_tile(tile, padn, L), idr[s], g);
     }
     if (a.x) {
 #pragma unroll
diff --git a/adt_amd/csrc/adt_seqpost_tt.cuh b/adt_amd/csrc/adt_seqpost_tt.cuh
--- a/adt_amd/csrc/adt_seqpost_tt.cuh
+++ b/adt_amd/csrc/adt_seqpost_tt.cuh
@@ -73,6 +73,7 @@
   const bool cls = ENC && H > 1 && a.drec != nullptr;
   sp_replica(a);
   SB_STAMP(0);
+  const int padn = (HD != 16 && a.pad_pre) ? a.pad_pre[b] : 0;
   const float* const ws3[3] = {a.W0, a.W1, a.W2};
   sp_wdma<3, NW>(a, ws3, wimg);
   TT dy[NS], xl[NS];
@@ -83,10 +84,11 @@
     const int tile = tileof(s);
     const int l = tile * 16 + c, row = b * L + l;
     const bool valid = tile >= 0 && l < L;
-    dy[s] = tt_load(a.gy + (size_t)row * 64, valid, g);
+    const bool live = valid && !tt_pad_tile(tile, padn, L);
+    dy[s] = tt_load(a.gy + (size_t)row * 64, lnl ? valid : live, g);
     if (ENC) xl[s] = tt_load(a.lnl_x + (size_t)row * 64, valid && lnl, g);
-    uraw[s] = tt_saved_request(a.u, row, valid, g, a.saved_bf16);
-    hreq[s] = tt_saved_request(a.xin, row, valid, g, a.saved_bf16);
+    uraw[s] = tt_saved_request(a.u, row, live, g, a.saved_bf16);
+    hreq[s] = tt_saved_request(a.xin, row, live, g, a.saved_bf16);
     idv[s] = tt_load_id(a.ids, row, valid);
   }
   if (a.gy_scale != 0.f) {
@@ -169,7 +171,7 @@
     if (tile < 0) continue;
     const int l = tile * 16 + c, row = b * L + l;
     const bool valid = l < L;
-    oreq[s] = tt_saved_request(a.o, row, valid, g, a.saved_bf16);
+    oreq[s] = tt_saved_request(a.o, row, valid && (cls || !tt_pad_tile(tile, padn, L)), g, a.saved_bf16);
     if constexpr (H == 2) {
       if (cls) {
         typedef const f32x4 __attribute__((address_space(1))) * gf4;
diff --git a/adt_amd/csrc/adt_seqxattn_tt.cuh b/adt_amd/csrc/adt_seqxattn_tt.cuh
--- a/adt_amd/csrc/adt_seqxattn_tt.cuh
+++ b/adt_amd/csrc/adt_seqxattn_tt.cuh
@@ -18,6 +18,7 @@
   void* do_bf16; float* do_delta; float do_scale;
   const __bf16* dO_bf16; const float* dO_delta;
   unsigned long long* stamps;
+  const int* pad_pre;
 };
 
 __host__ __device__ inline int xm_rows(int L) { return (L + 31) / 32 <= 4 ? 128 : SB_R; }
@@ -70,6 +71,7 @@
   const int nqt = (L + 15) / 16, npair = (L + 31) / 32;
 #define XM_STAMP(k) do { if (a.stamps && blockIdx.x == 0 && lane == 0) a.stamps[w * 16 + (k)] = __builtin_amdgcn_s_memtime(); } while (0)
   XM_STAMP(0);
+  const int padn = (HD != 16 && a.pad_pre) ? a.pad_pre[b] : 0;
   if (a.nrep > 1) {
     const size_t off = (size_t)(blockIdx.x % a.nrep) * a.rep_stride;
     if (a.db0) a.db0 += off;
@@ -113,9 +115,10 @@
     const gb4 pv = ok ? (gb4)(a.V + row * a.ldv + pa) : zb, po = ok ? (gb4)(a.O + row * a.ldo + pa) : zb;
     qa[k] = pq[0]; qc[k] = pq[4]; ka[k] = pk[0]; kc[k] = pk[4]; va[k] = pv[0]; vc[k] = pv[4];
     if (hand) {
-      const gb4 pdb = ok ? (gb4)(a.dO_bf16 + row * 64 + pa) : zb;
+      const bool okd = ok && !tt_pad_tile(r >> 4, padn, L);
+      const gb4 pdb = okd ? (gb4)(a.dO_bf16 + row * 64 + pa) : zb;
       da[k] = pdb[0]; dc[k] = pdb[4];
-      dlt[k] = *(ok ? (gf1)(a.dO_delta + row * 4 + (i & 7) / (HD / 8)) : (gf1)tt_zero_row);
+      dlt[k] = *(okd ? (gf1)(a.dO_delta + row * 4 + (i & 7) / (HD / 8)) : (gf1)tt_zero_row);
     } else {
       const gp4 pd = ok ? (gp4)(a.dO + row * a.lddo + c8) : (gp4)tt_zero_row + (i & 7);
       oa[k] = po[0]; oc[k] = po[4];
@@ -181,6 +184,7 @@
   const int lA = qt * 16 + c, lB = kt * 16 + c;
   const bool validA = has && lA < L, validB = has && lB < L;
   const size_t rowA = row_b + lA, rowB = row_b + lB;
+  const bool liveA = validA && !(hand && tt_pad_tile(qt, padn, L));
 
   TTB dq = xm_zero();
   bf16x4 fkl[NF], fkh[NF], fvl[NF], fvh[NF];
@@ -220,7 +224,7 @@
       adt_glds_block<NW>(reinterpret_cast<const __bf16*>(a.wp_img) + 6 * (ws4[j] - a.wp_base) + 3 * WPACK_IMG, wimg + j * TT_WIMG, TT_WIMG * 2);
   }
   TTSaved a1req;
-  if constexpr (HD != 16) a1req = tt_saved_request(a.xin, rowA, validA, g, 1);
+  if constexpr (HD != 16) a1req = tt_saved_request(a.xin, rowA, liveA, g, 1);
 
   TTB dk = xm_zero(), dv = xm_zero();
   if (has) {
@@ -246,13 +250,13 @@
         }
     }
   }
-  if constexpr (HD == 16) a1req = tt_saved_request(a.xin, rowA, validA, g, 1);
+  if constexpr (HD == 16) a1req = tt_saved_request(a.xin, rowA, liveA, g, 1);
   XM_STAMP(6);
   adt_wait_vm0();
   __syncthreads();
   XM_STAMP(7);
   TT da1 = tt_zero();
-  const TTSaved oreq = tt_saved_request(a.o, rowA, validA, g, 1);
+  const TTSaved oreq = tt_saved_request(a.o, rowA, liveA, g, 1);
   const TT fx = tt_load(a.f + rowB * 64, validB, g);
   if (has) {
     xm_put_rows(img0, lA, dq);
diff --git a/adt_amd/csrc/adt_step_plan.h b/adt_amd/csrc/adt_step_plan.h
--- a/adt_amd/csrc/adt_step_plan.h
+++ b/adt_amd/csrc/adt_step_plan.h
@@ -29,6 +29,7 @@
   bool embed3 = true;
   bool bce_merged = true;
   bool do_bf16{true};
+  bool pad_elide{true};
 };
 
 constexpr bool adt_seq_head_ok(int hd) { return hd == 16 || hd == 32 || hd == 64; }
@@ -98,6 +99,7 @@
   int side_sites;
   bool side_dp;
   bool loss_one_launch;
+  bool pad_elide;
   bool do_handover;
 };
 
@@ -132,6 +134,7 @@
   p.side_dp = sw.side_stream_dp;
   p.loss_one_launch = nl <= 4;
   p.do_handover = sw.do_bf16 && p.parts;
+  p.pad_elide = sw.pad_elide && p.parts && hd != 16;
   return p;
 }
 
diff --git a/adt_amd/csrc/adt_tt.cuh b/adt_amd/csrc/adt_tt.cuh
--- a/adt_amd/csrc/adt_tt.cuh
+++ b/adt_amd/csrc/adt_tt.cuh
@@ -82,6 +82,7 @@
   for (int nt = 0; nt < 4; ++nt) t.v[nt] = p[4 * nt];
   return t;
 }
+ADT_DEVICE_INLINE bool tt_pad_tile(int tile, int pad, int L) { return pad > 0 && min(tile * 16 + 16, L) <= pad; }
 ADT_DEVICE_INLINE TT tt_load_if(const float* row, bool valid, int g) {
   TT t;
 #pragma unroll
```

Measured after the change: 441,300 sequences/s, median of 6. +1.1%, better.
